# ObiRobotics/pf_monocular_pose_estimator

Hardware: AMD Instinct MI355X
Metric: particle-updates/sec (propagate+weight+resample) per GPU; frames/sec at N_particles (higher is better)
Workload: dtype f32; 1 GPU; C2: 5 LEDs, 100000 particles, 50 blobs/frame, f32 SoA state (BASELINE.json configs[1]); fused_fallbacks=0, state=f32, N_particles=100000, markers=5, blobs=50, rng=philox, parallelism=1 independent camera streams (1 per GPU), no collectives

## Files before the change

### include/pfmpe.h

```cpp
#ifndef PFMPE_H_
#define PFMPE_H_

#include <stdint.h>

#ifdef __cplusplus
extern "C" {
#endif

#define PFMPE_ABI_VERSION 1
#define PFMPE_MAX_MARKERS 16
#define PFMPE_MAX_BLOBS 1024

enum {
  PFMPE_OK = 0,
  PFMPE_E_ARG = -1,
  PFMPE_E_HIP = -2,
  PFMPE_E_CAP = -3,
  PFMPE_E_STATE = -4
};

enum { PFMPE_STATE_F32 = 0, PFMPE_STATE_F64 = 1, PFMPE_STATE_F16 = 2 };

enum {
  PFMPE_RNG_REFERENCE = 0,
// ... 113 lines not shown
void pfmpe_default_init_params(pfmpe_init_params* p);
int pfmpe_p3p_histogram(pfmpe_ctx* ctx, const double* blobs, int B, uint32_t* hist);
int pfmpe_initialise(pfmpe_ctx* ctx, const double* blobs, int B, const pfmpe_init_params* params,
                     pfmpe_init_out* out, uint32_t* hist);

#define PFMPE_INIT_MAX_STREAMS 64

typedef struct {
  const double* blobs;
  int32_t B;
  int32_t pad;
} pfmpe_init_in;
int pfmpe_initialise_multi(pfmpe_ctx* const* ctxs, int S, const pfmpe_init_in* in, const pfmpe_init_params* params,
                           pfmpe_init_out* out, uint32_t* const* hist);

typedef struct {
  int64_t items;
  int32_t first_block;
  int32_t blocks;
  int32_t bucket;
  int32_t lds_hist;
} pfmpe_init_plan;
int pfmpe_host_init_plan(const int32_t* M, const int32_t* B, int S, int num_cu, pfmpe_init_plan* plan,
                         int32_t* blocks_per_bucket);

typedef struct {
  int32_t threshold_value;
  int32_t active_markers;
  double gaussian_sigma;
  double min_blob_area;
  double max_blob_area;
  double max_width_height_distortion;
  double max_circular_distortion;
  double D[5];
  int32_t roi_x, roi_y, roi_w, roi_h;
} pfmpe_detect_params;
typedef struct {
  int32_t n;
  int32_t n_components;
  int32_t overflow;
  int32_t pad;
} pfmpe_detect_out;
void pfmpe_default_detect_params(pfmpe_detect_params* p);
int pfmpe_stage_image(pfmpe_ctx* ctx, const uint8_t* image, int width, int height, int pitch);
int pfmpe_find_leds(pfmpe_ctx* ctx, const uint8_t* image, int width, int height, int pitch,
                    const pfmpe_detect_params* params, double* blobs, float* distorted, int max_out,
                    pfmpe_detect_out* out);

#define PFMPE_DETECT_MAX_ROIS 64

int pfmpe_find_leds_multi(pfmpe_ctx* ctx, const uint8_t* image, int width, int height, int pitch,
                          const pfmpe_detect_params* params, int R, double* blobs, float* distorted,
                          int max_out, pfmpe_detect_out* out);

#define PFMPE_DETECT_MAX_IMAGES 64

typedef struct {
  pfmpe_ctx* ctx;
  const uint8_t* image;
  int32_t width, height, pitch, pad;
} pfmpe_detect_image;
int pfmpe_find_leds_streams(const pfmpe_detect_image* images, int I, const int32_t* image_of,
                            const pfmpe_detect_params* params, int R, double* blobs, float* distorted, int max_out,
                            pfmpe_detect_out* out);

typedef struct {
  int64_t offset;
  int32_t pitch;
  int32_t shared_with;
} pfmpe_detect_crop;
int pfmpe_host_detect_plan(const pfmpe_detect_image* images, int I, const int32_t* image_of,
                           const pfmpe_detect_params* params, int R, pfmpe_detect_crop* crops,
                           int64_t* upload_bytes);
int pfmpe_host_detect_pack(const pfmpe_detect_image* images, int I, const int32_t* image_of,
                           const pfmpe_detect_params* params, int R, const pfmpe_detect_crop* crops,
                           uint8_t* buffer, int64_t buffer_bytes);

int pfmpe_host_grow_roi(const int32_t roi[4], int32_t margin, int32_t image_w, int32_t image_h, int32_t grown[4]);

int pfmpe_parse_marker_yaml(const char* text, double* xyz, int max_markers);
typedef struct {
  pfmpe_params pf;
  pfmpe_init_params init;
  int32_t num_objects;
  int32_t markers_per_object[4];
  int32_t use_particle_filter;
  uint8_t downgrade[PFMPE_MAX_MARKERS];
} pfmpe_launch_config;
void pfmpe_default_launch_config(pfmpe_launch_config* cfg);
int pfmpe_parse_launch(const char* text, pfmpe_launch_config* cfg);
int pfmpe_parse_camera_info(const char* text, double* K, double* D, int32_t* width, int32_t* height);
int pfmpe_write_blob_stream(const char* path, const double* timestamps, const double* blobs, const int32_t* offsets,
                            int n_frames);
int pfmpe_read_blob_stream(const char* path, double* timestamps, double* blobs, int32_t* offsets, int max_frames,
                           int64_t max_blobs, int* n_frames, int64_t* n_blobs);
int pfmpe_stage_blob_stream(pfmpe_ctx* ctx, const char* path, int* n_frames);

int pfmpe_get_particles(pfmpe_ctx* ctx, int which, double* out);
int pfmpe_get_weights(pfmpe_ctx* ctx, double* out);
int pfmpe_get_counts(pfmpe_ctx* ctx, uint32_t* out);

enum { PFMPE_CLOUD_WEIGHTED = 0,
       PFMPE_CLOUD_POSTERIOR = 1 };
typedef struct {
  int64_t n;
  int32_t degenerate;
  int32_t pad;
  double wsum, ess;
  double mean_twist[6];
  double cov[36];
  double mean_pose[12];
  double max_trans, max_rot;
} pfmpe_cloud_out;
int pfmpe_cloud_stats(pfmpe_ctx* ctx, int which, const double* ref_pose12, pfmpe_cloud_out* out);

#define PFMPE_CLOUD_MAX_STREAMS 64

typedef struct {
  double ref_pose[12];
  int32_t which;
  int32_t pad;
} pfmpe_cloud_in;
int pfmpe_cloud_stats_multi(pfmpe_ctx* const* ctxs, int S, const pfmpe_cloud_in* in, pfmpe_cloud_out* out);

typedef struct { int32_t first_block, blocks; } pfmpe_cloud_plan;
int pfmpe_host_cloud_plan(const int32_t* N, int S, pfmpe_cloud_plan* plan, int32_t* total_blocks);

#define PFMPE_MODES_MAX 16
#define PFMPE_MODE_NONE 255
typedef struct {
  double trans_scale;
  double rot_scale;
  double max_dist;
} pfmpe_modes_params;
typedef struct {
  pfmpe_cloud_out stats;
  double share;
} pfmpe_mode_out;
void pfmpe_default_modes_params(pfmpe_modes_params* p);
int pfmpe_cloud_modes(pfmpe_ctx* ctx, int which, const double* seeds , int K,
                      const pfmpe_modes_params* params ,
                      pfmpe_mode_out* out , uint8_t* mode_of );
int pfmpe_host_cloud_assign(const double* poses, int64_t N, const double* seeds, int K,
                            const pfmpe_modes_params* params, uint8_t* mode_of, int64_t* counts );

enum { PFMPE_ASSOC_PROPAGATED = 0, PFMPE_ASSOC_POSTERIOR = 1 };
typedef struct {
  const double* blobs;
  int32_t B;
  int32_t bank_frame;
} pfmpe_assoc_in;
typedef struct {
  int64_t n;
  int32_t M, B;
  int64_t n_any;
  uint32_t matched[PFMPE_MAX_MARKERS];
  uint32_t mode_blob[PFMPE_MAX_MARKERS];
  uint32_t mode_votes[PFMPE_MAX_MARKERS];
  uint32_t second_votes[PFMPE_MAX_MARKERS];
  uint32_t npairs_hist[PFMPE_MAX_MARKERS + 1];
  uint32_t pad;
} pfmpe_assoc_out;
int pfmpe_assoc_stats(pfmpe_ctx* ctx, int which, const pfmpe_assoc_in* in, pfmpe_assoc_out* out, uint32_t* votes);
int pfmpe_get_pairs(pfmpe_ctx* ctx, int which, const pfmpe_assoc_in* in, int64_t first, int32_t count,
                    uint32_t* corr, int32_t* n_corr);

#define PFMPE_ASSOC_MAX_STREAMS 64
#define PFMPE_ASSOC_MAX_LAUNCHES 16

typedef struct {
  pfmpe_assoc_in blobs;
  int32_t which;
  int32_t pad;
} pfmpe_assoc_multi_in;
int pfmpe_assoc_stats_multi(pfmpe_ctx* const* ctxs, int S, const pfmpe_assoc_multi_in* in,
                            pfmpe_assoc_out* out, uint32_t* const* votes);

typedef struct {
  int64_t bins_offset;
  int32_t first_block, blocks, launch, lds_votes;
} pfmpe_assoc_plan;
typedef struct {
  int64_t bins_words;
  int32_t launches, pad;
  int32_t launch_blocks[PFMPE_ASSOC_MAX_LAUNCHES];
} pfmpe_assoc_plan_total;
int pfmpe_host_assoc_plan(const int32_t* N, const int32_t* M, const int32_t* B, const int32_t* which ,
                          const int32_t* prune , const int32_t* table_bytes , int S,
                          int state_dtype, pfmpe_assoc_plan* plan, pfmpe_assoc_plan_total* total);

typedef struct { double min_share; double lead; int32_t min_pairs; int32_t pad; } pfmpe_gate_params;
typedef struct { int32_t n_in, n_gated, fallback, pad; uint8_t reason[PFMPE_MAX_MARKERS]; } pfmpe_gate_out;
void pfmpe_default_gate_params(pfmpe_gate_params* p);
int pfmpe_host_gate_pairs(const uint32_t* votes, int M, int B, const uint32_t* corr ,
                          int n_corr, const pfmpe_gate_params* params ,
                          uint32_t* gated , pfmpe_gate_out* out);

#define PFMPE_TOP_MAX  1024
#define PFMPE_TOP_POOL 1024
enum { PFMPE_TOP_BY_WEIGHT = 0, PFMPE_TOP_BY_COUNT = 1 };
typedef struct {
  int32_t key;
  int32_t K;
  double  min_trans;
  double  min_rot;
} pfmpe_top_params;
typedef struct {
  int64_t n;
  int64_t n_positive;
  int32_t n_out;
  int32_t n_examined;
} pfmpe_top_out;
void pfmpe_default_top_params(pfmpe_top_params* p);
int pfmpe_top_particles(pfmpe_ctx* ctx, const pfmpe_top_params* params, const pfmpe_assoc_in* blobs, pfmpe_top_out* out,
                        int32_t* index, double* key_value, double* poses, uint32_t* corr, int32_t* n_corr);
int pfmpe_host_top_suppress(const double* poses, int32_t P, int32_t K, double min_trans, double min_rot,
                            int32_t* keep, int32_t* n_out, int32_t* n_examined);

typedef struct {
  int32_t max_iter;
  int32_t revert_on_divergence;
  double  converged;
} pfmpe_refine_params;
void pfmpe_default_refine_params(pfmpe_refine_params* p);

enum { PFMPE_REFINE_NO_PAIRS = 0, PFMPE_REFINE_CONVERGED = 1, PFMPE_REFINE_CAP_KEPT = 2, PFMPE_REFINE_CAP_REVERTED = 3 };
typedef struct {
  double pose[12];
  double rms_before, rms_after;
  int32_t iters;
  int32_t n_pairs;
  int32_t status, pad;
} pfmpe_refine_row;

typedef struct {
  int64_t n, n_with_pairs, n_converged, n_cap_kept, n_cap_reverted;
  int64_t iters_total; int32_t iters_max; int32_t pad;
  int64_t best;
  pfmpe_refine_row best_row;
  double best_cov[36];
} pfmpe_refine_out;

int pfmpe_refine_poses(pfmpe_ctx* ctx, const pfmpe_assoc_in* blobs, const pfmpe_refine_params* params,
                       const double* poses, const uint32_t* corr, int32_t K, pfmpe_refine_out* out,
                       pfmpe_refine_row* rows, double* cov);
int pfmpe_refine_cloud(pfmpe_ctx* ctx, int which, const pfmpe_assoc_in* blobs, const pfmpe_refine_params* params,
                       int64_t first, int32_t count, pfmpe_refine_out* out, pfmpe_refine_row* rows, double* cov);
#define PFMPE_REFINE_MAX_STREAMS 64
#define PFMPE_REFINE_MULTI_MAX_HYPOTHESES 65536
#define PFMPE_REFINE_DESC_BYTES 48

typedef struct {
  pfmpe_assoc_in blobs;
  const double* poses;
  const uint32_t* corr;
  int32_t K;
  int32_t pad;
} pfmpe_refine_in;
int pfmpe_refine_multi(pfmpe_ctx* const* ctxs, int S, const pfmpe_refine_in* in, const pfmpe_refine_params* params,
                       pfmpe_refine_out* out, pfmpe_refine_row* const* rows, double* const* cov);

typedef struct {
  int64_t first;
  int64_t model_offset;
  int64_t blobs_offset;
} pfmpe_refine_plan;
typedef struct {
  int64_t hypotheses;
  int64_t desc_offset, stream_of_offset, poses_offset, corr_offset;
  int64_t upload_bytes, download_bytes;
} pfmpe_refine_plan_total;
int pfmpe_host_refine_plan(const int32_t* K, const int32_t* B, int S, pfmpe_refine_plan* plan,
                           pfmpe_refine_plan_total* total);

int pfmpe_host_optimise_pose(const double* markers_xyz, int M, const double* K, const double* blobs, int B,
                             const uint32_t* corr, int n_rows, const pfmpe_refine_params* params, const double* pose12,
                             pfmpe_refine_row* row, double* cov36);

int pfmpe_step_refine(pfmpe_ctx* ctx, const pfmpe_frame_in* in, const pfmpe_refine_params* params,
                      pfmpe_frame_out* out, pfmpe_refine_out* gn, pfmpe_refine_row* row, double* cov36);
int pfmpe_step_refine_multi(pfmpe_ctx* const* ctxs, int S, const pfmpe_frame_in* in, const pfmpe_refine_params* params,
                            pfmpe_frame_out* out, pfmpe_refine_out* gn, pfmpe_refine_row* rows, double* cov);
int pfmpe_host_step_tail(const double* markers_xyz, int M, const double* K, const double* blobs, int B,
                         const pfmpe_frame_out* frame, const pfmpe_refine_params* params, pfmpe_refine_out* gn,
                         pfmpe_refine_row* row, double* cov36);

enum { PFMPE_OPT_RECORD_COUNTS = 1, PFMPE_OPT_PRUNE = 2, PFMPE_OPT_TIMING = 3, PFMPE_OPT_FUSED = 4,
       PFMPE_OPT_KEEP_PROPAGATED = 5, PFMPE_OPT_WAIT_BOUND_US = 6, PFMPE_OPT_FUSED_REARM = 7,
       PFMPE_OPT_MULTI_MAX_BLOCKS = 8, PFMPE_OPT_DEFER_RESAMPLE = 9 };
int pfmpe_set_option(pfmpe_ctx* ctx, int option, int64_t value);

enum { PFMPE_SHAPE_TWO_LAUNCH = 0,
       PFMPE_SHAPE_FRAME = 1,
       PFMPE_SHAPE_FRAME2 = 2 };
enum { PFMPE_INFO_FUSED = 1,
       PFMPE_INFO_FUSED_FALLBACKS = 2,
       PFMPE_INFO_LAST_SHAPE = 3,
       PFMPE_INFO_GUARD_SKIPS = 4,
       PFMPE_INFO_N = 5,
       PFMPE_INFO_LAST_WEIGH_PASS = 6,
       PFMPE_INFO_LAST_GRID = 7,
       PFMPE_INFO_LAST_RESAMPLE = 8,
       PFMPE_INFO_NUM_CU = 9,
       PFMPE_INFO_TAIL_FALLBACKS = 10 };
enum { PFMPE_WEIGH_BLOCKS = 0, PFMPE_WEIGH_STREAM = 1, PFMPE_WEIGH_PK = 2 };
enum { PFMPE_RESAMPLE_BLOCKS = 0, PFMPE_RESAMPLE_OWNERS = 1 };
int pfmpe_get_info(const pfmpe_ctx* ctx, int key, int64_t* value);

int pfmpe_stage_blob_bank(pfmpe_ctx* ctx, const double* blobs, const int32_t* offsets, int nframes);

enum { PFMPE_K_PROPAGATE = 0,
       PFMPE_K_RESAMPLE = 1,
       PFMPE_K_AUX = 2,
       PFMPE_K_FRAME = 3,
       PFMPE_K_ROI = 4,
       PFMPE_K_FINAL = 5,
       PFMPE_K_P3P_HIST = 6,
       PFMPE_K_P3P_CHECK = 7,
       PFMPE_K_DETECT = 8,
       PFMPE_K_COUNT = 9 };
int pfmpe_get_kernel_stats(pfmpe_ctx* ctx, int kernel, int64_t* launches, double* total_ms);
int pfmpe_reset_kernel_stats(pfmpe_ctx* ctx);
const char* pfmpe_kernel_name(int kernel);

double pfmpe_host_ref_uniform(uint32_t seed, uint64_t j, double a, double b);
void pfmpe_host_philox(const uint32_t ctr[4], const uint32_t key[2], uint32_t out[4]);
void pfmpe_host_pose_twist(const double* pose12, const double* ref_pose12, double* twist6);
int pfmpe_host_assoc_summary(const uint32_t* votes, int M, int B, pfmpe_assoc_out* out);

#ifdef __cplusplus
}
#endif
#endif
```

### pf_monocular_pose_estimator_amd/__init__.py

```python
from ._capi import (
    Engine, FrameIn, FrameOut, Params, PFError, default_params, load, host_philox, host_ref_uniform,
    STATE_F32, STATE_F64, STATE_F16, RNG_REFERENCE, RNG_PHILOX, FLAG_ACCEPTED, FLAG_REINIT,
    OPT_RECORD_COUNTS, OPT_PRUNE, OPT_TIMING, OPT_FUSED, OPT_KEEP_PROPAGATED, K_FRAME, K_ROI, K_FINAL, MAX_MARKERS, MAX_BLOBS, LIB_PATH,
    OPT_WAIT_BOUND_US, OPT_FUSED_REARM, OPT_MULTI_MAX_BLOCKS, OPT_DIAG, DIAG_LAG_LOADS, DIAG_ABANDON, DIAG_NO_STREAM, DIAG_FORCE_STREAM,
    DIAG_SERIAL_TOP, DIAG_NO_PK, DIAG_CORRUPT_DESC, DIAG_NO_DEFER, DIAG_BLOCK_RESAMPLE, DIAG_MIN_SIDE, DIAG_ABANDON_FINISH, OPT_DEFER_RESAMPLE, OK, E_ARG, E_HIP, E_CAP, E_STATE,
    SHAPE_TWO_LAUNCH, SHAPE_FRAME, SHAPE_FRAME2, INFO_FUSED, INFO_FUSED_FALLBACKS, INFO_LAST_SHAPE,
    INFO_GUARD_SKIPS, INFO_N, INFO_LAST_WEIGH_PASS, INFO_LAST_GRID, INFO_LAST_RESAMPLE, RESAMPLE_BLOCKS, RESAMPLE_OWNERS, WEIGH_BLOCKS, WEIGH_STREAM, WEIGH_PK,
    CLOUD_WEIGHTED, CLOUD_POSTERIOR, CloudOut, host_pose_twist,
    ASSOC_PROPAGATED, ASSOC_POSTERIOR, DIAG_ASSOC_DIRECT, AssocIn, AssocOut, host_assoc_summary,
    REFINE_NO_PAIRS, REFINE_CONVERGED, REFINE_CAP_KEPT, REFINE_CAP_REVERTED, REFINE_ROW_DTYPE, RefineParams, RefineRow,
    RefineOut, default_refine_params, host_optimise_pose,
    DETECT_MAX_ROIS, DetectParams, DetectOut, host_grow_roi,
    ROI_MAX_STREAMS, RoiIn, RoiOut, host_predict_roi,
    DETECT_MAX_IMAGES, DIAG_DET_COPY, DetectImage, DetectCrop, host_detect_plan, host_detect_pack,
    INIT_MAX_STREAMS, INFO_NUM_CU, InitIn, InitPlan, InitParams, InitOut, host_init_plan,
    REFINE_MAX_STREAMS, REFINE_MULTI_MAX_HYPOTHESES, REFINE_DESC_BYTES, RefineIn, RefinePlan, RefinePlanTotal,
    host_refine_plan,
    DIAG_TAIL_MISS, INFO_TAIL_FALLBACKS, host_step_tail,
    CLOUD_MAX_STREAMS, CloudIn, CloudPlan, host_cloud_plan,
    TOP_MAX, TOP_POOL, TOP_BY_WEIGHT, TOP_BY_COUNT, TopParams, TopOut, default_top_params, host_top_suppress,
    MODES_MAX, MODE_NONE, ModesParams, ModeOut, default_modes_params, host_cloud_assign,
    ASSOC_MAX_STREAMS, ASSOC_MAX_LAUNCHES, AssocMultiIn, AssocPlan, AssocPlanTotal, host_assoc_plan,
    GateParams, GateOut, default_gate_params, host_gate_pairs,
)

__all__ = [
    "Engine", "FrameIn", "FrameOut", "Params", "PFError", "default_params", "load",
    "STATE_F32", "STATE_F64", "RNG_REFERENCE", "RNG_PHILOX",
]
```

### pf_monocular_pose_estimator_amd/_capi.py

```python
from __future__ import annotations

import ctypes as C
import os

import numpy as np

_HERE = os.path.dirname(os.path.abspath(__file__))
LIB_PATH = os.path.join(_HERE, "libpfmpe.so")

MAX_MARKERS = 16
MAX_BLOBS = 1024

OK, E_ARG, E_HIP, E_CAP, E_STATE = 0, -1, -2, -3, -4
STATE_F32, STATE_F64, STATE_F16 = 0, 1, 2
RNG_REFERENCE, RNG_PHILOX = 0, 1
FLAG_ACCEPTED, FLAG_REINIT = 1, 4
OPT_RECORD_COUNTS, OPT_PRUNE, OPT_TIMING, OPT_FUSED, OPT_KEEP_PROPAGATED = 1, 2, 3, 4, 5
OPT_WAIT_BOUND_US, OPT_FUSED_REARM, OPT_MULTI_MAX_BLOCKS = 6, 7, 8
OPT_DIAG = 99
DIAG_LAG_LOADS, DIAG_ABANDON, DIAG_NO_STREAM, DIAG_FORCE_STREAM, DIAG_SERIAL_TOP = 64, 128, 512, 1024, 2048
DIAG_NO_PK, DIAG_CORRUPT_DESC, DIAG_NO_DEFER, DIAG_BLOCK_RESAMPLE, DIAG_MIN_SIDE = 4096, 8192, 16384, 32768, 65536
DIAG_ABANDON_FINISH = 131072
DIAG_DET_COPY = 524288
DIAG_TAIL_MISS = 1 << 20
DIAG_ASSOC_DIRECT = 262144
OPT_DEFER_RESAMPLE = 9
SHAPE_TWO_LAUNCH, SHAPE_FRAME, SHAPE_FRAME2 = 0, 1, 2
INFO_FUSED, INFO_FUSED_FALLBACKS, INFO_LAST_SHAPE, INFO_GUARD_SKIPS, INFO_N, INFO_LAST_WEIGH_PASS = 1, 2, 3, 4, 5, 6
INFO_LAST_GRID, INFO_LAST_RESAMPLE, INFO_NUM_CU, INFO_TAIL_FALLBACKS = 7, 8, 9, 10
WEIGH_BLOCKS, WEIGH_STREAM, WEIGH_PK = 0, 1, 2
RESAMPLE_BLOCKS, RESAMPLE_OWNERS = 0, 1
CLOUD_WEIGHTED, CLOUD_POSTERIOR = 0, 1
ASSOC_PROPAGATED, ASSOC_POSTERIOR = 0, 1
REFINE_NO_PAIRS, REFINE_CONVERGED, REFINE_CAP_KEPT, REFINE_CAP_REVERTED = 0, 1, 2, 3
K_PROPAGATE, K_RESAMPLE, K_AUX, K_FRAME, K_ROI, K_FINAL, K_P3P_HIST, K_P3P_CHECK, K_DETECT, K_COUNT = range(10)

EXPORTED_SYMBOLS = (
    "pfmpe_create", "pfmpe_destroy", "pfmpe_last_error", "pfmpe_abi_version",
    "pfmpe_set_model", "pfmpe_set_params", "pfmpe_default_params", "pfmpe_set_prior",
    "pfmpe_step", "pfmpe_step_batch", "pfmpe_step_multi", "pfmpe_step_multi_batch", "pfmpe_get_particles", "pfmpe_get_weights", "pfmpe_get_counts",
    "pfmpe_set_option", "pfmpe_stage_blob_bank", "pfmpe_get_kernel_stats",
    "pfmpe_reset_kernel_stats", "pfmpe_kernel_name", "pfmpe_host_ref_uniform", "pfmpe_host_philox",
    "pfmpe_predict_roi", "pfmpe_default_init_params", "pfmpe_p3p_histogram", "pfmpe_initialise",
    "pfmpe_parse_marker_yaml", "pfmpe_default_launch_config", "pfmpe_parse_launch", "pfmpe_parse_camera_info",
    "pfmpe_write_blob_stream", "pfmpe_read_blob_stream", "pfmpe_stage_blob_stream",
    "pfmpe_default_detect_params", "pfmpe_stage_image", "pfmpe_find_leds", "pfmpe_get_info",
    "pfmpe_cloud_stats", "pfmpe_host_pose_twist",
    "pfmpe_assoc_stats", "pfmpe_get_pairs", "pfmpe_host_assoc_summary",
    "pfmpe_default_refine_params", "pfmpe_refine_poses", "pfmpe_refine_cloud", "pfmpe_host_optimise_pose",
    "pfmpe_find_leds_multi", "pfmpe_host_grow_roi",
    "pfmpe_predict_roi_multi", "pfmpe_host_predict_roi",
    "pfmpe_find_leds_streams", "pfmpe_host_detect_plan", "pfmpe_host_detect_pack",
    "pfmpe_initialise_multi", "pfmpe_host_init_plan",
    "pfmpe_refine_multi", "pfmpe_host_refine_plan",
    "pfmpe_step_refine", "pfmpe_step_refine_multi", "pfmpe_host_step_tail",
    "pfmpe_cloud_stats_multi", "pfmpe_host_cloud_plan",
    "pfmpe_default_top_params", "pfmpe_top_particles", "pfmpe_host_top_suppress",
    "pfmpe_default_modes_params", "pfmpe_cloud_modes", "pfmpe_host_cloud_assign",
    "pfmpe_assoc_stats_multi", "pfmpe_host_assoc_plan", "pfmpe_default_gate_params", "pfmpe_host_gate_pairs",
)
MODES_MAX = 16
MODE_NONE = 255
TOP_MAX = 1024
TOP_POOL = 1024
TOP_BY_WEIGHT, TOP_BY_COUNT = 0, 1
DETECT_MAX_ROIS = 64
DETECT_MAX_IMAGES = 64
ROI_MAX_STREAMS = 64
INIT_MAX_STREAMS = 64
REFINE_MAX_STREAMS = 64
CLOUD_MAX_STREAMS = 64
ASSOC_MAX_STREAMS = 64
ASSOC_MAX_LAUNCHES = 16
REFINE_MULTI_MAX_HYPOTHESES = 65536
REFINE_DESC_BYTES = 48


class Params(C.Structure):
    _fields_ = [
        ("tol", C.c_double), ("tol_pf", C.c_double),
        ("ang_min", C.c_double), ("ang_max", C.c_double),
        ("trans_min", C.c_double), ("trans_max", C.c_double),
        ("growth", C.c_double),
        ("max_iter", C.c_int32), ("exit_cap", C.c_int32), ("accept_cap", C.c_int32),
        ("rng_mode", C.c_int32),
    ]


class FrameIn(C.Structure):
    _fields_ = [
        ("current_pose", C.c_double * 12), ("predicted_pose", C.c_double * 12),
        ("prediction", C.c_double * 12), ("cam_move_inv", C.c_double * 12),
        ("blobs", C.POINTER(C.c_double)), ("B", C.c_int32), ("bank_frame", C.c_int32),
        ("it_since_init", C.c_int32), ("force_iters", C.c_int32),
        ("dt", C.c_double), ("seed", C.c_uint64), ("frame_idx", C.c_uint64),
    ]


class RoiIn(C.Structure):
    _fields_ = [
        ("cam_move_inv", C.c_double * 12), ("prediction", C.c_double * 12), ("predicted_pose", C.c_double * 12),
        ("D", C.c_double * 5), ("image_w", C.c_int32), ("image_h", C.c_int32), ("border", C.c_int32),
        ("pad", C.c_int32),
    ]


class RoiOut(C.Structure):
    _fields_ = [("x", C.c_int32), ("y", C.c_int32), ("width", C.c_int32), ("height", C.c_int32),
                ("bbox", C.c_double * 4)]


class InitParams(C.Structure):
    _fields_ = [("certainty_threshold", C.c_double), ("valid_corr_threshold", C.c_double),
                ("n_particles", C.c_int32), ("max_candidates", C.c_int32)]


class InitOut(C.Structure):
    _fields_ = [("found", C.c_int32), ("flag_fail", C.c_int32), ("n_estimates", C.c_int32),
                ("n_candidates", C.c_int32), ("first_match", C.c_int32), ("n_corr", C.c_int32),
                ("corr", C.c_uint32 * (2 * MAX_MARKERS)), ("predicted_pose", C.c_double * 12),
                ("hist_total", C.c_uint64)]

    def as_dict(self) -> dict:
        return {"found": self.found, "flag_fail": self.flag_fail, "n_estimates": self.n_estimates,
                "n_candidates": self.n_candidates, "first_match": self.first_match,
                "pairs": np.array(self.corr[: 2 * self.n_corr], dtype=np.uint32).reshape(-1, 2),
                "predicted_pose": np.array(self.predicted_pose), "hist_total": self.hist_total}


class InitIn(C.Structure):
    _fields_ = [("blobs", C.POINTER(C.c_double)), ("B", C.c_int32), ("pad", C.c_int32)]


class InitPlan(C.Structure):
    _fields_ = [("items", C.c_int64), ("first_block", C.c_int32), ("blocks", C.c_int32), ("bucket", C.c_int32),
                ("lds_hist", C.c_int32)]

    def as_dict(self) -> dict:
        return {k: getattr(self, k) for k, _ in self._fields_}


class DetectParams(C.Structure):
    _fields_ = [("threshold_value", C.c_int32), ("active_markers", C.c_int32), ("gaussian_sigma", C.c_double),
                ("min_blob_area", C.c_double), ("max_blob_area", C.c_double),
                ("max_width_height_distortion", C.c_double), ("max_circular_distortion", C.c_double),
                ("D", C.c_double * 5), ("roi_x", C.c_int32), ("roi_y", C.c_int32), ("roi_w", C.c_int32),
                ("roi_h", C.c_int32)]


class DetectOut(C.Structure):
    _fields_ = [("n", C.c_int32), ("n_components", C.c_int32), ("overflow", C.c_int32), ("pad", C.c_int32)]


class DetectImage(C.Structure):
    _fields_ = [("ctx", C.c_void_p), ("image", C.POINTER(C.c_uint8)), ("width", C.c_int32), ("height", C.c_int32),
                ("pitch", C.c_int32), ("pad", C.c_int32)]


class DetectCrop(C.Structure):
    _fields_ = [("offset", C.c_int64), ("pitch", C.c_int32), ("shared_with", C.c_int32)]


class LaunchConfig(C.Structure):
    _fields_ = [("pf", Params), ("init", InitParams), ("num_objects", C.c_int32),
                ("markers_per_object", C.c_int32 * 4), ("use_particle_filter", C.c_int32),
                ("downgrade", C.c_uint8 * MAX_MARKERS)]


class FrameOut(C.Structure):
    _fields_ = [
        ("iters", C.c_int32), ("kept_iter", C.c_int32), ("most_likely_idx", C.c_int32),
        ("accepted", C.c_int32), ("resampled", C.c_int32), ("winner_idx", C.c_int32),
        ("n_corr", C.c_int32), ("flag_fail", C.c_int32),
        ("highest_prob", C.c_double), ("prob_sum", C.c_double),
        ("winner_pose", C.c_double * 12), ("most_likely_pose", C.c_double * 12),
        ("corr", C.c_uint32 * (2 * MAX_MARKERS)),
    ]

    def pairs(self) -> np.ndarray:
        return np.array(self.corr[: 2 * self.n_corr], dtype=np.uint32).reshape(-1, 2)

    def as_dict(self) -> dict:
        return {
            "iters": self.iters, "kept_iter": self.kept_iter, "most_likely_idx": self.most_likely_idx,
            "accepted": self.accepted, "resampled": self.resampled, "winner_idx": self.winner_idx,
            "n_corr": self.n_corr, "flag_fail": self.flag_fail, "highest_prob": self.highest_prob,
            "prob_sum": self.prob_sum, "winner_pose": np.array(self.winner_pose),
            "most_likely_pose": np.array(self.most_likely_pose), "pairs": self.pairs(),
        }


class CloudOut(C.Structure):
    _fields_ = [("n", C.c_int64), ("degenerate", C.c_int32), ("pad", C.c_int32),
                ("wsum", C.c_double), ("ess", C.c_double), ("mean_twist", C.c_double * 6),
                ("cov", C.c_double * 36), ("mean_pose", C.c_double * 12),
                ("max_trans", C.c_double), ("max_rot", C.c_double)]

    def as_dict(self) -> dict:
        return {"n": self.n, "degenerate": self.degenerate, "wsum": self.wsum, "ess": self.ess,
                "mean_twist": np.array(self.mean_twist), "cov": np.array(self.cov).reshape(6, 6),
                "mean_pose": np.array(self.mean_pose), "max_trans": self.max_trans, "max_rot": self.max_rot}


class CloudIn(C.Structure):
    _fields_ = [("ref_pose", C.c_double * 12), ("which", C.c_int32), ("pad", C.c_int32)]


class CloudPlan(C.Structure):
    _fields_ = [("first_block", C.c_int32), ("blocks", C.c_int32)]

    def as_dict(self) -> dict:
        return {"first_block": self.first_block, "blocks": self.blocks}


class ModesParams(C.Structure):
    _fields_ = [("trans_scale", C.c_double), ("rot_scale", C.c_double), ("max_dist", C.c_double)]


class ModeOut(C.Structure):
    _fields_ = [("stats", CloudOut), ("share", C.c_double)]

    def as_dict(self) -> dict:
        d = self.stats.as_dict()
        d["share"] = self.share
        return d


assert C.sizeof(ModesParams) == 24 and C.sizeof(CloudOut) == 480 and C.sizeof(ModeOut) == 488


class AssocIn(C.Structure):
    _fields_ = [("blobs", C.POINTER(C.c_double)), ("B", C.c_int32), ("bank_frame", C.c_int32)]


class AssocOut(C.Structure):
    _fields_ = [("n", C.c_int64), ("M", C.c_int32), ("B", C.c_int32), ("n_any", C.c_int64),
                ("matched", C.c_uint32 * MAX_MARKERS), ("mode_blob", C.c_uint32 * MAX_MARKERS),
                ("mode_votes", C.c_uint32 * MAX_MARKERS), ("second_votes", C.c_uint32 * MAX_MARKERS),
                ("npairs_hist", C.c_uint32 * (MAX_MARKERS + 1)), ("pad", C.c_uint32)]

    def as_dict(self) -> dict:
        M = self.M
        d = {"n": self.n, "M": M, "B": self.B, "n_any": self.n_any}
        for k in ("matched", "mode_blob", "mode_votes", "second_votes"):
            d[k] = np.array(getattr(self, k)[:M], dtype=np.uint32)
        d["npairs_hist"] = np.array(self.npairs_hist[: M + 1], dtype=np.uint32)
        return d


class AssocMultiIn(C.Structure):
    _fields_ = [("blobs", AssocIn), ("which", C.c_int32), ("pad", C.c_int32)]


class AssocPlan(C.Structure):
    _fields_ = [("bins_offset", C.c_int64), ("first_block", C.c_int32), ("blocks", C.c_int32),
                ("launch", C.c_int32), ("lds_votes", C.c_int32)]

    def as_dict(self) -> dict:
        return {k: getattr(self, k) for k, _ in self._fields_}


class AssocPlanTotal(C.Structure):
    _fields_ = [("bins_words", C.c_int64), ("launches", C.c_int32), ("pad", C.c_int32),
                ("launch_blocks", C.c_int32 * ASSOC_MAX_LAUNCHES)]

    def as_dict(self) -> dict:
        return {"bins_words": self.bins_words, "launches": self.launches,
                "launch_blocks": list(self.launch_blocks[: self.launches])}


class GateParams(C.Structure):
    _fields_ = [("min_share", C.c_double), ("lead", C.c_double), ("min_pairs", C.c_int32), ("pad", C.c_int32)]


class GateOut(C.Structure):
    _fields_ = [("n_in", C.c_int32), ("n_gated", C.c_int32), ("fallback", C.c_int32), ("pad", C.c_int32),
                ("reason", C.c_uint8 * MAX_MARKERS)]


assert (C.sizeof(AssocMultiIn), C.sizeof(AssocPlan), C.sizeof(AssocPlanTotal), C.sizeof(GateParams),
        C.sizeof(GateOut)) == (24, 24, 80, 24, 32)


class TopParams(C.Structure):
    _fields_ = [("key", C.c_int32), ("K", C.c_int32), ("min_trans", C.c_double), ("min_rot", C.c_double)]


class TopOut(C.Structure):
    _fields_ = [("n", C.c_int64), ("n_positive", C.c_int64), ("n_out", C.c_int32), ("n_examined", C.c_int32)]

    def as_dict(self) -> dict:
        return {k: getattr(self, k) for k, _ in self._fields_}


class RefineParams(C.Structure):
    _fields_ = [("max_iter", C.c_int32), ("revert_on_divergence", C.c_int32), ("converged", C.c_double)]


class RefineRow(C.Structure):
    _fields_ = [("pose", C.c_double * 12), ("rms_before", C.c_double), ("rms_after", C.c_double),
                ("iters", C.c_int32), ("n_pairs", C.c_int32), ("status", C.c_int32), ("pad", C.c_int32)]


REFINE_ROW_DTYPE = np.dtype([("pose", np.float64, 12), ("rms_before", np.float64), ("rms_after", np.float64),
                             ("iters", np.int32), ("n_pairs", np.int32), ("status", np.int32), ("pad", np.int32)])


class RefineOut(C.Structure):
    _fields_ = [("n", C.c_int64), ("n_with_pairs", C.c_int64), ("n_converged", C.c_int64), ("n_cap_kept", C.c_int64),
                ("n_cap_reverted", C.c_int64), ("iters_total", C.c_int64), ("iters_max", C.c_int32), ("pad", C.c_int32),
                ("best", C.c_int64), ("best_row", RefineRow), ("best_cov", C.c_double * 36)]

    def as_dict(self) -> dict:
        d = {k: getattr(self, k) for k in ("n", "n_with_pairs", "n_converged", "n_cap_kept", "n_cap_reverted",
                                           "iters_total", "iters_max", "best")}
        d["best_row"] = np.frombuffer(bytes(self.best_row), dtype=REFINE_ROW_DTYPE)[0].copy()
        d["best_cov"] = np.array(self.best_cov).reshape(6, 6)
        return d


class RefineIn(C.Structure):
    _fields_ = [("blobs", AssocIn), ("poses", C.POINTER(C.c_double)), ("corr", C.POINTER(C.c_uint32)),
                ("K", C.c_int32), ("pad", C.c_int32)]


class RefinePlan(C.Structure):
    _fields_ = [("first", C.c_int64), ("model_offset", C.c_int64), ("blobs_offset", C.c_int64)]

    def as_dict(self) -> dict:
        return {k: getattr(self, k) for k, _ in self._fields_}


# ... 1131 lines not shown
```

### pf_monocular_pose_estimator_amd/csrc/pf_kernels.hpp

```cpp
#pragma once
#include <stddef.h>
#include <stdint.h>

#include <algorithm>
#include <cstring>
#include <type_traits>

#include "pf_desc_tag.hpp"
#include "pf_likelihood.hpp"

namespace pfmpe {

template <typename T, int RNG>
__device__ __forceinline__ double target_num(const FrameArgsT<T>& fa, int iters, int64_t k) {
  double U;
  if (RNG == kRngReference) {
    const uint64_t motion = fa.N > 2 ? (uint64_t)12 * (uint64_t)(fa.N - 2) * (uint64_t)iters : 0u;
    const uint32_t g1 = lcg_output(fa.lcg_x0, motion + 2u * (uint64_t)k + 1u);
    const uint32_t g2 = lcg_next(g1);
    U = ref_uniform(ref_canonical(g1, g2), 0.0, 1.0);
  } else {
    const U32x4 o = philox4x32_10((uint32_t)k, kTagResample << 24, fa.flo, fa.fhi, fa.key0, fa.key1);
    U = u53(o.x, o.y);
  }
// ... 2247 lines not shown
  __shared__ ResampleLds<T> rsh;
  __shared__ OutDev rec;
  __shared__ FrameLds fsh;

  if (stamps && threadIdx.x == 0) stamp_min(stamps, 0, rt_now());
  const int n = blockIdx.x * kBlock + threadIdx.x;
  const bool valid = n < fa.N;
  const int lane = lane_id(), wv = wave_id();
  const int blk = blockIdx.x, g = blk / fa.gsz;

  copy_table(table, smem, (size_t)fa.tbytes);
  T A[12];
  if (valid && n >= 2) load_prior(fa, prior, n, A);
  const uint32_t gen_base = ((uint32_t)seq & 0xffffu) << 16;
  Ctrl c = load_ctrl_wt(ctrl);
  stage_consts(fa, sc);
  __syncthreads();
  const LdsBlobs<T> tb = view_table<T>(smem, fa.B);
  if (stamps && threadIdx.x == 0) {
    const uint64_t t = rt_now();
    stamp_max(stamps, 8, t);
    stamp_min(stamps, 19, t);
  }

  T P[12], w = (T)0;
  int iter = 0;
  for (;; ++iter) {
    const int slot = c.cur_slot;
    if (valid) {
      w = weigh_particle<T, RNG, MAXM, PRUNE>(fa, sc, tb, A, n, iter, P);
      (slot ? w1 : w0)[n] = w;
    }
    if (stamps && threadIdx.x == 0) stamp_max(stamps, 9, rt_now());
    publish_iteration<T, RNG>(fa, w, valid, n, slot, iter, wsh, part0, part1, bscan0, bscan1, gpart0, gpart1, gscan,
                              ctrl, gcount_w, tcount_w, gen, gen_base, stamps, blk);
    if (wv == 0) {
      int ab = 0;
      if (lane == 0) {
        const uint32_t want = gen_base + (uint32_t)iter + 1u;
        const uint64_t t0 = rt_now();
        while (__hip_atomic_load((gu32_t*)gen, __ATOMIC_RELAXED, __HIP_MEMORY_SCOPE_AGENT) != want) {
          __builtin_amdgcn_s_sleep(2);
          if (rt_now() - t0 > fa.wait_ticks) {
            ab = 1;
            break;
          }
        }
      }
      ab = lane_value(ab, 0);
      if (!ab) {
        constexpr int kCw = (int)(sizeof(Ctrl) / 8);
        static_assert(sizeof(Ctrl) % 8 == 0 && kCw + 8 <= 64, "Ctrl words");
        const uint64_t* src = nullptr;
        uint64_t* dst = nullptr;
        if (lane < kCw) {
          src = (const uint64_t*)ctrl + lane;
          dst = (uint64_t*)&fsh.c + lane;
        } else if (lane < kCw + 6) {
          const int sl = (lane - kCw) / 3, q = (lane - kCw) % 3;
          src = (const uint64_t*)((sl ? bscan1 : bscan0) + blk) + q;
          dst = (uint64_t*)&fsh.bs[sl] + q;
        } else if (lane < kCw + 8) {
          src = (const uint64_t*)(gscan + g) + (lane - kCw - 6);
          dst = (uint64_t*)&fsh.gs + (lane - kCw - 6);
        }
        if (src) *dst = ld_wt(src);
      }
      if (lane == 0) fsh.abort = ab;
    }
    __syncthreads();
    if (fsh.abort) return;
    c = fsh.c;
    if (c.done) break;
  }

  if (!c.accepted) {
    if (blk == 0 && wv == 0)
      finalize_frame<T, RNG, MAXM, SP>(fa, sc, c, ctrl, prior, -1, cand, mlpose, rec, out, 2 * seq + 1, stamps);
    return;
  }
  const int kslot = c.kept_slot;
  const bool have_P = c.kept_iter == iter;
  double wd = 0.0;
  if (valid) {
    if (have_P) {
      wd = (double)w;
    } else {
      wd = (double)(kslot ? w1 : w0)[n];
    }
  }
  const BlockScan bs = fsh.bs[kslot];
  const GroupScan gs = fsh.gs;
  if (flat)
    resample_phase<T, RNG, MAXM, SP, 2>(fa, sc, c, ctrl, table, prior, post, wd, A, P, have_P, bs, gs, rsh, rec, tb, cand,
                                        mlpose, cpart, cgroup, gcount_r, tcount_r, counts, out, seq, stamps, flat, blk);
  else
    resample_phase<T, RNG, MAXM, SP, 1>(fa, sc, c, ctrl, table, prior, post, wd, A, P, have_P, bs, gs, rsh, rec, tb, cand,
                                        mlpose, cpart, cgroup, gcount_r, tcount_r, counts, out, seq, stamps, nullptr,
                                        blk);
}

struct WaveArg {
  double maxw, minw;
  int argmax, argmin;
};
struct Frame2Lds {
  GroupPart gp[2][kFlatMaxGroups];
  WaveArg wa[2][kWaves];
  BlockScan bs[2];
  int dirty[kWaves];
  GroupScan gs;
  Ctrl c;
  Frame2Tail tail;
  int abort;
};

struct BlockIn {
  bool vb, mine;
  BlockPart p;
};
__device__ __forceinline__ bool group_math2(const BlockIn (&in)[2], GroupPart (&out)[2], BlockScan* own, WaveArg& wa,
                                            double (&zmin_in)[2]) {
  double sum[2], maxrel[2], minrel[2];
  double maxw = -INFINITY, minw = INFINITY;
  int amax = 0x7fffffff, amin = 0x7fffffff;
  bool min_placeholder = true, dirty = false;
#pragma unroll
  for (int k = 0; k < 2; ++k) {
    const bool vb = in[k].vb;
    if (vb) {
      cmb_max(maxw, amax, in[k].p.maxw, in[k].p.argmax);
      cmb_min(minw, amin, in[k].p.minw, in[k].p.argmin);
    }
    min_placeholder &= !vb || (in[k].p.minw == (double)INFINITY && in[k].p.argmin == 0x7fffffff);
    dirty |= vb && !(in[k].p.minw >= 0.0 && in[k].p.sum == in[k].p.sum);
    sum[k] = vb ? in[k].p.sum : 0.0;
    maxrel[k] = vb ? in[k].p.maxrel : -INFINITY;
    minrel[k] = vb ? in[k].p.minrel : INFINITY;
  }
  double incl[2] = {sum[0], sum[1]};
  if (__builtin_amdgcn_ballot_w64(!min_placeholder) == 0) {
    scan_steps([&](auto st) {
      using S = decltype(st);
      st_sum<S>(incl[0]);
      st_sum<S>(incl[1]);
      st_argmax<S>(maxw, amax);
    });
    minw = INFINITY;
    amin = 0x7fffffff;
  } else {
    scan_steps([&](auto st) {
      using S = decltype(st);
      st_sum<S>(incl[0]);
      st_sum<S>(incl[1]);
      st_argmax<S>(maxw, amax);
      st_argmin<S>(minw, amin);
    });
    bcast63(minw, amin);
  }
  double E[2], zi_max[2];
#pragma unroll
  for (int k = 0; k < 2; ++k) {
    E[k] = 0.0 + wave_shr1(incl[k], 0.0);
    zi_max[k] = in[k].vb ? E[k] + maxrel[k] : -INFINITY;
    zmin_in[k] = in[k].vb ? E[k] + minrel[k] : INFINITY;
  }
  scan_steps([&](auto st) {
    using S = decltype(st);
    st_max<S>(zi_max[0]);
    st_max<S>(zi_max[1]);
  });
  bcast63(maxw, amax);
  wa.maxw = maxw;
  wa.minw = minw;
  wa.argmax = amax;
  wa.argmin = amin;
#pragma unroll
  for (int k = 0; k < 2; ++k) {
    double zp_max = wave_shr1(zi_max[k], -(double)INFINITY);
    zp_max = zp_max > -INFINITY ? zp_max : -INFINITY;
    if (in[k].vb && in[k].mine) {
      own->E = E[k];
      own->zin_max = zp_max;
      own->zin_min = INFINITY;
      own->pad = 0.0;
    }
    const double tmax = lane_value(zi_max[k], 63);
    GroupPart& r = out[k];
    r.sum = 0.0 + lane_value(incl[k], 63);
    r.zmax = tmax > -INFINITY ? tmax : -INFINITY;
    r.zmin = INFINITY;
    r.maxw = -INFINITY;
    r.minw = INFINITY;
    r.argmax = r.argmin = 0x7fffffff;
  }
  return __builtin_amdgcn_ballot_w64(dirty) != 0;
}
__device__ __forceinline__ void group_zmin2(const BlockIn (&in)[2], double (&zi_min)[2], BlockScan* own, GroupPart* gp0,
                                            GroupPart* gp1) {
  scan_steps([&](auto st) {
    using S = decltype(st);
    st_min<S>(zi_min[0]);
    st_min<S>(zi_min[1]);
  });
#pragma unroll
  for (int k = 0; k < 2; ++k) {
    double zp_min = wave_shr1(zi_min[k], (double)INFINITY);
    zp_min = zp_min < INFINITY ? zp_min : INFINITY;
    if (in[k].vb && in[k].mine) own->zin_min = zp_min;
    const double tmin = lane_value(zi_min[k], 63);
    GroupPart* g = k ? gp1 : gp0;
    if (g && lane_id() == 0) g->zmin = tmin < INFINITY ? tmin : INFINITY;
  }
}

__device__ __forceinline__ double lanes8_incl_sum(double x) {
  x = x + dpp<kDppRowShr1>(x, 0.0);
  x = x + dpp<kDppRowShr2>(x, 0.0);
  x = x + dpp<kDppRowShr4>(x, 0.0);
  return x + 0.0;
}

template <typename T, int RNG, typename KeptF, typename ArgF>
__device__ __forceinline__ Ctrl top_math_regs(const FrameArgsT<T>& fa, Ctrl c, int iter, int slot, const GroupPart& q0,
                                              KeptF qk, ArgF garg, double* G_out, double* Gin_out,
                                              double* run_out) {
  const int lane = lane_id();
  const int ngrp = fa.ngrp;
  double incl = lanes8_incl_sum(lane < ngrp ? q0.sum : 0.0);
  double mv, mn_;
  int mi, ni_;
  garg(slot, mv, mi, mn_, ni_);
  if (mv > c.best_max) {
    c.best_max = mv;
    c.best_idx = mi;
    c.best_iter = iter;
    c.best_slot = slot;
    c.has_best = 1;
  }
  c.iters = iter + 1;
  const bool go_on = fa.force_iters > 0 ? (c.iters < fa.force_iters) : (c.iters < fa.max_iter && mv < fa.exit_thr);
  c.cur_slot = c.has_best ? 1 - c.best_slot : 1 - slot;
  if (!go_on) {
    c.done = 1;
    c.kept_slot = c.has_best ? c.best_slot : slot;
    c.kept_iter = c.has_best ? c.best_iter : iter;
    GroupPart kq = q0;
    double amv = mv, anv = mn_;
    int ami = mi, ani = ni_;
    if (c.kept_slot != slot) {
      kq = qk(c.kept_slot);
      incl = lanes8_incl_sum(lane < ngrp ? kq.sum : 0.0);
      garg(c.kept_slot, amv, ami, anv, ani);
    }
    const double S = 0.0 + lane_value(incl, 7);
    double run = -INFINITY;
    {
      const double prev = wave_shr1(incl, 0.0);
      const double G = lane == 0 ? 0.0 : 0.0 + prev;
      double cm = -INFINITY;
      if (lane < ngrp && S != 0.0) cm = (G + (S > 0.0 ? kq.zmax : kq.zmin)) / S;
      const double im = wave_incl_max(cm);
      double ex = wave_shr1(im, -(double)INFINITY);
      ex = ex > run ? ex : run;
      *G_out = G;
      *Gin_out = ex;
      const double tm = lane_value(im, 63);
      run = tm > run ? tm : run;
    }
    if (S == 0.0) run = -INFINITY;
    const double highest = c.has_best ? c.best_max : 0.0;
    c.S = S;
    c.invS = 1.0 / S;
    c.accepted = (S != 0.0 && highest > fa.accept_thr) ? 1 : 0;
    if (c.accepted) {
      c.most_likely_idx = c.best_idx;
#if PFMPE_TAIL_KT_IN_COUNTS
      *run_out = run;
      c.K_total = 0;
#else
      int64_t kt = lane == 0 ? count_targets<T, RNG>(fa, c.iters, run) : 0;
      c.K_total = (int64_t)(((uint64_t)(uint32_t)__builtin_amdgcn_readlane((int)(uint32_t)kt, 0)) |
                            ((uint64_t)(uint32_t)__builtin_amdgcn_readlane((int)(uint32_t)((uint64_t)kt >> 32), 0) << 32));
#endif
    } else {
      c.most_likely_idx = (S < 0.0) ? ani : ami;
      c.K_total = 0;
    }
  }
  return c;
}

#ifndef PFMPE_FRAME2_MIN_WAVES
#define PFMPE_FRAME2_MIN_WAVES 3
#endif
template <typename T>
struct Frame2Shared {
  LdsConst<T> sc;
  WeighLds wsh;
  ResampleLds<T> rsh;
  OutDev rec;
  Frame2Lds fl;
};
template <typename T, int RNG, int MAXM, bool PRUNE, typename SP>
__device__ __forceinline__ bool frame2_body(
    const FrameArgsT<T>& fa, const uint32_t* fa_words, const unsigned char* __restrict__ table,
    const SP* __restrict__ prior, SP* __restrict__ post, T* __restrict__ w0, T* __restrict__ w1,
    BlockPart* __restrict__ part0, BlockPart* __restrict__ part1, Ctrl* __restrict__ ctrl,
    CountPart* __restrict__ cpart, uint32_t* __restrict__ flat, uint32_t* __restrict__ counts, Cand* __restrict__ cand,
    double* __restrict__ mlpose, RecOut* __restrict__ out, int32_t seq, uint64_t* __restrict__ stamps,
    unsigned char* smem, Frame2Shared<T>& S2) {
  LdsConst<T>& sc = S2.sc;
  WeighLds& wsh = S2.wsh;
  ResampleLds<T>& rsh = S2.rsh;
  OutDev& rec = S2.rec;
  Frame2Lds& fl = S2.fl;
  if (stamps && threadIdx.x == 0) stamp_min(stamps, 0, rt_now());
  const int n = blockIdx.x * kBlock + threadIdx.x;
  const bool valid = n < fa.N;
  const int lane = lane_id(), wv = wave_id();
  const int blk = blockIdx.x, g_own = blk / fa.gsz;

  T A[12];
  if (valid && n >= 2) load_prior(fa, prior, n, A);
  stage_table_consts(table, smem, (size_t)fa.tbytes, fa_words, sc);
  if (threadIdx.x == 0) {
    fl.c = zero_ctrl();
    fl.abort = 0;
  }
  __syncthreads();
  const LdsBlobs<T> tb = view_table<T>(smem, fa.B);
  if (stamps && threadIdx.x == 0) {
    const uint64_t t = rt_now();
    stamp_max(stamps, 8, t);
    stamp_min(stamps, 19, t);
  }

  T P[12], w = (T)0;
  Ctrl c = fl.c;
  int iter = 0;
  for (;; ++iter) {
    const int slot = c.cur_slot;
    if (valid) {
      w = weigh_particle<T, RNG, MAXM, PRUNE, true>(fa, sc, tb, A, n, iter, P, nullptr, stamps);
      (slot ? w1 : w0)[n] = w;
    }
    if (stamps && threadIdx.x == 0) stamp_max(stamps, 9, rt_now());
    {
      double wi, rmx, rmn;
      T mx, mn;
      int ix, in_;
      wave_weight_partials(w, valid, n, wi, rmx, rmn, mx, ix, mn, in_);
      if (lane == 63) wsh.tot[wv] = wi;
      if (lane == 0) {
        wsh.rmax[wv] = rmx;
        wsh.rmin[wv] = rmn;
        wsh.mx[wv] = (double)mx;
        wsh.mn[wv] = (double)mn;
        wsh.ix[wv] = ix;
        wsh.in_[wv] = in_;
      }
      __syncthreads();
      if (wv == 0) {
        if (lane == 0) {
          double pre = 0.0, maxrel = -INFINITY, minrel = INFINITY, bmx = wsh.mx[0], bmn = wsh.mn[0];
          int bix = wsh.ix[0], bin = wsh.in_[0];
#pragma unroll
          for (int ww = 0; ww < kWaves; ++ww) {
            const double a = pre + wsh.rmax[ww], b = pre + wsh.rmin[ww];
            maxrel = a > maxrel ? a : maxrel;
            minrel = b < minrel ? b : minrel;
            if (ww) {
              cmb_max(bmx, bix, wsh.mx[ww], wsh.ix[ww]);
              cmb_min(bmn, bin, wsh.mn[ww], wsh.in_[ww]);
            }
            pre = pre + wsh.tot[ww];
          }
          BlockPart* bp = ((iter & 1) ? part1 : part0) + blk;
          st_wt_d(&bp->sum, pre);
          st_wt_d(&bp->maxrel, maxrel);
          st_wt_d(&bp->minrel, minrel);
          st_wt_d(&bp->maxw, bmx);
          st_wt_d(&bp->minw, bmn);
          st_wt(&bp->argmax, pack2(bix, bin));
          if (stamps) stamp_max(stamps, 1, rt_now());
          flat_arrive(flat, blk);
        }
        const uint32_t target = fa.flat_base_w + (uint32_t)(iter + 1) * (uint32_t)fa.nblk;
        const bool ok = !(fa.diag & kDiagAbandon) && flat_wait(flat, target, fa.wait_ticks);
        if (lane == 0 && !ok) fl.abort = 1;
      }
      __syncthreads();
      if (fl.abort) return false;
    }
    if (stamps && threadIdx.x == 0) stamp_max(stamps, 2, rt_now());
    BlockIn in[2];
    double zmin_in[2];
    {
      const BlockPart* pp = (iter & 1) ? part1 : part0;
      if ((fa.diag & kDiagLagLoads) && blk == fa.nblk - 1) {
        const uint64_t t0 = rt_now();
        while (rt_now() - t0 < 2000u) __builtin_amdgcn_s_sleep(2);
      }
      const int b0 = threadIdx.x, b1 = threadIdx.x + kBlock;
      const bool v0 = b0 < fa.nblk, v1 = b1 < fa.nblk;
      PartRaw r0, r1;
      ld_part_issue(pp + (v0 ? b0 : 0), r0);
      ld_part_issue(pp + (v1 ? b1 : 0), r1);
      wait_parts(r0, r1);
      if (stamps && threadIdx.x == 0) stamp_max(stamps, 24, rt_now());
      in[0].vb = v0;
      in[0].mine = b0 == blk;
      in[0].p = unpack_part(r0);
      in[1].vb = v1;
      in[1].mine = b1 == blk;
      in[1].p = unpack_part(r1);
      GroupPart gp[2];
      WaveArg wa;
      const bool dirty = group_math2(in, gp, &fl.bs[slot], wa, zmin_in);
      if (lane == 0) fl.wa[slot][wv] = wa;
      if (lane == 0 && wv < fa.ngrp) fl.gp[slot][wv] = gp[0];
      if (lane == 0 && wv + kWaves < fa.ngrp) fl.gp[slot][wv + kWaves] = gp[1];
      if (lane == 0) fl.dirty[wv] = dirty;
    }
    if (stamps && threadIdx.x == 0) stamp_max(stamps, 25, rt_now());
    __syncthreads();
    int dirty = 0;
#pragma unroll
    for (int w = 0; w < kWaves; ++w) dirty |= fl.dirty[w];
    if (dirty || (fa.diag & kDiagMinSide)) {
      group_zmin2(in, zmin_in, &fl.bs[slot], wv < fa.ngrp ? &fl.gp[slot][wv] : nullptr,
                  wv + kWaves < fa.ngrp ? &fl.gp[slot][wv + kWaves] : nullptr);
      __syncthreads();
    }
    if (wv == 0) {
      auto qk = [&](int ks) {
        const bool v = lane < fa.ngrp;
        const GroupPart& src = fl.gp[ks][v ? lane : 0];
        GroupPart q;
        q.sum = v ? src.sum : 0.0;
        q.zmax = v ? src.zmax : -INFINITY;
        q.zmin = v ? src.zmin : INFINITY;
        q.maxw = v ? src.maxw : -INFINITY;
        q.minw = v ? src.minw : INFINITY;
        q.argmax = v ? src.argmax : 0x7fffffff;
        q.argmin = v ? src.argmin : 0x7fffffff;
        return q;
      };
      const GroupPart q0 = qk(slot);
      auto garg = [&](int ks, double& mxv, int& mxi, double& mnv, int& mni) {
        mxv = fl.wa[ks][0].maxw;
        mxi = fl.wa[ks][0].argmax;
        mnv = fl.wa[ks][0].minw;
        mni = fl.wa[ks][0].argmin;
#pragma unroll
        for (int w = 1; w < kWaves; ++w) {
          cmb_max(mxv, mxi, fl.wa[ks][w].maxw, fl.wa[ks][w].argmax);
          cmb_min(mnv, mni, fl.wa[ks][w].minw, fl.wa[ks][w].argmin);
        }
      };
      double G = 0.0, Gin = -INFINITY, run = -INFINITY;
      const Ctrl cn = top_math_regs<T, RNG>(fa, c, iter, slot, q0, qk, garg, &G, &Gin, &run);
      if (lane == 0) fl.tail.run = run;
      if (lane == g_own) {
        fl.gs.G = G;
        fl.gs.Gin = Gin;
      }
      if (lane == 0) fl.c = cn;
      if (stamps && lane == 0) stamp_max(stamps, 26, rt_now());
    }
    __syncthreads();
    c = fl.c;
    if (stamps && threadIdx.x == 0) stamp_max(stamps, 3, rt_now());
    if (c.done) break;
  }

  if (!c.accepted) {
    if (blk == 0 && wv == 0)
      finalize_frame<T, RNG, MAXM, SP>(fa, sc, c, ctrl, prior, -1, cand, mlpose, rec, out, 2 * seq + 1, stamps);
    return true;
  }
  const int kslot = c.kept_slot;
  const bool have_P = c.kept_iter == iter;
  double wd = 0.0;
  if (valid) wd = have_P ? (double)w : (double)(kslot ? w1 : w0)[n];
  const BlockScan bs = fl.bs[kslot];
  const GroupScan gs = fl.gs;
  resample_phase<T, RNG, MAXM, SP, 2>(fa, sc, c, ctrl, table, prior, post, wd, A, P, have_P, bs, gs, rsh, rec,
                                                 tb, cand, mlpose, cpart, nullptr, nullptr, nullptr, counts, out, seq,
                                                 stamps, flat, blk, nullptr, nullptr, &fl.tail);
  return true;
}

template <typename T, int RNG, int MAXM, bool PRUNE, typename SP>
__global__ __launch_bounds__(kBlock) __attribute__((amdgpu_waves_per_eu(PFMPE_FRAME2_MIN_WAVES))) void k_frame2(
    const FrameArgsT<T> fa, const unsigned char* __restrict__ table, const SP* __restrict__ prior,
    SP* __restrict__ post, T* __restrict__ w0, T* __restrict__ w1, BlockPart* __restrict__ part0,
    BlockPart* __restrict__ part1, Ctrl* __restrict__ ctrl, CountPart* __restrict__ cpart,
    uint32_t* __restrict__ flat, uint32_t* __restrict__ counts, Cand* __restrict__ cand,
    double* __restrict__ mlpose, RecOut* __restrict__ out, int32_t seq, uint64_t* __restrict__ stamps) {
  extern __shared__ __attribute__((aligned(16))) unsigned char smem[];
  __shared__ Frame2Shared<T> S2;
  (void)frame2_body<T, RNG, MAXM, PRUNE, SP>(fa, (const uint32_t*)__builtin_amdgcn_kernarg_segment_ptr(), table, prior,
                                             post, w0, w1, part0, part1, ctrl, cpart, flat, counts, cand, mlpose, out,
                                             seq, stamps, smem, S2);
}

template <typename T, int RNG, typename SP>
__global__ __launch_bounds__(kBlock) void k_regen(const FrameArgsT<T> fa, int kept_iter, const SP* __restrict__ prior,
                                                 double* __restrict__ poses) {
  __shared__ LdsConst<T> sc;
  stage_consts(fa, sc);
  __syncthreads();
  const int n = blockIdx.x * blockDim.x + threadIdx.x;
  if (n >= fa.N) return;
  T P[12];
  make_particle<T, RNG, SP>(fa, sc, prior, n, kept_iter, P);
  for (int q = 0; q < 12; ++q) poses[12 * (int64_t)n + q] = (double)P[q];
}
template <typename T, int RNG, typename SP>
__global__ __launch_bounds__(kBlock) void k_regen_list(const FrameArgsT<T> fa, int kept_iter, const SP* __restrict__ prior,
                                                      const int32_t* __restrict__ list, const uint32_t* __restrict__ count,
                                                      int limit, double* __restrict__ poses) {
  __shared__ LdsConst<T> sc;
  stage_consts(fa, sc);
  __syncthreads();
  const int i = blockIdx.x * blockDim.x + threadIdx.x;
  const uint32_t cnt = *count;
  if (i >= limit || (uint32_t)i >= cnt) return;
  const int n = list[i];
  if (n < 0 || n >= fa.N) return;
  T P[12];
  make_particle<T, RNG, SP>(fa, sc, prior, n, kept_iter, P);
  for (int q = 0; q < 12; ++q) poses[12 * (int64_t)i + q] = (double)P[q];
}
template <typename T, int RNG, typename SP>
__global__ __launch_bounds__(64) void k_group_top_multi(const StreamDesc<T, SP>* __restrict__ descs, int S,
                                                        const uint32_t* __restrict__ status, uint32_t gen, int iter) {
  const int s = (int)blockIdx.y;
  if (s >= S || __builtin_amdgcn_readfirstlane(status[s]) != gen) return;
  const StreamDesc<T, SP>& d = descs[s];
  const int g = (int)blockIdx.x;
  const int ngrp = __builtin_amdgcn_readfirstlane(d.fa.ngrp);
  if (g >= ngrp) return;
  Ctrl* ctrl = d.ctrl;
  if (load_ctrl_word<(int)offsetof(Ctrl, done)>(ctrl)) return;
  const int slot = load_ctrl_word<(int)offsetof(Ctrl, cur_slot)>(ctrl);
  const GroupPart gr = propagate_group<true>(__builtin_amdgcn_readfirstlane(d.fa.nblk), __builtin_amdgcn_readfirstlane(d.fa.gsz),
                                             g, slot ? d.part1 : d.part0, slot ? d.bscan1 : d.bscan0,
                                             slot ? d.gpart1 : d.gpart0);
  const bool single = ngrp == 1;
  if (!single && !wave_arrive_last(d.tcount_w, ngrp)) return;
  propagate_top<T, RNG>(d.fa, ctrl, iter, d.gpart0, d.gpart1, d.gscan, nullptr, 0u, gr, single, slot);
}
template <typename T, typename SP>
__global__ __launch_bounds__(64) void k_group_multi(const StreamDesc<T, SP>* __restrict__ descs, int S,
                                                    const uint32_t* __restrict__ status, uint32_t gen) {
  const int s = (int)blockIdx.y;
  if (s >= S || __builtin_amdgcn_readfirstlane(status[s]) != gen) return;
  const StreamDesc<T, SP>& d = descs[s];
  const int g = (int)blockIdx.x;
  if (g >= __builtin_amdgcn_readfirstlane(d.fa.ngrp)) return;
  if (load_ctrl_word<(int)offsetof(Ctrl, done)>(d.ctrl)) return;
  const int slot = load_ctrl_word<(int)offsetof(Ctrl, cur_slot)>(d.ctrl);
  (void)propagate_group<true>(__builtin_amdgcn_readfirstlane(d.fa.nblk), __builtin_amdgcn_readfirstlane(d.fa.gsz), g,
                              slot ? d.part1 : d.part0, slot ? d.bscan1 : d.bscan0, slot ? d.gpart1 : d.gpart0);
}
template <typename T, int RNG, typename SP>
__global__ __launch_bounds__(64 * kTopWaves) void k_top_wide_multi(const StreamDesc<T, SP>* __restrict__ descs, int S,
                                                                const uint32_t* __restrict__ status, uint32_t gen,
                                                                int iter) {
  extern __shared__ __attribute__((aligned(16))) GroupPart gsm[];
  __shared__ TopWideLds tw;
  const int s = (int)blockIdx.x;
  if (s >= S || __builtin_amdgcn_readfirstlane(status[s]) != gen) return;
  const StreamDesc<T, SP>& d = descs[s];
  top_wide_body<T, RNG>(d.fa, d.gpart0, d.gpart1, d.gscan, d.ctrl, iter, gsm, tw);
}
template <typename T, int RNG, typename SP>
__global__ __launch_bounds__(64) void k_top_multi(const StreamDesc<T, SP>* __restrict__ descs, int S,
                                                  const uint32_t* __restrict__ status, uint32_t gen, int iter) {
  const int s = (int)blockIdx.x;
  if (s >= S || __builtin_amdgcn_readfirstlane(status[s]) != gen) return;
  const StreamDesc<T, SP>& d = descs[s];
  top_body<T, RNG>(d.fa, d.gpart0, d.gpart1, d.gscan, d.ctrl, iter, 0, nullptr);
}

}
```

### pf_monocular_pose_estimator_amd/csrc/pf_likelihood.hpp

```cpp
#pragma once
#include <algorithm>
#include <cmath>
#include <cstring>
#include <vector>

#include "pf_state.hpp"
#include "pf_wave.hpp"

namespace pfmpe {

template <typename T>
__device__ __forceinline__ void k_times_pose(const LdsConst<T>& sc, const T* P, bool k_upper, T* Q) {
  if (std::is_same<T, float>::value && k_upper) {
#pragma unroll
    for (int j = 0; j < 4; j += 2) {
      const f32x2 p0 = pk2(P[0 * 4 + j], P[0 * 4 + j + 1]);
      const f32x2 p1 = pk2(P[1 * 4 + j], P[1 * 4 + j + 1]);
      const f32x2 p2 = pk2(P[2 * 4 + j], P[2 * 4 + j + 1]);
      f32x2 s = p0 * sc.K[0];
      s = pk_fma(pk2(sc.K[1], sc.K[1]), p1, s);
      s = pk_fma(pk2(sc.K[2], sc.K[2]), p2, s);
      const f32x2 s1 = pk_fma(pk2(sc.K[5], sc.K[5]), p2, p1 * sc.K[4]);
      Q[0 * 4 + j] = s.x;
      Q[0 * 4 + j + 1] = s.y;
      Q[1 * 4 + j] = s1.x;
      Q[1 * 4 + j + 1] = s1.y;
      Q[2 * 4 + j] = P[2 * 4 + j];
      Q[2 * 4 + j + 1] = P[2 * 4 + j + 1];
    }
    return;
  }
#pragma unroll
  for (int i = 0; i < 3; ++i) {
#pragma unroll
    for (int j = 0; j < 4; ++j) {
      T s = sc.K[i * 3 + 0] * P[0 * 4 + j];
      s = fmadd(sc.K[i * 3 + 1], P[1 * 4 + j], s);
      s = fmadd(sc.K[i * 3 + 2], P[2 * 4 + j], s);
      Q[i * 4 + j] = s;
    }
  }
}

template <typename T, int MAXM>
__device__ __forceinline__ void project_markers(const FrameArgsT<T>& fa, const LdsConst<T>& sc, const T* P, T* u,
                                                T* v) {
  T Q[12];
  k_times_pose<T>(sc, P, fa.k_upper != 0, Q);
  if constexpr (std::is_same<T, float>::value) {
    const f32x2 q0 = pk2(Q[0], Q[4]), q1 = pk2(Q[1], Q[5]), q2 = pk2(Q[2], Q[6]), q3 = pk2(Q[3], Q[7]);
#pragma unroll
    for (int j = 0; j < MAXM; ++j) {
      const float X = sc.markers[3 * j], Y = sc.markers[3 * j + 1], Z = sc.markers[3 * j + 2];
      f32x2 s = q0 * X;
      s = pk_fma(q1, pk2(Y, Y), s);
      s = pk_fma(q2, pk2(Z, Z), s);
      s = s + q3;
      float z = Q[8] * X;
      z = fmadd(Q[9], Y, z);
      z = fmadd(Q[10], Z, z);
      z = z + Q[11];
      const f32x2 uv = s * rcp_t(z);
      u[j] = uv.x;
      v[j] = uv.y;
    }
    return;
  }
#pragma unroll
  for (int j = 0; j < MAXM; ++j) {
    if (marker_live<MAXM>(j, fa.M)) {
      const T X = sc.markers[3 * j], Y = sc.markers[3 * j + 1], Z = sc.markers[3 * j + 2];
      T p[3];
#pragma unroll
      for (int i = 0; i < 3; ++i) {
        T s = Q[i * 4 + 0] * X;
        s = fmadd(Q[i * 4 + 1], Y, s);
        s = fmadd(Q[i * 4 + 2], Z, s);
        p[i] = s + Q[i * 4 + 3];
      }
      persp(p[0], p[1], p[2], &u[j], &v[j]);
    } else {
      u[j] = v[j] = (T)0;
    }
  }
}

template <typename T>
__device__ __forceinline__ void project_one(const LdsConst<T>& sc, const T* P, int j, bool k_upper, T& u, T& v) {
  T Q[12];
  k_times_pose<T>(sc, P, k_upper, Q);
  const T X = sc.markers[3 * j], Y = sc.markers[3 * j + 1], Z = sc.markers[3 * j + 2];
  T p[3];
#pragma unroll
  for (int i = 0; i < 3; ++i) {
    T s = Q[i * 4 + 0] * X;
    s = fmadd(Q[i * 4 + 1], Y, s);
    s = fmadd(Q[i * 4 + 2], Z, s);
    p[i] = s + Q[i * 4 + 3];
  }
  persp(p[0], p[1], p[2], &u, &v);
}

__host__ __device__ __forceinline__ constexpr int bucket_count(int B) {
  int nb = 128;
  while (nb < kMaxBuckets && nb < 2 * B) nb *= 2;
  return nb;
}
template <typename T>
__host__ __device__ __forceinline__ int bucket_of(T x, T xmin, T inv_bw, int nb) {
  const T f = (x - xmin) * inv_bw;
  if (!(f >= (T)0)) return 0;
  if (f >= (T)(nb - 1)) return nb - 1;
  return (int)f;
}
template <typename T>
struct alignas(2 * sizeof(T)) BlobXY {
  T x, y;
};

template <typename T>
struct LdsBlobs;

__device__ __forceinline__ int bucket_of_bf(float x, float xmin, float inv_bw, int nb) {
  const float f = (x - xmin) * inv_bw;
  return (int)__builtin_fminf(__builtin_fmaxf(f, 0.0f), (float)(nb - 1));
}

template <typename T, int MAXM, bool PRUNE, bool PHASED = false>
__device__ __forceinline__ int column_minima(const FrameArgsT<T>& fa, const T* u, const T* v,
                                             const LdsBlobs<T>& tb, T* m, int* r) {
  const int B = fa.B, M = fa.M;
  int visited = 0;
  if constexpr (std::is_same<T, float>::value) {
    const GridArgs& ga = fa.grid;
    if (PRUNE && ga.on) {
      const unsigned char* cells = tb.base + ga.cell_off;
      const unsigned char* ents = tb.base + ga.ent_off;
      const f32x2 ic = pk2(ga.inv_c, ga.inv_c), oc = pk2(ga.ox, ga.oy);
      if constexpr (PHASED) {
        uint32_t rec[MAXM];
  #pragma unroll
        for (int j = 0; j < MAXM; ++j) {
          rec[j] = 0;
          if (marker_live<MAXM>(j, M)) {
            const f32x2 f = pk_fma(pk2(u[j], v[j]), ic, oc);
            const int cx = (int)__builtin_amdgcn_fmed3f(f.x, 0.0f, ga.fmaxx);
            const int cy = (int)__builtin_amdgcn_fmed3f(f.y, 0.0f, ga.fmaxy);
            rec[j] = *(const uint32_t*)(cells + mad24(cy, ga.ncx4, cx << 2));
          }
        }
        constexpr int c1 = MAXM > kExactM ? 2 : 1;
        bool more = false;
  #pragma unroll
        for (int j = 0; j < MAXM; ++j) {
          float bd = INFINITY;
          int bo = 0;
          if (marker_live<MAXM>(j, M)) {
            const f32x2 uvj = pk2(u[j], v[j]);
            const GridEnt* e = (const GridEnt*)(ents + (rec[j] & 0xffffu));
            const int n = (int)(rec[j] >> 16);
            visited += n;
            more |= n > c1;
            const GridEnt e0 = e[0];
            const f32x2 dd = pk2(e0.x, e0.y) - uvj;
            bd = __builtin_fminf(fmadd(dd.x, dd.x, dd.y * dd.y), INFINITY);
            bo = e0.orig;
            if constexpr (c1 == 2) {
              const GridEnt e1 = e[1];
              const f32x2 d1 = pk2(e1.x, e1.y) - uvj;
              const float d = fmadd(d1.x, d1.x, d1.y * d1.y);
              const bool take = (n > 1) & (d < bd);
              bd = take ? d : bd;
              bo = take ? e1.orig : bo;
            }
          }
          m[j] = bd;
          r[j] = bo;
        }
        if (__builtin_amdgcn_ballot_w64(more)) {
  #pragma unroll
          for (int j = 0; j < MAXM; ++j) {
            if (!marker_live<MAXM>(j, M)) continue;
            const int n = (int)(rec[j] >> 16);
            if (!__builtin_amdgcn_ballot_w64(n > c1)) continue;
            const f32x2 uvj = pk2(u[j], v[j]);
            const GridEnt* e = (const GridEnt*)(ents + (rec[j] & 0xffffu));
            float bd = m[j];
            int bo = r[j];
            auto visit = [&](const GridEnt& ec, bool in) {
              const f32x2 dd = pk2(ec.x, ec.y) - uvj;
              const float d = fmadd(dd.x, dd.x, dd.y * dd.y);
              const bool take = in & (d < bd);
              bd = take ? d : bd;
              bo = take ? ec.orig : bo;
            };
  #pragma unroll 2
            for (int c = c1; c < n; c += 2) {
              const GridEnt ea = e[c], eb = e[c + 1];
              visit(ea, true);
              visit(eb, c + 1 < n);
            }
            m[j] = bd;
            r[j] = bo;
          }
        }
      } else {
  #pragma unroll
        for (int j = 0; j < MAXM; ++j) {
          float bd = INFINITY;
          int bo = 0;
          if (marker_live<MAXM>(j, M)) {
            const f32x2 uvj = pk2(u[j], v[j]);
            const f32x2 f = pk_fma(uvj, ic, oc);
            const int cx = (int)__builtin_amdgcn_fmed3f(f.x, 0.0f, ga.fmaxx);
            const int cy = (int)__builtin_amdgcn_fmed3f(f.y, 0.0f, ga.fmaxy);
            const uint32_t rec = *(const uint32_t*)(cells + mad24(cy, ga.ncx4, cx << 2));
            const GridEnt* e = (const GridEnt*)(ents + (rec & 0xffffu));
            const int n = (int)(rec >> 16);
            visited += n;
            auto visit = [&](const GridEnt& ec, bool in) {
              const f32x2 dd = pk2(ec.x, ec.y) - uvj;
              const float d = fmadd(dd.x, dd.x, dd.y * dd.y);
              const bool take = in & (d < bd);
              bd = take ? d : bd;
              bo = take ? ec.orig : bo;
            };
            constexpr int c1 = MAXM > kExactM ? 2 : 1;
            {
              const GridEnt e0 = e[0];
              const f32x2 dd = pk2(e0.x, e0.y) - uvj;
              bd = __builtin_fminf(fmadd(dd.x, dd.x, dd.y * dd.y), INFINITY);
              bo = e0.orig;
              if constexpr (c1 == 2) visit(e[1], n > 1);
            }
            if (__builtin_amdgcn_ballot_w64(n > c1)) {
  #pragma unroll 2
              for (int c = c1; c < n; c += 2) {
                const GridEnt ea = e[c], eb = e[c + 1];
                visit(ea, true);
                visit(eb, c + 1 < n);
              }
            }
          }
          m[j] = bd;
          r[j] = bo;
        }
      }
      return visited;
    }
    const float fmaxb = (float)(tb.nb - 1);
    const float base_lo = tb.xmin + fa.tolq, base_hi = tb.xmin - fa.tolq;
#pragma unroll
    for (int j = 0; j < MAXM; ++j) {
      uint64_t best = ((uint64_t)0x7f800000u << 32) | 0x7fffffffu;
      if (marker_live<MAXM>(j, M)) {
        int c0 = 0, c1 = B;
        if (PRUNE) {
          const float flo = (u[j] - base_lo) * tb.inv_bw;
          const float fhi = (u[j] - base_hi) * tb.inv_bw;
          c0 = tb.bstart[(int)__builtin_amdgcn_fmed3f(flo, 0.0f, fmaxb)];
          c1 = tb.bstart[(int)__builtin_amdgcn_fmed3f(fhi, 0.0f, fmaxb) + 1];
        }
        visited += c1 - c0;
        const float uj = u[j], vj = v[j];
        const f32x2 uvj = pk2(uj, vj);
        auto visit = [&](BlobXY<float> p, int o, bool in) {
          const f32x2 dd = pk2(p.x, p.y) - uvj;
          const float d = fmadd(dd.x, dd.x, dd.y * dd.y);
          const uint64_t key = ((uint64_t)__float_as_uint(d) << 32) | (uint32_t)o;
          best = (in & (key < best)) ? key : best;
        };
        for (int c = c0; c < c1; c += 2) {
          const BlobXY<float> pa = tb.bxy[c], pb = tb.bxy[c + 1];
          const int oa = tb.orig[c], ob = tb.orig[c + 1];
          visit(pa, oa, true);
          visit(pb, ob, c + 1 < c1);
        }
      }
      const float bm = __uint_as_float((uint32_t)(best >> 32));
      m[j] = bm;
      r[j] = bm < INFINITY ? (int)(uint32_t)best : 0;
    }
    return visited;
  }
#pragma unroll
  for (int j = 0; j < MAXM; ++j) {
    T best = inf_t<T>();
    int bc = -1;
    if (marker_live<MAXM>(j, M)) {
      int c0 = 0, c1 = B;
      if (PRUNE) {
        c0 = tb.bstart[bucket_of(u[j] - fa.tolq, tb.xmin, tb.inv_bw, tb.nb)];
        c1 = tb.bstart[bucket_of(u[j] + fa.tolq, tb.xmin, tb.inv_bw, tb.nb) + 1];
      }
      visited += c1 - c0;
      auto visit = [&](int c, BlobXY<T> p) {
        const T dx = p.x - u[j];
        const T dy = p.y - v[j];
        const T d = fmadd(dx, dx, dy * dy);
        if (d < best) {
          best = d;
          bc = c;
        } else if (d == best && bc >= 0 && tb.orig[c] < tb.orig[bc]) {
          bc = c;
        }
      };
      int c = c0;
      for (; c + 1 < c1; c += 2) {
        const BlobXY<T> pa = tb.bxy[c], pb = tb.bxy[c + 1];
        visit(c, pa);
        visit(c + 1, pb);
      }
      if (c < c1) visit(c, tb.bxy[c]);
    }
    m[j] = best;
    r[j] = bc >= 0 ? tb.orig[bc] : 0;
  }
  return visited;
}

template <typename T>
__device__ __forceinline__ bool nan_at_origin(T b0x, T b0y, T u0, T v0) {
  const T dx = b0x - u0, dy = b0y - v0;
  const T d = dx * dx + dy * dy;
  return d != d;
}
template <typename T>
__device__ __forceinline__ bool nan_at_origin_tb(const FrameArgsT<T>& fa, const LdsBlobs<T>& tb, T u0, T v0) {
  if (fa.grid.b0fin) return __builtin_isunordered(u0, v0);
  const T* hdr = (const T*)tb.base;
  return nan_at_origin(hdr[2], hdr[3], u0, v0);
}

template <typename T>
__device__ __forceinline__ void cas_key(T& ma, int& ja, int& ra, T& mb, int& jb, int& rb) {
  const bool sw = mb < ma || (mb == ma && jb < ja);
  const T m0 = sw ? mb : ma, m1 = sw ? ma : mb;
  const int j0 = sw ? jb : ja, j1 = sw ? ja : jb;
  const int r0 = sw ? rb : ra, r1 = sw ? ra : rb;
  ma = m0; mb = m1; ja = j0; jb = j1; ra = r0; rb = r1;
}
template <typename T, int MAXM>
__device__ __forceinline__ void sort_minima(T* km, int* kj, int* kr) {
#pragma unroll
  for (int p = 1; p < MAXM; p <<= 1)
#pragma unroll
    for (int k = p; k >= 1; k >>= 1)
#pragma unroll
      for (int j = k % p; j + k < MAXM; j += 2 * k)
#pragma unroll
        for (int i = 0; i < k; ++i)
          if (i + j + k < MAXM && (i + j) / (2 * p) == (i + j + k) / (2 * p))
            cas_key(km[i + j], kj[i + j], kr[i + j], km[i + j + k], kj[i + j + k], kr[i + j + k]);
}

template <typename T, int MAXM, bool PAIRS>
__device__ __forceinline__ T score_minima(const FrameArgsT<T>& fa, const T* m, const int* r, uint32_t* pairs,
                                          int* npairs) {
  const int B = fa.B, M = fa.M;
  const int L = B < M ? B : M;
  const T tol = fa.tol, tol_pf = fa.tol_pf, Mt = (T)M;
  T km[MAXM];
  int kj[MAXM], kr[MAXM];
#pragma unroll
  for (int j = 0; j < MAXM; ++j) {
    km[j] = marker_live<MAXM>(j, M) ? m[j] : inf_t<T>();
    kj[j] = j;
    kr[j] = r[j];
  }
  sort_minima<T, MAXM>(km, kj, kr);
  T Pr = (T)0;
  int s = 1;
  bool live = true;
  if (PAIRS) *npairs = 0;
#pragma unroll
  for (int k = 0; k < MAXM; ++k) {
    if (k < L && live) {
      const T d = sqrt_t(km[k]);
      if (!(d <= tol_pf)) {
        live = false;
      } else {
        const T q = div_t(tol - d, tol);
        Pr = Pr + (Mt + q * q);
        bool dup = false;
#pragma unroll
        for (int e = 0; e < k; ++e) dup |= kr[e] == kr[k];
        if (dup) {
          Pr = Pr - (T)(s * 3);
          ++s;
        }
        if ((fa.downgrade >> kj[k]) & 1u) Pr = Pr - (T)2;
        if (PAIRS) {
          pairs[2 * k] = (uint32_t)kj[k] + 1u;
          pairs[2 * k + 1] = (uint32_t)kr[k] + 1u;
          *npairs = k + 1;
        }
      }
    }
  }
  return Pr;
}

template <int MAXM>
__device__ __forceinline__ float score_unordered(const FrameArgsT<float>& fa, const float* m, const int* r) {
  const int M = fa.M;
  const float tol = fa.tol, tol_pf = fa.tol_pf, Mt = (float)M;
  const float rtol = rcp_t(tol);
  float Pr = 0.0f;
  int dups = 0;
  bool acc[MAXM];
#pragma unroll
  for (int j = 0; j < MAXM; ++j) {
    const float d = sqrt_t(m[j]);
    acc[j] = d <= tol_pf;
    const float q = (tol - d) * rtol;
    Pr = acc[j] ? Pr + (Mt + q * q) : Pr;
    bool dup = false;
#pragma unroll
    for (int e = 0; e < j; ++e) dup |= acc[e] & (r[e] == r[j]);
    dups += (acc[j] & dup) ? 1 : 0;
  }
  int ndg = 0;
  if (fa.downgrade) {
#pragma unroll
    for (int j = 0; j < MAXM; ++j) ndg += (acc[j] && ((fa.downgrade >> j) & 1u)) ? 1 : 0;
  }
  return Pr - (float)(3 * dups * (dups + 1) / 2 + 2 * ndg);
}

constexpr int kGridMaxCells = 8192;
constexpr int kGridCoarseCells = 2048;
#ifndef PFMPE_GRID_FINE_MIN_BLOBS
#define PFMPE_GRID_FINE_MIN_BLOBS 128
#endif
constexpr int kGridFineMinBlobs = PFMPE_GRID_FINE_MIN_BLOBS;
constexpr int kGridMaxEntries = 1024;
template <typename T>
struct BlobTable {
  static constexpr size_t off_bstart() { return align16(4 * sizeof(T)); }
  static constexpr size_t off_xy(int B) { return off_bstart() + align16((size_t)(bucket_count(B) + 1) * 4); }
  static constexpr size_t off_orig(int B) { return off_xy(B) + align16((size_t)B * sizeof(BlobXY<T>)); }
  static constexpr size_t bytes(int B) { return off_orig(B) + align16((size_t)B * 4); }
  static constexpr size_t off_grid(int B) { return bytes(B); }
  static constexpr size_t grid_bytes(int ncell, int nent) {
    return sizeof(GridHdr) + align16((size_t)ncell * 4) + (size_t)(nent + 1) * sizeof(GridEnt);
  }
  static constexpr size_t total_bytes(int B, int ncell, int nent) { return bytes(B) + grid_bytes(ncell, nent); }
  static constexpr size_t max_bytes() { return total_bytes(kMaxBlobs, kGridMaxCells, kGridMaxEntries); }
  static constexpr size_t lds_bytes(size_t tbytes) { return tbytes + 16; }
};

template <typename T>
struct LdsBlobs {
  const unsigned char* base;
  const BlobXY<T>* bxy;
  const int32_t* orig;
  const int32_t* bstart;
  T xmin, inv_bw;
  int nb;
};

template <typename T>
__host__ __device__ __forceinline__ LdsBlobs<T> view_table(const unsigned char* base, int B) {
  LdsBlobs<T> t;
  const T* hdr = (const T*)base;
  t.base = base;
  t.xmin = hdr[0];
  t.inv_bw = hdr[1];
  t.nb = bucket_count(B);
  t.bstart = (const int32_t*)(base + BlobTable<T>::off_bstart());
  t.bxy = (const BlobXY<T>*)(base + BlobTable<T>::off_xy(B));
  t.orig = (const int32_t*)(base + BlobTable<T>::off_orig(B));
  return t;
}

template <typename T>
inline GridArgs grid_args(const GridHdr& gh, int B, float tolq) {
  GridArgs g{};
  g.b0fin = gh.b0fin;
  g.on = (gh.ncell > 0 && gh.gtolq >= tolq) ? 1 : 0;
  if (!g.on) return g;
  g.inv_c = gh.inv_c;
  g.ox = (float)(-(double)gh.gx0 * (double)gh.inv_c);
  g.oy = (float)(-(double)gh.gy0 * (double)gh.inv_c);
  g.fmaxx = gh.fmaxx;
  g.fmaxy = gh.fmaxy;
  g.ncx4 = 4 * gh.ncx;
  g.cell_off = (int32_t)(BlobTable<T>::off_grid(B) + sizeof(GridHdr));
  g.ent_off = g.cell_off + (int32_t)align16((size_t)gh.ncell * 4);
  return g;
}

template <typename T>
inline size_t build_blob_table_host(const double* blobs, int B, double tolq, unsigned char* dst) {
  T xmin = (T)INFINITY, xmax = -(T)INFINITY;
  for (int i = 0; i < B; ++i) {
    const T x = (T)blobs[2 * i];
    xmin = x < xmin ? x : xmin;
    xmax = x > xmax ? x : xmax;
  }
  if (B == 0 || !(xmax - xmin < (T)INFINITY)) {
    xmin = (T)0;
    xmax = (T)1;
  }
  T span = xmax - xmin;
  if (!(span > (T)0)) span = (T)1;
  const int nb = bucket_count(B);
  const T inv_bw = (T)nb / span;
  T* hdr = (T*)dst;
  hdr[0] = xmin;
  hdr[1] = inv_bw;
  hdr[2] = B > 0 ? (T)blobs[0] : (T)0;
  hdr[3] = B > 0 ? (T)blobs[1] : (T)0;
  int32_t* bstart = (int32_t*)(dst + BlobTable<T>::off_bstart());
  BlobXY<T>* xy = (BlobXY<T>*)(dst + BlobTable<T>::off_xy(B));
  int32_t* orig = (int32_t*)(dst + BlobTable<T>::off_orig(B));
  int32_t cnt[kMaxBuckets + 1] = {0};
  for (int i = 0; i < B; ++i) ++cnt[bucket_of((T)blobs[2 * i], xmin, inv_bw, nb) + 1];
  for (int b = 0; b < nb; ++b) cnt[b + 1] += cnt[b];
  for (int b = 0; b <= nb; ++b) bstart[b] = cnt[b];
  for (int i = 0; i < B; ++i) {
    const int pos = cnt[bucket_of((T)blobs[2 * i], xmin, inv_bw, nb)]++;
    xy[pos].x = (T)blobs[2 * i];
    xy[pos].y = (T)blobs[2 * i + 1];
    orig[pos] = i;
  }
  GridHdr* gh = (GridHdr*)(dst + BlobTable<T>::off_grid(B));
  std::memset(gh, 0, sizeof(GridHdr));
  gh->b0fin = (B > 0 && std::isfinite((double)hdr[2]) && std::isfinite((double)hdr[3])) ? 1 : 0;
  size_t total = BlobTable<T>::total_bytes(B, 0, 0);
  if (!std::is_same<T, float>::value || B == 0) return total;
  const double m = tolq + 0.01;
  double bx0 = INFINITY, bx1 = -INFINITY, by0 = INFINITY, by1 = -INFINITY;
  for (int i = 0; i < B; ++i) {
    const double x = (double)(float)blobs[2 * i], y = (double)(float)blobs[2 * i + 1];
    if (!(x - x == 0.0) || !(y - y == 0.0)) return total;
    bx0 = std::min(bx0, x), bx1 = std::max(bx1, x), by0 = std::min(by0, y), by1 = std::max(by1, y);
  }
  const double gx0 = bx0 - m, gy0 = by0 - m, w = bx1 - bx0 + 2 * m, h = by1 - by0 + 2 * m;
  for (int budget = B >= kGridFineMinBlobs ? kGridMaxCells : kGridCoarseCells;; budget = kGridCoarseCells) {
  double cs = std::max(2.0 * m, std::sqrt(w * h / (double)budget));
  int ncx = (int)std::ceil(w / cs), ncy = (int)std::ceil(h / cs);
  while ((int64_t)ncx * ncy > budget) {
    cs *= 1.0625;
    ncx = (int)std::ceil(w / cs);
    ncy = (int)std::ceil(h / cs);
  }
  ncx = std::max(1, ncx);
  ncy = std::max(1, ncy);
  const float inv_c = (float)(1.0 / cs), gx0f = (float)gx0, gy0f = (float)gy0;
  {
    const double ex = std::ldexp(std::abs((double)gx0f) * (double)inv_c + ncx + 1.0, -23) * cs;
    const double ey = std::ldexp(std::abs((double)gy0f) * (double)inv_c + ncy + 1.0, -23) * cs;
    if (!(std::max(ex, ey) <= 0.25 * (m - tolq))) return total;
  }
  auto crange = [&](double lo, double hi, float inv, float org, int n, int& c0, int& c1) {
    const double f0 = (lo - (double)org) * (double)inv, f1 = (hi - (double)org) * (double)inv;
    c0 = (int)std::max(0.0, std::min((double)(n - 1), std::floor(f0)));
    c1 = (int)std::max(0.0, std::min((double)(n - 1), std::floor(f1)));
  };
  const int ncell = ncx * ncy;
  std::vector<int32_t> count(ncell + 1, 0);
  int nent = 0;
  for (int pass = 0; pass < 2; ++pass) {
    std::vector<int32_t> fill;
    if (pass == 1) {
      for (int c = 0; c < ncell; ++c) count[c + 1] += count[c];
      fill.assign(count.begin(), count.end() - 1);
    }
    for (int i = 0; i < B; ++i) {
      const double x = (double)(float)blobs[2 * i], y = (double)(float)blobs[2 * i + 1];
      int cx0, cx1, cy0, cy1;
      crange(x - m, x + m, inv_c, gx0f, ncx, cx0, cx1);
      crange(y - m, y + m, inv_c, gy0f, ncy, cy0, cy1);
      for (int cy = cy0; cy <= cy1; ++cy)
        for (int cx = cx0; cx <= cx1; ++cx) {
          const int c = cy * ncx + cx;
          if (pass == 0) {
            ++count[c + 1];
            ++nent;
          } else {
            const int e = 1 + fill[c]++;
            GridEnt* ent = (GridEnt*)((unsigned char*)gh + sizeof(GridHdr) + align16((size_t)ncell * 4));
            ent[e] = GridEnt{(float)blobs[2 * i], (float)blobs[2 * i + 1], i, 0};
          }
        }
    }
    if (pass == 0 && nent > kGridMaxEntries) break;
  }
  if (nent > kGridMaxEntries) {
    if (budget == kGridCoarseCells) return total;
    continue;
  }
  uint32_t* cell = (uint32_t*)((unsigned char*)gh + sizeof(GridHdr));
  for (int c = 0; c < ncell; ++c) {
    const uint32_t n = (uint32_t)(count[c + 1] - count[c]);
    cell[c] = (n ? (uint32_t)(1 + count[c]) * (uint32_t)sizeof(GridEnt) : 0u) | (n << 16);
  }
  GridEnt* ent = (GridEnt*)((unsigned char*)cell + align16((size_t)ncell * 4));
  ent[0] = GridEnt{INFINITY, INFINITY, 0, 0};

  gh->inv_c = inv_c;
  gh->gx0 = gx0f;
  gh->gy0 = gy0f;
  gh->fmaxx = (float)(ncx - 1);
  gh->fmaxy = (float)(ncy - 1);
  gh->gtolq = (float)tolq;
  gh->ncx = ncx;
  gh->ncell = ncell;
  gh->nent = nent;
  return BlobTable<T>::total_bytes(B, ncell, nent);
  }
}

__device__ __forceinline__ void copy_table(const unsigned char* __restrict__ src, unsigned char* dst, size_t bytes) {
  typedef __attribute__((address_space(1))) const u32x4_t gv4_t;
  gv4_t* s4 = (gv4_t*)src;
  u32x4_t* d4 = (u32x4_t*)dst;
  const int n4 = (int)(bytes / 16);
  for (int i = threadIdx.x; i < n4; i += kBlock) d4[i] = s4[i];
}

template <typename T>
__device__ __forceinline__ void stage_table_consts(const unsigned char* __restrict__ src, unsigned char* dst, size_t bytes,
                                                   const uint32_t* cw_src, LdsConst<T>& sc) {
  typedef __attribute__((address_space(1))) const u32x4_t gv4_t;
  gv4_t* s4 = (gv4_t*)src;
  u32x4_t* d4 = (u32x4_t*)dst;
  const int n4 = (int)(bytes / 16);
  const int t = threadIdx.x;
  constexpr int kWordsC = (int)(sizeof(LdsConst<T>) / 4);
  static_assert(kWordsC <= kBlock, "one constant word per thread");
  u32x4_t r0 = {0u, 0u, 0u, 0u}, r1 = {0u, 0u, 0u, 0u};
  uint32_t cw = 0u;
  if (t < n4) r0 = s4[t];
  if (t + kBlock < n4) r1 = s4[t + kBlock];
  if (t < kWordsC) cw = cw_src[t];
  if (t < n4) d4[t] = r0;
  if (t + kBlock < n4) d4[t + kBlock] = r1;
  if (t < kWordsC) ((uint32_t*)&sc)[t] = cw;
  for (int i = t + 2 * kBlock; i < n4; i += kBlock) d4[i] = s4[i];
}

template <typename T, int RNG, int MAXM, bool PRUNE, bool PHASED = false>
__device__ __forceinline__ T weigh_particle(const FrameArgsT<T>& fa, const LdsConst<T>& sc, const LdsBlobs<T>& tb,
                                            const T* A, int n, int iter, T* P, int* nvisit = nullptr,
                                            uint64_t* st = nullptr) {
  T u[MAXM], v[MAXM];
  propagate<T, RNG>(fa, sc, A, n, iter, P);
  if (st && threadIdx.x == 0) stamp_max(st, 27, rt_now() + (P[11] == (T)12345 ? 1 : 0));
  project_markers<T, MAXM>(fa, sc, P, u, v);
  if (st && threadIdx.x == 0) stamp_max(st, 28, rt_now() + (u[0] == (T)12345 ? 1 : 0));
  T w = (T)0;
  if (fa.B > 0 && !nan_at_origin_tb(fa, tb, u[0], v[0])) {
    T m[MAXM];
    int r[MAXM];
    const int visited = column_minima<T, MAXM, PRUNE, PHASED>(fa, u, v, tb, m, r);
    if (nvisit) *nvisit = visited;
    if (st && threadIdx.x == 0) stamp_max(st, 29, rt_now() + (m[0] == (T)12345 ? 1 : 0));
    if constexpr (std::is_same<T, float>::value) {
      if (fa.B >= fa.M && !(fa.diag & kDiagSortedScore))
        w = score_unordered<MAXM>(fa, m, r);
      else
        w = score_minima<T, MAXM, false>(fa, m, r, nullptr, nullptr);
    } else {
      w = score_minima<T, MAXM, false>(fa, m, r, nullptr, nullptr);
    }
  }
  return w;
}

}
```

### pf_monocular_pose_estimator_amd/csrc/pf_rng.hpp

```cpp
#pragma once
#include <stdint.h>

#if defined(__HIPCC__)
#include <hip/hip_runtime.h>
#define PF_HD __host__ __device__ __forceinline__
#else
#define PF_HD inline
#endif

namespace pfmpe {

constexpr uint32_t kLcgA = 16807u;
constexpr uint32_t kLcgM = 2147483647u;

PF_HD uint32_t mulmod_m31(uint32_t a, uint32_t b) {
  const uint64_t p = (uint64_t)a * (uint64_t)b;
  uint64_t r = (p & kLcgM) + (p >> 31);
  r = (r & kLcgM) + (r >> 31);
  return (uint32_t)(r >= kLcgM ? r - kLcgM : r);
}

PF_HD uint32_t powmod_a(uint64_t e) {
  e %= (uint64_t)(kLcgM - 1u);
  uint32_t result = 1u, base = kLcgA;
  while (e) {
    if (e & 1u) result = mulmod_m31(result, base);
    base = mulmod_m31(base, base);
    e >>= 1;
  }
  return result;
}

PF_HD uint32_t lcg_seed(uint32_t s) {
  const uint32_t x = s % kLcgM;
  return x == 0u ? 1u : x;
}

PF_HD uint32_t lcg_output(uint32_t x0, uint64_t j) { return mulmod_m31(powmod_a(j), x0); }

PF_HD uint32_t lcg_next(uint32_t x) { return mulmod_m31(x, kLcgA); }

PF_HD double ref_canonical(uint32_t g1, uint32_t g2) {
  double sum = (double)(g1 - 1u);
  const double t = (double)(g2 - 1u) * 2147483646.0;
  sum = sum + t;
  double ret = sum / 4611686009837453312.0;
  if (ret >= 1.0) ret = 0x1.fffffffffffffp-1;
  return ret;
}

PF_HD double ref_uniform(double u, double a, double b) { return u * (b - a) + a; }

struct U32x4 {
  uint32_t x, y, z, w;
};

PF_HD uint32_t xor3_key(uint32_t a, uint32_t b, uint32_t k) {
#if defined(__HIP_DEVICE_COMPILE__)
  uint32_t r;
  asm("v_bitop3_b32 %0, %1, %2, %3 bitop3:0x96" : "=v"(r) : "v"(a), "v"(b), "s"(k));
  return r;
#else
  return a ^ b ^ k;
#endif
}

PF_HD U32x4 philox4x32_10(uint32_t c0, uint32_t c1, uint32_t c2, uint32_t c3, uint32_t k0, uint32_t k1) {
#if defined(__HIP_DEVICE_COMPILE__)
  asm volatile("" : "+s"(k0), "+s"(k1));
#endif
#pragma unroll
  for (int r = 0; r < 10; ++r) {
    if (r) {
      k0 += 0x9E3779B9u;
      k1 += 0xBB67AE85u;
    }
    const uint64_t p0 = (uint64_t)0xD2511F53u * c0;
    const uint64_t p1 = (uint64_t)0xCD9E8D57u * c2;
    const uint32_t n0 = xor3_key((uint32_t)(p1 >> 32), c1, k0);
    const uint32_t n1 = (uint32_t)p1;
    const uint32_t n2 = xor3_key((uint32_t)(p0 >> 32), c3, k1);
    const uint32_t n3 = (uint32_t)p0;
    c0 = n0; c1 = n1; c2 = n2; c3 = n3;
  }
  return U32x4{c0, c1, c2, c3};
}

PF_HD float u24f(uint32_t x) { return (float)(x >> 8) * (1.0f / 16777216.0f); }
PF_HD double u24d(uint32_t x) { return (double)(x >> 8) * (1.0 / 16777216.0); }
PF_HD double u53(uint32_t x0, uint32_t x1) {
  return ((double)(x0 >> 5) * 67108864.0 + (double)(x1 >> 6)) * (1.0 / 9007199254740992.0);
}

enum : uint32_t { kTagMotion = 0u, kTagResample = 2u };

struct Draws6 {
  uint32_t v[6];
};
PF_HD Draws6 philox_motion6(uint32_t n, uint32_t iter, uint32_t flo, uint32_t fhi, uint32_t k0, uint32_t k1) {
  const U32x4 o = philox4x32_10(n, iter | (kTagMotion << 24), flo, fhi, k0, k1);
  Draws6 d;
  d.v[0] = o.x >> 11;
  d.v[1] = o.y >> 11;
  d.v[2] = o.z >> 11;
  d.v[3] = o.w >> 11;
  d.v[4] = ((o.x & 0x7FFu) << 10) | (o.y & 0x3FFu);
  d.v[5] = ((o.z & 0x7FFu) << 10) | (o.w & 0x3FFu);
  return d;
}
PF_HD float u21f(uint32_t v) { return (float)v * (1.0f / 2097152.0f); }
PF_HD double u21d(uint32_t v) { return (double)v * (1.0 / 2097152.0); }

}
```

### pf_monocular_pose_estimator_amd/csrc/pf_state.hpp

```cpp
#pragma once
#include <hip/hip_fp16.h>
#include <math.h>

#include <type_traits>

#include "pf_rng.hpp"
#include "pf_types.hpp"

namespace pfmpe {

__host__ __device__ __forceinline__ float fmadd(float a, float b, float c) { return __builtin_fmaf(a, b, c); }
__host__ __device__ __forceinline__ double fmadd(double a, double b, double c) { return a * b + c; }
__device__ __forceinline__ void sincos_t(float x, float* s, float* c) {
  if (fabsf(x) <= 0.25f) {
    const float x2 = x * x;
    *s = x * fmadd(x2, fmadd(x2, fmadd(x2, fmadd(x2, 1.0f / 362880.0f, -1.0f / 5040.0f), 1.0f / 120.0f),
                             -1.0f / 6.0f), 1.0f);
    *c = fmadd(x2, fmadd(x2, fmadd(x2, fmadd(x2, 1.0f / 40320.0f, -1.0f / 720.0f), 1.0f / 24.0f), -0.5f), 1.0f);
  } else {
    sincosf(x, s, c);
  }
}
constexpr float kSmallAngle = 0.03f;
__device__ __forceinline__ void sincos_small(float x, float* s, float* c) {
  const float x2 = x * x;
  *s = x * fmadd(x2, -1.0f / 6.0f, 1.0f);
  *c = fmadd(x2, fmadd(x2, 1.0f / 24.0f, -0.5f), 1.0f);
}
__device__ __forceinline__ void sincos_t(double x, double* s, double* c) {
  *s = sin(x);
  *c = cos(x);
}
__device__ __forceinline__ void sincos_small(double x, double* s, double* c) { sincos_t(x, s, c); }
__device__ __forceinline__ float fmax_t(float a, float b) { return __builtin_fmaxf(a, b); }
__device__ __forceinline__ double fmax_t(double a, double b) { return __builtin_fmax(a, b); }
__device__ __forceinline__ float fmin_t(float a, float b) { return __builtin_fminf(a, b); }
__device__ __forceinline__ double fmin_t(double a, double b) { return __builtin_fmin(a, b); }
__device__ __forceinline__ float sqrt_t(float x) { return __builtin_amdgcn_sqrtf(x); }
__device__ __forceinline__ double sqrt_t(double x) { return sqrt(x); }
__device__ __forceinline__ float rcp_t(float b) { return __builtin_amdgcn_rcpf(b); }
__device__ __forceinline__ float div_t(float a, float b) { return a * __builtin_amdgcn_rcpf(b); }
__device__ __forceinline__ double div_t(double a, double b) { return a / b; }
__device__ __forceinline__ void persp(float p0, float p1, float p2, float* u, float* v) {
  const float r = rcp_t(p2);
  *u = p0 * r;
  *v = p1 * r;
}
__device__ __forceinline__ void persp(double p0, double p1, double p2, double* u, double* v) {
  *u = p0 / p2;
  *v = p1 / p2;
}
template <typename T>
__device__ __forceinline__ T inf_t() {
  return (T)INFINITY;
}

template <typename T>
__device__ __forceinline__ void stage_consts_from(const uint32_t* src, LdsConst<T>& sc) {
  static_assert(offsetof(FrameArgsT<T>, cur) == 0 && offsetof(FrameArgsT<T>, hi) == offsetof(LdsConst<T>, hi) &&
                    offsetof(FrameArgsT<T>, rgs) == offsetof(LdsConst<T>, rgs),
                "LdsConst must mirror the head of FrameArgsT");
  static_assert(sizeof(LdsConst<T>) % 4 == 0, "dword copy");
  uint32_t* dst = (uint32_t*)&sc;
  constexpr int kWordsC = (int)(sizeof(LdsConst<T>) / 4);
  for (int i = threadIdx.x; i < kWordsC; i += kBlock) dst[i] = src[i];
}
template <typename T>
__device__ __forceinline__ void stage_consts(const FrameArgsT<T>& fa, LdsConst<T>& sc) {
  (void)fa;
  stage_consts_from<T>((const uint32_t*)__builtin_amdgcn_kernarg_segment_ptr(), sc);
}

template <typename T>
__host__ __device__ __forceinline__ void compose(const T* A, const T* B, T* C) {
#pragma unroll
  for (int i = 0; i < 3; ++i) {
#pragma unroll
    for (int j = 0; j < 4; ++j) {
      T s = A[i * 4 + 0] * B[0 * 4 + j];
      s = fmadd(A[i * 4 + 1], B[1 * 4 + j], s);
      s = fmadd(A[i * 4 + 2], B[2 * 4 + j], s);
      if (j == 3) s = s + A[i * 4 + 3];
      C[i * 4 + j] = s;
    }
  }
}

typedef float f32x2 __attribute__((ext_vector_type(2)));
typedef uint32_t u32x4_t __attribute__((ext_vector_type(4)));

template <typename T, typename SP>
struct StateIO {
  static __host__ __device__ __forceinline__ T load(SP v, T) { return (T)v; }
  static __host__ __device__ __forceinline__ SP store(T v, T) { return (SP)v; }
};
template <>
struct StateIO<float, __half> {
  static __device__ __forceinline__ float load(__half v, float anchor) { return __half2float(v) + anchor; }
  static __device__ __forceinline__ __half store(float v, float anchor) { return __float2half(v - anchor); }
};

template <typename SP>
struct BufPlanes : std::false_type {};
template <>
struct BufPlanes<float> : std::true_type {};
template <>
struct BufPlanes<__half> : std::true_type {};

template <typename SP>
__device__ __forceinline__ __amdgpu_buffer_rsrc_t plane_rsrc(const SP* base, int64_t ld) {
  const uint32_t bytes = (uint32_t)(12 * ld * (int64_t)sizeof(SP));
  return __builtin_amdgcn_make_buffer_rsrc((void*)base, (short)0, (int)bytes, 0x00020000);
}
template <typename SP, int POL = 0>
__device__ __forceinline__ SP buf_ld(__amdgpu_buffer_rsrc_t r, uint32_t voff, uint32_t soff) {
  if constexpr (std::is_same<SP, float>::value)
    return __uint_as_float(__builtin_amdgcn_raw_buffer_load_b32(r, voff, soff, POL));
  else
    return __ushort_as_half(__builtin_amdgcn_raw_buffer_load_b16(r, voff, soff, POL));
}
constexpr int kPolSc1 = 16;
template <int POL = 0>
__device__ __forceinline__ void buf_st(float v, __amdgpu_buffer_rsrc_t r, uint32_t voff, uint32_t soff) {
  __builtin_amdgcn_raw_buffer_store_b32(__float_as_uint(v), r, voff, soff, POL);
}
template <int POL = 0>
__device__ __forceinline__ void buf_st(__half v, __amdgpu_buffer_rsrc_t r, uint32_t voff, uint32_t soff) {
  __builtin_amdgcn_raw_buffer_store_b16(__half_as_ushort(v), r, voff, soff, POL);
}

#ifndef PFMPE_F16_PAIRS
#define PFMPE_F16_PAIRS 1
#endif
template <typename SP>
__host__ __device__ __forceinline__ constexpr bool f16_pairs() {
  return std::is_same<SP, __half>::value && PFMPE_F16_PAIRS != 0;
}
template <typename SP>
__host__ __device__ __forceinline__ int64_t plane_index(int q, int64_t n, int64_t ld) {
  if constexpr (f16_pairs<SP>())
    return (int64_t)(q >> 1) * 2 * ld + 2 * n + (q & 1);
  else
    return (int64_t)q * ld + n;
}

template <typename SP, int POL = 0>
__device__ __forceinline__ void load_state_raw(const SP* __restrict__ base, int64_t ld, int n, SP* v) {
  if constexpr (f16_pairs<SP>()) {
    const __amdgpu_buffer_rsrc_t r = plane_rsrc(base, ld);
    const uint32_t pps = (uint32_t)(ld * 4);
#pragma unroll
    for (int p = 0; p < 6; ++p) {
      const uint32_t w = __builtin_amdgcn_raw_buffer_load_b32(r, (uint32_t)n * 4u, (uint32_t)p * pps, POL);
      v[2 * p] = __ushort_as_half((unsigned short)(w & 0xffffu));
      v[2 * p + 1] = __ushort_as_half((unsigned short)(w >> 16));
    }
  } else if constexpr (BufPlanes<SP>::value) {
    const __amdgpu_buffer_rsrc_t r = plane_rsrc(base, ld);
    const uint32_t ps = (uint32_t)(ld * (int64_t)sizeof(SP));
#pragma unroll
    for (int q = 0; q < 12; ++q) v[q] = buf_ld<SP, POL>(r, (uint32_t)n * (uint32_t)sizeof(SP), (uint32_t)q * ps);
  } else if constexpr (POL != 0) {
#pragma unroll
    for (int q = 0; q < 12; ++q)
      v[q] = __hip_atomic_load((const __attribute__((address_space(1))) SP*)(base + (int64_t)q * ld + n),
                               __ATOMIC_RELAXED, __HIP_MEMORY_SCOPE_AGENT);
  } else {
#pragma unroll
    for (int q = 0; q < 12; ++q) v[q] = base[(int64_t)q * ld + n];
  }
}
template <typename SP>
__device__ __forceinline__ void store_state_raw(SP* __restrict__ base, int64_t ld, int k, const SP* v) {
  constexpr int pol = 0;
  if constexpr (f16_pairs<SP>()) {
    const __amdgpu_buffer_rsrc_t r = plane_rsrc((const SP*)base, ld);
    const uint32_t pps = (uint32_t)(ld * 4);
#pragma unroll
    for (int p = 0; p < 6; ++p) {
      const uint32_t w = (uint32_t)__half_as_ushort(v[2 * p]) | ((uint32_t)__half_as_ushort(v[2 * p + 1]) << 16);
      __builtin_amdgcn_raw_buffer_store_b32(w, r, (uint32_t)k * 4u, (uint32_t)p * pps, pol);
    }
  } else if constexpr (BufPlanes<SP>::value) {
    const __amdgpu_buffer_rsrc_t r = plane_rsrc((const SP*)base, ld);
    const uint32_t ps = (uint32_t)(ld * (int64_t)sizeof(SP));
#pragma unroll
    for (int q = 0; q < 12; ++q) buf_st<pol>(v[q], r, (uint32_t)k * (uint32_t)sizeof(SP), (uint32_t)q * ps);
  } else {
#pragma unroll
    for (int q = 0; q < 12; ++q) base[(int64_t)q * ld + k] = v[q];
  }
}

__device__ __forceinline__ void store_state_words_f16(__half* __restrict__ base, int64_t ld, int k, const uint32_t* w) {
  const __amdgpu_buffer_rsrc_t r = plane_rsrc((const __half*)base, ld);
  if constexpr (f16_pairs<__half>()) {
    const uint32_t pps = (uint32_t)(ld * 4);
#pragma unroll
    for (int j = 0; j < 6; ++j) __builtin_amdgcn_raw_buffer_store_b32(w[j], r, (uint32_t)k * 4u, (uint32_t)j * pps, 0);
    return;
  }
  const uint32_t ps = (uint32_t)(ld * (int64_t)sizeof(__half));
  const uint32_t voff = (uint32_t)k * 2u;
#pragma unroll
  for (int j = 0; j < 6; ++j) {
    __builtin_amdgcn_raw_buffer_store_b16((uint16_t)w[j], r, voff, (uint32_t)(2 * j) * ps, 0);
    asm volatile("s_nop 4\n\tbuffer_store_short_d16_hi %0, %1, %2, %3 offen" ::"v"(w[j]), "v"(voff), "s"(r),
                 "s"((uint32_t)(2 * j + 1) * ps)
                 : "memory");
  }
}

typedef unsigned short u16x2 __attribute__((ext_vector_type(2)));
template <typename SP>
struct RawState {
  SP v[12];
};
template <>
struct RawState<__half> {
  u16x2 p[6];
};
template <>
struct RawState<float> {
  uint32_t v[12];
};
__device__ __forceinline__ int in_planes(int n, int N) { return (int)min((unsigned)n, (unsigned)(N - 1)); }
template <typename SP>
__device__ __forceinline__ void load_state_prefetch(const SP* __restrict__ base, int64_t ld, int n, bool want,
                                                    RawState<SP>& R) {
  if constexpr (BufPlanes<SP>::value) {
    const __amdgpu_buffer_rsrc_t r = plane_rsrc(base, ld);
    const uint32_t ps = (uint32_t)(ld * (int64_t)sizeof(SP));
    if constexpr (f16_pairs<SP>()) {
#pragma unroll
      for (int k = 0; k < 6; ++k)
        R.p[k] = __builtin_bit_cast(u16x2, __builtin_amdgcn_raw_buffer_load_b32(r, (uint32_t)n * 4u, (uint32_t)k * (uint32_t)(ld * 4), 0));
    } else if constexpr (sizeof(SP) == 2) {
#pragma unroll
      for (int k = 0; k < 6; ++k) {
        u16x2 x = R.p[k];
        x.x = __builtin_amdgcn_raw_buffer_load_b16(r, (uint32_t)n * 2u, (uint32_t)(2 * k) * ps, 0);
        x.y = __builtin_amdgcn_raw_buffer_load_b16(r, (uint32_t)n * 2u, (uint32_t)(2 * k + 1) * ps, 0);
        R.p[k] = x;
      }
    } else {
#pragma unroll
      for (int q = 0; q < 12; ++q) R.v[q] = __builtin_amdgcn_raw_buffer_load_b32(r, (uint32_t)n * 4u, (uint32_t)q * ps, 0);
    }
  } else {
    if (want) load_state_raw<SP>(base, ld, n, R.v);
  }
}
template <typename T, typename SP>
__device__ __forceinline__ T state_from_raw(const RawState<SP>& R, int q, T anchor) {
  if constexpr (std::is_same<SP, __half>::value)
    return StateIO<T, SP>::load(__ushort_as_half((q & 1) ? R.p[q >> 1].y : R.p[q >> 1].x), anchor);
  else if constexpr (std::is_same<SP, float>::value)
    return StateIO<T, SP>::load(__uint_as_float(R.v[q]), anchor);
  else
    return StateIO<T, SP>::load(R.v[q], anchor);
}

template <typename T>
__device__ __forceinline__ int prior_row(const FrameArgsT<T>& fa, int n) {
  return fa.owner ? (int)fa.owner[n] : n;
}
template <typename T, typename SP, int POL = 0>
__device__ __forceinline__ void load_prior(const FrameArgsT<T>& fa, const SP* __restrict__ prior, int n, T* A) {
  SP v[12];
  load_state_raw<SP, POL>(prior, fa.ld, prior_row(fa, n), v);
#pragma unroll
  for (int q = 0; q < 12; ++q) A[q] = StateIO<T, SP>::load(v[q], fa.anc_in[q]);
}
template <typename T, typename SP>
__device__ __forceinline__ void store_pose(SP* __restrict__ dst, int64_t ld, int k, const T* P, const T* anc) {
  if constexpr (std::is_same<SP, __half>::value && std::is_same<T, float>::value) {
    typedef _Float16 f16x2 __attribute__((ext_vector_type(2)));
    uint32_t w[6];
#pragma unroll
    for (int j = 0; j < 6; ++j) {
      const f32x2 d = f32x2{P[2 * j], P[2 * j + 1]} - f32x2{anc[2 * j], anc[2 * j + 1]};
      w[j] = __builtin_bit_cast(uint32_t, __builtin_convertvector(d, f16x2));
    }
    store_state_words_f16(dst, ld, k, w);
    return;
  }
  SP v[12];
#pragma unroll
  for (int q = 0; q < 12; ++q) v[q] = StateIO<T, SP>::store(P[q], anc[q]);
  store_state_raw<SP>(dst, ld, k, v);
}

template <typename T>
__device__ __forceinline__ T u21_t(uint32_t v);
template <>
__device__ __forceinline__ float u21_t<float>(uint32_t v) { return u21f(v); }
template <>
__device__ __forceinline__ double u21_t<double>(uint32_t v) { return u21d(v); }

template <typename T, int RNG>
__device__ __forceinline__ void propagate(const FrameArgsT<T>& fa, const LdsConst<T>& sc, const T* A_in, int n,
                                          int iter, T* P) {
  if (n == 0) {
#pragma unroll
    for (int q = 0; q < 12; ++q) P[q] = sc.cur[q];
    return;
  }
  if (n == 1) {
#pragma unroll
    for (int q = 0; q < 12; ++q) P[q] = sc.pred[q];
    return;
  }
  T A[12];
#pragma unroll
  for (int q = 0; q < 12; ++q) A[q] = A_in[q];
  if (fa.it > 1) {
    if (!fa.cam_identity) {
      T X[12];
      compose(sc.cam, A, X);
#pragma unroll
      for (int q = 0; q < 12; ++q) A[q] = X[q];
    }
    if ((iter % 10) != 0) {
      T X[12];
      compose(A, sc.predm, X);
#pragma unroll
      for (int q = 0; q < 12; ++q) A[q] = X[q];
    }
  }
  const double gd = 1.0 + fa.growth * (double)(iter / 10);
  T d[6];
  if (RNG == kRngReference) {
    const uint64_t before = 12u * ((uint64_t)(fa.N - 2) * (uint64_t)iter + (uint64_t)(n - 2));
    uint32_t g = lcg_output(fa.lcg_x0, before + 1u);
#pragma unroll
    for (int q = 0; q < 6; ++q) {
      const uint32_t g1 = g;
      const uint32_t g2 = lcg_next(g1);
      g = lcg_next(g2);
      d[q] = (T)(ref_uniform(ref_canonical(g1, g2), fa.dlo[q], fa.dhi[q]) * gd);
    }
  } else {
    const Draws6 r = philox_motion6((uint32_t)n, (uint32_t)iter, fa.flo, fa.fhi, fa.key0, fa.key1);
#pragma unroll
    for (int q = 0; q < 6; ++q) d[q] = (T)r.v[q] * sc.rgs[q] + sc.lo[q];
    if (iter >= 10) {
      asm volatile("");
      const T g = (T)gd;
#pragma unroll
      for (int q = 0; q < 6; ++q) d[q] = d[q] * g;
    }
  }
  T sa, ca, sb, cb, sz, cz;
  if (fa.small_angles) {
    sincos_small(d[0], &sa, &ca);
    sincos_small(d[1], &sb, &cb);
    sincos_small(d[2], &sz, &cz);
  } else {
    sincos_t(d[0], &sa, &ca);
    sincos_t(d[1], &sb, &cb);
    sincos_t(d[2], &sz, &cz);
  }
#pragma unroll
  for (int i = 0; i < 3; ++i) {
    const T a0 = A[i * 4 + 0], a1 = A[i * 4 + 1], a2 = A[i * 4 + 2];
    const T z0 = fmadd(a1, sz, a0 * cz);
    const T z1 = fmadd(a1, cz, a0 * (-sz));
    const T y0 = fmadd(a2, (-sb), z0 * cb);
    const T y2 = fmadd(a2, cb, z0 * sb);
    const T x1 = fmadd(y2, sa, z1 * ca);
    const T x2 = fmadd(y2, ca, z1 * (-sa));
    P[i * 4 + 0] = y0;
    P[i * 4 + 1] = x1;
    P[i * 4 + 2] = x2;
    P[i * 4 + 3] = A[i * 4 + 3] + d[3 + i];
  }
}

template <typename T, int RNG, typename SP>
__device__ __forceinline__ void make_particle(const FrameArgsT<T>& fa, const LdsConst<T>& sc,
                                              const SP* __restrict__ prior, int n, int iter, T* P) {
  T A[12];
  if (n >= 2) load_prior(fa, prior, n, A);
  propagate<T, RNG>(fa, sc, A, n, iter, P);
}

__device__ __forceinline__ int mad24(int a, int b, int c) {
  return (int)(((unsigned)a & 0xffffffu) * ((unsigned)b & 0xffffffu)) + c;
}
__device__ __forceinline__ f32x2 pk_fma(f32x2 a, f32x2 b, f32x2 c) { return __builtin_elementwise_fma(a, b, c); }
__device__ __forceinline__ f32x2 pk2(float a, float b) { return f32x2{a, b}; }

}
```

### pf_monocular_pose_estimator_amd/csrc/pf_types.hpp

```cpp
#pragma once
#include <hip/hip_runtime.h>
#include <stddef.h>
#include <stdint.h>

namespace pfmpe {

constexpr int kBlock = 256;
constexpr int kWaves = kBlock / 64;
constexpr int kGroup = 64;
constexpr int kMaxMarkers = 16;
constexpr int kMaxBlobs = 1024;
constexpr int kMaxBuckets = 512;
constexpr int kMaxIter = 4096;
constexpr int kPlanes = 12;

enum : int { kRngReference = 0, kRngPhilox = 1 };

constexpr int kExactM = 5;
template <int MAXM>
__host__ __device__ __forceinline__ bool marker_live(int j, int M) {
  return MAXM == kExactM ? j < kExactM : j < M;
}

struct alignas(16) GridEnt {
  float x, y;
  int32_t orig, pad;
};
struct GridArgs {
  float inv_c, ox, oy, pad0;
  float fmaxx, fmaxy;
  int32_t ncx4, on;
  int32_t cell_off, ent_off;
  int32_t b0fin;
  int32_t pad2;
};

template <typename T>
struct FrameArgsT {
  T cur[12], pred[12], predm[12], cam[12];
  T markers[kMaxMarkers * 3];
  T K[9];
  T lo[6], hi[6];
  T rgs[6];
  double dlo[6], dhi[6];
  double growth;
  T tol, tol_pf, tolq;
  double exit_thr, accept_thr;
  uint32_t key0, key1, flo, fhi;
  uint32_t lcg_x0;
  uint32_t downgrade;
  int32_t N, M, B, it;
  int32_t cam_identity, max_iter, force_iters, nblk;
  int32_t ngrp, gsz;
  int32_t diag;
  int32_t small_angles;
  int32_t k_upper;
  uint32_t wait_ticks;
  uint32_t flat_base_w, flat_base_c;
  int32_t tbytes;
  uint32_t gtag;
  GridArgs grid;
  int64_t ld;
  T anc_in[12], anc_out[12];
  const uint32_t* owner;
  uint32_t* owner_out;
};

template <typename T>
struct LdsConst {
  T cur[12], pred[12], predm[12], cam[12];
  T markers[kMaxMarkers * 3];
  T K[9];
  T lo[6], hi[6];
  T rgs[6];
};

struct Ctrl {
  double best_max;
  double S;
  double invS;
  int32_t done, has_best, best_idx, best_iter, best_slot, cur_slot;
  int32_t iters, kept_slot, kept_iter, accepted, most_likely_idx, pad0;
  int64_t K_total;
};

struct alignas(16) BlockPart {
  double sum;
  double maxrel, minrel;
  double maxw, minw;
  int32_t argmax, argmin;
};
struct alignas(16) GroupPart {
  double sum;
  double zmax, zmin;
  double maxw, minw;
  int32_t argmax, argmin;
};
struct alignas(16) BlockScan {
  double E, zin_max, zin_min, pad;
};
struct alignas(16) GroupScan {
  double G, Gin;
};
struct alignas(8) CountPart {
  int32_t maxcount, idx;
};
constexpr int kWinShards = 64;
constexpr int kWinStride = 16;
constexpr size_t kWinBytes = (size_t)(2 * kWinShards) * kWinStride * sizeof(unsigned long long);
__host__ __device__ __forceinline__ uint32_t* win_arrive(unsigned long long* winkey) {
  return (uint32_t*)(winkey + kWinShards * kWinStride);
}
constexpr int kArriveStride = 2 * kWinStride;
__host__ __device__ __forceinline__ unsigned long long win_key(int count, int idx) {
  return ((unsigned long long)(uint32_t)count << 32) | (uint32_t)(0x7fffffff - idx);
}

struct OutDev {
  int32_t iters, kept_iter, most_likely_idx, accepted, resampled, winner_idx, n_corr, flag_fail;
  double highest_prob, prob_sum;
  double winner_pose[12], most_likely_pose[12];
  uint32_t corr[2 * kMaxMarkers];
  int32_t kept_slot;
  int32_t tag;
};
constexpr int kRecWords = (int)(offsetof(OutDev, tag) / 4);
constexpr int kRecGran = 128;
static_assert(offsetof(OutDev, tag) % 4 == 0 && kRecWords <= kRecGran && kRecWords > 64, "record granules");
struct RecOut {
  uint64_t g[kRecGran];
};

constexpr int kStamps = 32;
enum : int {
  kDiagStamps = 4,
  kDiagVisits = 8,
  kDiagTreeCount = 16,
  kDiagSqrtGroups = 32,
  kDiagLagLoads = 64,
  kDiagAbandon = 128,
  kDiagSortedScore = 256,
  kDiagNoStream = 512,
  kDiagForceStream = 1024,
  kDiagSerialTop = 2048,
  kDiagNoPk = 4096,
  kDiagCorruptDesc = 8192,
  kDiagNoDefer = 16384,
  kDiagMinSide = 65536,
  kDiagAbandonFinish = 131072,
  kDiagBlockResample = 32768,
  kDiagAssocDirect = 262144,
  kDiagDetCopy = 524288,
  kDiagTailMiss = 1 << 20
};

constexpr int kShards = 8;
constexpr int kShardStride = 32;
constexpr int kFlatCountSet = kShards * kShardStride;
constexpr int kFlatWords = 2 * kShards * kShardStride;
constexpr int kFlatMaxGroups = 8;

constexpr size_t kGranPartBytes = (size_t)kFlatMaxGroups * kGroup * sizeof(BlockPart);
constexpr size_t kGranCountOff = 2 * kGranPartBytes;
constexpr size_t kGranBytes = kGranCountOff + (size_t)kFlatMaxGroups * kGroup * 16;

__host__ __device__ constexpr size_t align16(size_t x) { return (x + 15) / 16 * 16; }
struct GridHdr {
  float inv_c, gx0, gy0, pad0;
  float fmaxx, fmaxy;
  float gtolq;
  int32_t ncx, ncell, nent;
  int32_t b0fin, pad;
};
static_assert(sizeof(GridHdr) == 48, "grid header");

constexpr int kCandGran = 57;
struct alignas(16) Cand {
  uint64_t g[64];
};

struct AssocArgs {
  const double* dense;
  uint32_t* votes;
  uint32_t* corr;
  int32_t* n_corr;
  int32_t first, count;
  int32_t lds_votes;
  int32_t pad;
};
constexpr int kAssocMaxBlocks = 1024;
constexpr size_t kAssocLdsLimit = 64 * 1024;
__host__ __device__ inline int assoc_bins(int M, int B) { return M * B + M + 1; }

}
```

### pf_monocular_pose_estimator_amd/csrc/pfmpe_ctx.hpp

```cpp
#pragma once
#include <hip/hip_runtime.h>
#include <hip/hip_ext.h>

#include <hip/hip_fp16.h>

#include <time.h>

#include <algorithm>
#include <atomic>
#include <cmath>
#include <cstdio>
#include <cstddef>
#include <cstring>
#include <string>
#include <map>
#include <memory>
#include <optional>
#include <type_traits>
#include <vector>

#include "../../include/pfmpe.h"
#include "pf_types.hpp"

using namespace pfmpe;

static_assert(offsetof(OutDev, kept_slot) == sizeof(pfmpe_frame_out), "OutDev must start with pfmpe_frame_out");
static_assert(offsetof(OutDev, corr) == offsetof(pfmpe_frame_out, corr), "OutDev layout");
static_assert(offsetof(OutDev, prob_sum) == offsetof(pfmpe_frame_out, prob_sum), "OutDev layout");
static_assert(PFMPE_MAX_MARKERS == kMaxMarkers, "marker capacity mismatch");
static_assert(PFMPE_MAX_BLOBS == kMaxBlobs, "blob capacity mismatch");

struct EventPair {
  hipEvent_t a, b;
  int kid;
};

struct BatchFence {
  hipEvent_t ev = nullptr;
  hipStream_t stream = nullptr;
  bool recorded = false;
  ~BatchFence() {
    if (ev) (void)hipEventDestroy(ev);
  }
};

enum class Mem { Device, Pinned, Mapped };
inline std::atomic<int64_t>& live_blocks() {
  static std::atomic<int64_t> n{0};
  return n;
}
template <typename T, Mem K = Mem::Device>
class Buf {
 public:
  Buf() = default;
  Buf(const Buf&) = delete;
  Buf& operator=(const Buf&) = delete;
  Buf(Buf&& o) noexcept { swap(o); }
  Buf& operator=(Buf&& o) noexcept {
    Buf t(std::move(o));
    swap(t);
    return *this;
  }
  ~Buf() { reset(); }
  void swap(Buf& o) noexcept {
    std::swap(p_, o.p_);
    std::swap(dev_, o.dev_);
    std::swap(cap_, o.cap_);
  }
  T* get() const { return p_; }
  T* dev() const { return dev_; }
  size_t bytes() const { return cap_; }
  explicit operator bool() const { return p_ != nullptr; }
  int alloc(pfmpe_ctx* c, size_t bytes);
  int ensure(pfmpe_ctx* c, size_t bytes) { return p_ ? PFMPE_OK : alloc(c, bytes); }
  int grow(pfmpe_ctx* c, size_t need, size_t capacity);
  void reset() {
    if (p_) {
      (void)(K == Mem::Device ? hipFree((void*)p_) : hipHostFree((void*)p_));
      live_blocks() -= 1;
    }
    p_ = dev_ = nullptr;
    cap_ = 0;
  }

 private:
  T* p_ = nullptr;
  T* dev_ = nullptr;
  size_t cap_ = 0;
};

struct CtxQueue {
  hipStream_t stream = nullptr;
  std::vector<EventPair> ev_pool;
  hipEvent_t own_ev = nullptr;
  CtxQueue() = default;
  CtxQueue(const CtxQueue&) = delete;
  CtxQueue& operator=(const CtxQueue&) = delete;
  ~CtxQueue() {
    for (auto& e : ev_pool) {
      (void)hipEventDestroy(e.a);
      (void)hipEventDestroy(e.b);
    }
    if (own_ev) (void)hipEventDestroy(own_ev);
    if (stream) (void)hipStreamDestroy(stream);
  }
};

struct pfmpe_ctx : CtxQueue {
  int device = 0;
  int max_particles = 0, max_markers = 0, max_blobs = 0, state_dtype = PFMPE_STATE_F32;
  size_t es = 4;
  size_t ws = 4;
  double anchor[2][12] = {{0}};
  int64_t ld = 0;
  int max_blk = 0;

  Buf<void> d_state[2];
  int prior_idx = 0;
  Buf<void> d_w[2];
  Buf<void> d_prop[2];
  Buf<uint32_t> d_owner[2];
  int prior_owner = -1;
  int frame_owner_out = -1;
  bool defer = true;
  int max_grp = 0;
  Buf<BlockPart> d_part[2];
  Buf<BlockScan> d_bscan[2];
  Buf<GroupPart> d_gpart[2];
  Buf<GroupScan> d_gscan;
  Buf<CountPart> d_cpart;
  Buf<unsigned long long> d_winkey;
  Buf<CountPart> d_cgroup;
  Buf<uint32_t> d_counters;
  Buf<uint32_t> d_gen;
  Buf<Cand> d_cand;
  Buf<double> d_mlpose;
  Buf<uint32_t> d_pairs;
  Buf<unsigned char> d_refine;
  Buf<unsigned char> d_top;
  Buf<unsigned char, Mem::Pinned> h_top;
  Buf<unsigned char> d_refm;
  Buf<unsigned char, Mem::Pinned> h_refm;
  Buf<unsigned char, Mem::Mapped> h_tail;
  int tail_S = 0;
  int32_t tail_seq0 = 0;
  int64_t tail_fallbacks = 0;
  Buf<unsigned char> d_init;
  Buf<unsigned char, Mem::Pinned> h_init;
  Buf<unsigned char> d_det;
  Buf<uint8_t> d_img;
  int img_w = 0, img_h = 0, img_pitch = 0;
  Buf<void, Mem::Mapped> h_det;
  Buf<unsigned char> d_detm;
  Buf<unsigned char, Mem::Mapped> h_detm;
  Buf<void, Mem::Mapped> h_detm_out;
  Buf<uint8_t, Mem::Mapped> h_detm_pix;
  Buf<unsigned char> d_roim;
  Buf<unsigned char, Mem::Mapped> h_roim;
  Buf<unsigned char> d_cloudm;
  Buf<unsigned char, Mem::Mapped> h_cloudm;
  Buf<unsigned char> d_modes;
  Buf<unsigned char, Mem::Pinned> h_modes;
  Buf<unsigned char> d_assocm;
  Buf<unsigned char, Mem::Pinned> h_assocm;
  int num_cu = 0;
  bool coop = false;
  int fused = 2;
  Buf<uint32_t> d_flat;
  Buf<unsigned char> d_gran;
  uint32_t gframe = 0;
  uint32_t flat_base_w = 0, flat_base_c = 0;
  int64_t fused_fallbacks = 0;
  int fused_user = 2;
  int64_t fused_rearm = 0;
  int64_t clean_since_fallback = 0;
  int64_t wait_bound_us = 2000000;
  int64_t multi_max_blocks = 160000;
  int last_shape = -1;
  int last_weigh_pass = -1;
  int last_resample = -1;
  int64_t guard_skips = 0;
  std::map<std::pair<const void*, size_t>, int> occ;
  int64_t mt_enter = 0, mt_ns[4] = {0, 0, 0, 0}, mt_batches = 0;
  Buf<Ctrl> d_ctrl;
  Buf<RecOut, Mem::Mapped> h_rec;
  std::unique_ptr<OutDev> h_out;
  int32_t seq = 0;
  Buf<unsigned char> d_table;
  Buf<unsigned char, Mem::Pinned> h_table;
  Buf<unsigned char> d_bank;
  std::vector<size_t> bank_off;
  std::vector<int32_t> bank_B;
  std::vector<GridHdr> bank_grid;
  std::vector<double> bank_blobs;
  std::vector<int32_t> bank_offsets;
  double bank_tol_pf = 0.0;
  int last_grid = -1;
  Buf<double> d_xfer;
  Buf<uint32_t> d_counts;
  Buf<uint64_t> d_stamps;
  Buf<unsigned char> d_multi;
  Buf<unsigned char, Mem::Mapped> h_multi;
  hipEvent_t br_a = nullptr, br_b = nullptr;
  uint32_t multi_gen = 0;
  std::vector<int64_t> map_sig;
  hipStream_t last_stream = nullptr;
  std::shared_ptr<BatchFence> last_fence;
  std::shared_ptr<BatchFence> lead_fence;

  int M = 0;
  double markers[kMaxMarkers * 3] = {0};
  double K[9] = {0};
  uint32_t downgrade = 0;
  bool has_model = false;
  pfmpe_params params{};
  int N = 0;
  bool has_prior = false;

  bool record_counts = false;
  bool prune = true;
  bool keep_prop = true;
  int timing = 0;
  bool timing_now = false;
  int64_t timing_frame = 0;
  int diag = 0;

  FrameArgsT<float> last_fa_f{};
  FrameArgsT<double> last_fa_d{};
  bool has_last = false;
  int last_prior_idx = 0;
  bool last_accepted = false;
  int last_kept_slot = 0, last_kept_iter = 0;

  size_t ev_used = 0;
  int64_t k_launches[PFMPE_K_COUNT] = {0};
  double k_ms[PFMPE_K_COUNT] = {0};

  std::string err;
};

namespace pfmpe_impl {

constexpr int kMaxDevices = 64;
inline std::atomic<int>& fused_inflight(int dev) {
  static std::atomic<int> flags[kMaxDevices];
  return flags[(dev >= 0 && dev < kMaxDevices) ? dev : 0];
}

inline int fail(pfmpe_ctx* c, int code, const std::string& msg) {
  if (c) c->err = msg;
  return code;
}

#define HIPCHK(ctx, expr)                                                                       \
  do {                                                                                          \
    hipError_t e_ = (expr);                                                                     \
    if (e_ != hipSuccess)                                                                       \
      return fail((ctx), PFMPE_E_HIP, std::string(#expr) + ": " + hipGetErrorString(e_));       \
  } while (0)

#define RET(expr)              \
  do {                         \
    int r_ = (expr);           \
    if (r_ != PFMPE_OK) return r_; \
  } while (0)

}

template <typename T, Mem K>
int Buf<T, K>::alloc(pfmpe_ctx* c, size_t bytes) {
  reset();
  void* p = nullptr;
  const hipError_t e = K == Mem::Device   ? hipMalloc(&p, bytes)
                       : K == Mem::Pinned ? hipHostMalloc(&p, bytes, hipHostMallocDefault)
                                          : hipHostMalloc(&p, bytes, hipHostMallocMapped | hipHostMallocCoherent);
  if (e != hipSuccess)
    return pfmpe_impl::fail(c, PFMPE_E_HIP, "allocating " + std::to_string(bytes) + " bytes: " + hipGetErrorString(e));
  live_blocks() += 1;
  p_ = (T*)p;
  cap_ = bytes;
  if (K == Mem::Mapped) {
    void* d = nullptr;
    if (const hipError_t g = hipHostGetDevicePointer(&d, p, 0); g != hipSuccess) {
      reset();
      return pfmpe_impl::fail(c, PFMPE_E_HIP, std::string("hipHostGetDevicePointer: ") + hipGetErrorString(g));
    }
    dev_ = (T*)d;
  }
  return PFMPE_OK;
}
template <typename T, Mem K>
int Buf<T, K>::grow(pfmpe_ctx* c, size_t need, size_t capacity) {
  if (need <= cap_) return PFMPE_OK;
  if (p_)
    if (const hipError_t e = hipStreamSynchronize(c->stream); e != hipSuccess)
      return pfmpe_impl::fail(c, PFMPE_E_HIP, std::string("hipStreamSynchronize: ") + hipGetErrorString(e));
  return alloc(c, capacity);
}

template <typename T_, typename SP_, int RNG_ = 0>
struct StateTag {
  using T = T_;
  using SP = SP_;
  static constexpr int RNG = RNG_;
};
template <typename F>
auto visit_state(const pfmpe_ctx* c, F&& f) {
  switch (c->state_dtype) {
    case PFMPE_STATE_F64: return f(StateTag<double, double>{});
    case PFMPE_STATE_F16: return f(StateTag<float, __half>{});
    default: return f(StateTag<float, float>{});
  }
}
template <typename F>
auto visit_state_rng(const pfmpe_ctx* c, F&& f) {
  return visit_state(c, [&](auto s) {
    using S = decltype(s);
    return c->params.rng_mode == PFMPE_RNG_REFERENCE ? f(StateTag<typename S::T, typename S::SP, kRngReference>{})
                                                     : f(StateTag<typename S::T, typename S::SP, kRngPhilox>{});
  });
}
template <typename F>
auto visit_m(int M, bool exact5, F&& f) {
  if (exact5) return f(std::integral_constant<int, kExactM>{});
  if (M <= 8) return f(std::integral_constant<int, 8>{});
  if (M <= 12) return f(std::integral_constant<int, 12>{});
  return f(std::integral_constant<int, 16>{});
}

namespace pfmpe_impl {

inline int order_after(pfmpe_ctx* c, hipStream_t to, pfmpe_ctx* err) {
  if (!c->last_stream || c->last_stream == to) return PFMPE_OK;
  if (c->last_fence) {
    if (c->last_fence->stream) {
      if (!c->last_fence->recorded) {
        HIPCHK(err, hipEventRecord(c->last_fence->ev, c->last_fence->stream));
        c->last_fence->recorded = true;
      }
      HIPCHK(err, hipStreamWaitEvent(to, c->last_fence->ev, 0));
    }
  } else {
    if (!c->own_ev) HIPCHK(err, hipEventCreateWithFlags(&c->own_ev, hipEventDisableTiming));
    HIPCHK(err, hipEventRecord(c->own_ev, c->last_stream));
    HIPCHK(err, hipStreamWaitEvent(to, c->own_ev, 0));
  }
  c->last_stream = nullptr;
  c->last_fence.reset();
  return PFMPE_OK;
}

inline int seal_lead_fence(pfmpe_ctx* c) {
  BatchFence* f = c->lead_fence.get();
  if (!f || f->recorded || c->lead_fence.use_count() < 2) return PFMPE_OK;
  HIPCHK(c, hipEventRecord(f->ev, c->stream));
  f->recorded = true;
  return PFMPE_OK;
}

inline int set_device(pfmpe_ctx* c) {
  HIPCHK(c, hipSetDevice(c->device));
  if (const int r_ = seal_lead_fence(c)) return r_;
  if (const int r_ = order_after(c, c->stream, c)) return r_;
  c->last_stream = c->stream;
  return PFMPE_OK;
}

inline int open_bracket(pfmpe_ctx* c, int kid, EventPair** out) {
  *out = nullptr;
  if (!c->timing_now) return PFMPE_OK;
  if (c->ev_used == c->ev_pool.size()) {
    EventPair p{};
    p.kid = kid;
    HIPCHK(c, hipEventCreate(&p.a));
    HIPCHK(c, hipEventCreate(&p.b));
    c->ev_pool.push_back(p);
  }
  *out = &c->ev_pool[c->ev_used++];
  (*out)->kid = kid;
  return PFMPE_OK;
}
template <typename Launch>
int launch_ext(pfmpe_ctx* c, int kid, Launch&& fn) {
  EventPair* ep = nullptr;
  if (const int r_ = open_bracket(c, kid, &ep)) return r_;
  if (ep) {
    c->br_a = ep->a;
    c->br_b = ep->b;
  }
  fn();
  c->br_a = c->br_b = nullptr;
  HIPCHK(c, hipGetLastError());
  return PFMPE_OK;
}
template <typename Launch>
int launch(pfmpe_ctx* c, int kid, Launch&& fn) {
  EventPair* ep = nullptr;
  if (const int r_ = open_bracket(c, kid, &ep)) return r_;
  if (ep) HIPCHK(c, hipEventRecord(ep->a, c->stream));
  fn();
  HIPCHK(c, hipGetLastError());
  if (ep) HIPCHK(c, hipEventRecord(ep->b, c->stream));
  return PFMPE_OK;
}
template <typename... KArgs, typename... Args>
inline void klaunch(pfmpe_ctx* c, void (*kernel)(KArgs...), dim3 grid, dim3 block, size_t lds, Args... args) {
  if (c->br_b) {
    hipExtLaunchKernelGGL(kernel, grid, block, (uint32_t)lds, c->stream, c->br_a, c->br_b, 0u, args...);
    c->br_a = nullptr;
  } else {
    hipLaunchKernelGGL(kernel, grid, block, lds, c->stream, args...);
  }
}

template <typename F>
int timed(pfmpe_ctx* c, F&& fn) {
  const size_t ev_mark = c->ev_used;
  c->timing_now = c->timing > 0;
  const int rc = fn();
  c->timing_now = false;
  if (rc != PFMPE_OK && c->ev_used > ev_mark) c->ev_used = ev_mark;
  return rc;
}

constexpr size_t kHarvestPairs = 256;
constexpr size_t kEventPrealloc = 64;
inline int harvest_timing(pfmpe_ctx* c) {
  if (c->ev_used == 0) return PFMPE_OK;
  HIPCHK(c, hipEventSynchronize(c->ev_pool[c->ev_used - 1].b));
  for (size_t i = 0; i < c->ev_used; ++i) {
    float ms = 0.f;
    HIPCHK(c, hipEventElapsedTime(&ms, c->ev_pool[i].a, c->ev_pool[i].b));
    c->k_launches[c->ev_pool[i].kid] += 1;
    c->k_ms[c->ev_pool[i].kid] += ms;
  }
  c->ev_used = 0;
  return PFMPE_OK;
}

inline bool take_record(pfmpe_ctx* c, int32_t want) {
  volatile const uint64_t* g = c->h_rec.get()->g;
  const uint32_t t = (uint32_t)(g[0] >> 32);
  if ((int32_t)(t >> 1) != want) return false;
  if (t & 1u) {
    for (int k = kRecWords - 1; k > 0; --k)
      if ((uint32_t)(g[k] >> 32) != t) return false;
    __atomic_thread_fence(__ATOMIC_ACQUIRE);
    uint32_t* w = (uint32_t*)c->h_out.get();
    for (int k = 0; k < kRecWords; ++k) w[k] = (uint32_t)g[k];
  }
  c->h_out->tag = (int32_t)t;
  return true;
}
constexpr int64_t kQueryAfterNs = 200000;
inline int64_t now_ns() {
  timespec ts;
  clock_gettime(CLOCK_MONOTONIC, &ts);
  return (int64_t)ts.tv_sec * 1000000000ll + ts.tv_nsec;
}
inline int wait_frame(pfmpe_ctx* c, hipStream_t on = nullptr) {
  const int32_t want = c->seq;
  int64_t next_query = 0;
  for (uint64_t spin = 0;; ++spin) {
    if (take_record(c, want)) return PFMPE_OK;
    if ((spin & 63u) != 63u) {
      __builtin_ia32_pause();
      continue;
    }
    const int64_t t = now_ns();
    if (next_query == 0) next_query = t + kQueryAfterNs;
    if (t >= next_query) {
      next_query = t + kQueryAfterNs;
      const hipError_t q = hipStreamQuery(on ? on : c->stream);
      if (q == hipSuccess) {
        if (take_record(c, want)) return PFMPE_OK;
        return fail(c, PFMPE_E_HIP, "frame record was not written");
      }
      if (q != hipErrorNotReady) return fail(c, PFMPE_E_HIP, std::string("stream error: ") + hipGetErrorString(q));
    }
    __builtin_ia32_pause();
  }
// ... 178 lines not shown
```

### pf_monocular_pose_estimator_amd/csrc/pfmpe_engine.hip

```cpp
#include "pf_gn.hpp"
#include "pf_likelihood.hpp"
#include "pf_tail.hpp"
#include "pfmpe_prior.hpp"

using namespace pfmpe_impl;

PFMPE_DECLARE_INSTANCE(float, kRngReference, float, extern)
PFMPE_DECLARE_INSTANCE(float, kRngPhilox, float, extern)
PFMPE_DECLARE_INSTANCE(double, kRngReference, double, extern)
PFMPE_DECLARE_INSTANCE(double, kRngPhilox, double, extern)
PFMPE_DECLARE_INSTANCE(float, kRngReference, __half, extern)
PFMPE_DECLARE_INSTANCE(float, kRngPhilox, __half, extern)

namespace pfmpe_impl {

int dispatch_regen(pfmpe_ctx* c, int kept_iter, const void* prior, double* out) {
  return visit_state_rng(c, [&](auto s) {
    using S = decltype(s);
    return regen_m<typename S::T, S::RNG, typename S::SP>(c, kept_iter, prior, out);
  });
}

int dispatch_regen_list(pfmpe_ctx* c, int kept_iter, const void* prior, const int32_t* list, const uint32_t* count,
                        int limit, double* out) {
// ... 461 lines not shown
  RET(set_device(c));
  RET(ensure_xfer(c));
  const int N = c->N;
  if (which == 0)
    RET(dispatch_regen(c, c->last_kept_iter, c->d_state[c->last_prior_idx].get(), c->d_xfer.get()));
  else
    RET(export_prior(c, N));
  HIPCHK(c, hipMemcpyAsync(out, c->d_xfer.get(), (size_t)N * 12 * sizeof(double), hipMemcpyDeviceToHost, c->stream));
  HIPCHK(c, hipStreamSynchronize(c->stream));
  RET(harvest_timing(c));
  return PFMPE_OK;
}

int pfmpe_get_weights(pfmpe_ctx* c, double* out) {
  if (!c) return PFMPE_E_ARG;
  if (!out) return fail(c, PFMPE_E_ARG, "get_weights: null out");
  if (!c->has_last) return fail(c, PFMPE_E_STATE, "get_weights: no step yet");
  RET(set_device(c));
  RET(ensure_xfer(c));
  const int N = c->N;
  visit_state(c, [&](auto s) {
    using T = typename decltype(s)::T;
    hipLaunchKernelGGL((k_weights_export<T>), dim3((N + 255) / 256), dim3(256), 0, c->stream,
                       (const T*)c->d_w[c->last_kept_slot].get(), c->d_xfer.get(), N);
  });
  HIPCHK(c, hipGetLastError());
  HIPCHK(c, hipMemcpyAsync(out, c->d_xfer.get(), (size_t)N * sizeof(double), hipMemcpyDeviceToHost, c->stream));
  HIPCHK(c, hipStreamSynchronize(c->stream));
  return PFMPE_OK;
}

int pfmpe_get_counts(pfmpe_ctx* c, uint32_t* out) {
  if (!c) return PFMPE_E_ARG;
  if (!out) return fail(c, PFMPE_E_ARG, "get_counts: null out");
  if (!c->record_counts || !c->d_counts.get()) return fail(c, PFMPE_E_STATE, "get_counts: PFMPE_OPT_RECORD_COUNTS off");
  if (!c->has_last || !c->last_accepted) return fail(c, PFMPE_E_STATE, "get_counts: last step did not resample");
  RET(set_device(c));
  HIPCHK(c, hipMemcpyAsync(out, c->d_counts.get(), (size_t)c->N * sizeof(uint32_t), hipMemcpyDeviceToHost, c->stream));
  HIPCHK(c, hipStreamSynchronize(c->stream));
  return PFMPE_OK;
}

namespace {
void tail_summary(const pfmpe_refine_row& r, const double* cov, pfmpe_refine_out* o) {
  std::memset(o, 0, sizeof(*o));
  o->n = 1;
  o->n_with_pairs = r.n_pairs > 0 ? 1 : 0;
  o->n_converged = r.status == PFMPE_REFINE_CONVERGED ? 1 : 0;
  o->n_cap_kept = r.status == PFMPE_REFINE_CAP_KEPT ? 1 : 0;
  o->n_cap_reverted = r.status == PFMPE_REFINE_CAP_REVERTED ? 1 : 0;
  o->iters_total = r.iters;
  o->iters_max = r.iters;
  o->best = -1;
  if (gn_eligible(r)) {
    o->best = 0;
    o->best_row = r;
    std::memcpy(o->best_cov, cov, sizeof(o->best_cov));
  }
}
void tail_empty(pfmpe_refine_out* o) {
  std::memset(o, 0, sizeof(*o));
  o->best = -1;
}

struct TailLayout {
  size_t rec_off, in_off;
  static size_t align(size_t x) { return (x + 255) / 256 * 256; }
  explicit TailLayout(int S) : rec_off(align((size_t)S * sizeof(TailDesc))), in_off(rec_off + (size_t)S * sizeof(TailRec)) {}
  static size_t stream_bytes(int B) { return align(kTailModelBytes + 2 * (size_t)B * sizeof(double)); }
};
struct TailStream {
  const pfmpe_ctx* c;
  const double* blobs;
  int B;
  pfmpe_refine_params prm;
};
void tail_blobs(const pfmpe_ctx* c, const pfmpe_frame_in* in, TailStream* st) {
  st->c = c;
  st->B = in->B;
  st->blobs = in->bank_frame >= 0 ? c->bank_blobs.data() + 2 * (size_t)c->bank_offsets[in->bank_frame] : in->blobs;
}
int tail_stage(pfmpe_ctx* c0, const std::vector<TailStream>& st) {
  const int S = (int)st.size();
  const TailLayout L(S);
  size_t need = L.in_off;
  for (const TailStream& t : st) need += TailLayout::stream_bytes(t.B);
  if (need > UINT32_MAX) return fail(c0, PFMPE_E_CAP, "step_refine: the staging block exceeds 4 GiB");
  RET(c0->h_tail.grow(c0, need, need + need / 2));
  unsigned char* h = c0->h_tail.get();
  unsigned char* d = c0->h_tail.dev();
  std::memset(h + L.rec_off, 0, (size_t)S * sizeof(TailRec));
  size_t off = L.in_off;
  for (int s = 0; s < S; ++s) {
    const pfmpe_ctx* c = st[s].c;
    TailDesc x{};
    x.rec = ((const RecOut*)c->h_rec.dev())->g;
    x.out = ((TailRec*)(d + L.rec_off) + s)->g;
    x.model_off = (uint32_t)off;
    x.blobs_off = (uint32_t)(off + kTailModelBytes);
    x.seq0 = c->seq;
    x.M = c->M;
    x.B = st[s].B;
    x.max_iter = st[s].prm.max_iter;
    x.revert = st[s].prm.revert_on_divergence ? 1 : 0;
    x.converged = st[s].prm.converged;
    std::memcpy(h + (size_t)s * sizeof(TailDesc), &x, sizeof(x));
    std::memcpy(h + off, c->markers, sizeof(c->markers));
    std::memcpy(h + off + sizeof(c->markers), c->K, sizeof(c->K));
    if (st[s].B > 0) std::memcpy(h + x.blobs_off, st[s].blobs, 2 * (size_t)st[s].B * sizeof(double));
    off += TailLayout::stream_bytes(st[s].B);
  }
  __atomic_thread_fence(__ATOMIC_RELEASE);
  return PFMPE_OK;
}
static_assert(sizeof(((pfmpe_ctx*)nullptr)->markers) + sizeof(((pfmpe_ctx*)nullptr)->K) <= kTailModelBytes, "tail model");

uint32_t tail_wait(pfmpe_ctx* c0, int S, int s, int32_t want, pfmpe_refine_row* row, double* cov) {
  volatile const uint64_t* g = ((const TailRec*)(c0->h_tail.get() + TailLayout(S).rec_off) + s)->g;
  auto take = [&](uint32_t* state) {
    const uint32_t t = (uint32_t)(g[0] >> 32);
    if (t == 0u || (int32_t)(t >> 2) != want) return false;
    *state = t & 3u;
    if (*state != kTailRefined) return true;
    for (int k = kTailWords - 1; k > 0; --k)
      if ((uint32_t)(g[k] >> 32) != t) return false;
    __atomic_thread_fence(__ATOMIC_ACQUIRE);
    uint32_t w[kTailWords];
    for (int k = 0; k < kTailWords; ++k) w[k] = (uint32_t)g[k];
    std::memcpy(row, w + 1, sizeof(*row));
    std::memcpy(cov, w + 1 + kTailRowWords, 36 * sizeof(double));
    return true;
  };
  uint32_t state = kTailNotReady;
  int64_t next_query = 0;
  for (uint64_t spin = 0;; ++spin) {
    if (take(&state)) return state;
    if ((spin & 63u) != 63u) {
      __builtin_ia32_pause();
      continue;
    }
    const int64_t t = now_ns();
    if (next_query == 0) next_query = t + kQueryAfterNs;
    if (t >= next_query) {
      next_query = t + kQueryAfterNs;
      if (hipStreamQuery(c0->stream) != hipErrorNotReady) return take(&state) ? state : (uint32_t)kTailNotReady;
    }
    __builtin_ia32_pause();
  }
}

int tail_collect(pfmpe_ctx* c0, int S, int s, pfmpe_ctx* c, const TailStream& st, const pfmpe_frame_out* out,
                 pfmpe_refine_out* gn, pfmpe_refine_row* row, double* cov36) {
  pfmpe_refine_row r;
  double cov[36];
  const uint32_t state = tail_wait(c0, S, s, c->seq, &r, cov);
  if (state == kTailRefined) {
    tail_summary(r, cov, gn);
    if (row) *row = r;
    if (cov36) std::memcpy(cov36, cov, sizeof(cov));
    return PFMPE_OK;
  }
  if (state == kTailEmpty) {
    tail_empty(gn);
    return PFMPE_OK;
  }
  c->tail_fallbacks += 1;
  if (!tail_wanted(out->flag_fail, out->winner_pose)) {
    tail_empty(gn);
    return PFMPE_OK;
  }
  pfmpe_assoc_in ain{};
  ain.blobs = st.blobs;
  ain.B = st.B;
  ain.bank_frame = -1;
  return pfmpe_refine_poses(c, &ain, &st.prm, out->winner_pose, out->corr, 1, gn, row, cov36);
}
struct TailScope {
  pfmpe_ctx* c;
  TailScope(pfmpe_ctx* c_, int S) : c(c_) {
    c->tail_S = S;
    c->tail_seq0 = c->seq;
  }
  ~TailScope() { c->tail_S = 0; }
};
}

int pfmpe_step_refine(pfmpe_ctx* c, const pfmpe_frame_in* in, const pfmpe_refine_params* params, pfmpe_frame_out* out,
                      pfmpe_refine_out* gn, pfmpe_refine_row* row, double* cov36) {
  RET(check_step(c, in, out));
  std::vector<TailStream> st(1);
  pfmpe_default_refine_params(&st[0].prm);
  if (params) st[0].prm = *params;
  if (!gn) return fail(c, PFMPE_E_ARG, "step_refine: null gn");
  if (!refine_params_ok(st[0].prm)) return fail(c, PFMPE_E_ARG, "step_refine: bad parameters");
  tail_blobs(c, in, &st[0]);
  HIPCHK(c, hipSetDevice(c->device));
  RET(tail_stage(c, st));
  {
    TailScope scope(c, 1);
    RET(step_run(c, in, out));
  }
  return tail_collect(c, 1, 0, c, st[0], out, gn, row, cov36);
}

int pfmpe_step_refine_multi(pfmpe_ctx* const* ctxs, int S, const pfmpe_frame_in* in, const pfmpe_refine_params* params,
                            pfmpe_frame_out* out, pfmpe_refine_out* gn, pfmpe_refine_row* rows, double* cov) {
  RET(step_multi_check(ctxs, S, in, out, "step_refine_multi"));
  pfmpe_ctx* c0 = ctxs[0];
  if (!gn) return fail(c0, PFMPE_E_ARG, "step_refine_multi: null gn");
  std::vector<TailStream> st(S);
  for (int s = 0; s < S; ++s) {
    pfmpe_default_refine_params(&st[s].prm);
    if (params) st[s].prm = params[s];
    if (!refine_params_ok(st[s].prm))
      return fail(c0, PFMPE_E_ARG, "step_refine_multi: stream " + std::to_string(s) + ": bad parameters");
    tail_blobs(ctxs[s], &in[s], &st[s]);
  }
  HIPCHK(c0, hipSetDevice(c0->device));
  RET(tail_stage(c0, st));
  {
    TailScope scope(c0, S);
    RET(step_multi_run(ctxs, S, in, out));
  }
  for (int s = 0; s < S; ++s)
    RET(tail_collect(c0, S, s, ctxs[s], st[s], &out[s], &gn[s], rows ? rows + s : nullptr,
                     cov ? cov + 36 * (size_t)s : nullptr));
  return PFMPE_OK;
}

int pfmpe_host_step_tail(const double* markers_xyz, int M, const double* K, const double* blobs, int B,
                         const pfmpe_frame_out* frame, const pfmpe_refine_params* params, pfmpe_refine_out* gn,
                         pfmpe_refine_row* row, double* cov36) {
  pfmpe_refine_params prm;
  pfmpe_default_refine_params(&prm);
  if (params) prm = *params;
  if (!markers_xyz || !K || !frame || !gn || M < 1 || M > kMaxMarkers || B < 0 || (B > 0 && !blobs)) return PFMPE_E_ARG;
  if (!refine_params_ok(prm)) return PFMPE_E_ARG;
  if (!tail_wanted(frame->flag_fail, frame->winner_pose)) {
    tail_empty(gn);
    return PFMPE_OK;
  }
  double model[kMaxMarkers * 3] = {0}, zb[2 * kMaxMarkers] = {0}, c36[36];
  uint32_t lcorr[2 * kMaxMarkers];
  std::memcpy(model, markers_xyz, (size_t)M * 3 * sizeof(double));
  for (int j = 0; j < kMaxMarkers; ++j) {
    if (!tail_pair(frame->corr, j, M, B, lcorr + 2 * j)) return PFMPE_E_ARG;
    if (lcorr[2 * j + 1] != 0u) {
      zb[2 * j] = blobs[2 * (size_t)(frame->corr[2 * j + 1] - 1u)];
      zb[2 * j + 1] = blobs[2 * (size_t)(frame->corr[2 * j + 1] - 1u) + 1];
    }
  }
  pfmpe_refine_row r;
  tail_refine(model, K, zb, lcorr, prm.max_iter, prm.revert_on_divergence ? 1 : 0, prm.converged, frame->winner_pose, r,
              c36);
  tail_summary(r, c36, gn);
  if (row) *row = r;
  if (cov36) std::memcpy(cov36, c36, sizeof(c36));
  return PFMPE_OK;
}

int pfmpe_debug_stamps(pfmpe_ctx* c, uint64_t* out) {
  if (!c || !c->d_stamps) return PFMPE_E_STATE;
  RET(set_device(c));
  hipStream_t st = c->stream;
  const size_t rows = 1 + (size_t)c->max_blk;
  if (!out) {
    HIPCHK(c, hipMemsetAsync(c->d_stamps.get(), 0, rows * kStamps * sizeof(uint64_t), st));
    HIPCHK(c, hipStreamSynchronize(st));
    return PFMPE_OK;
  }
  std::vector<uint64_t> h(rows * kStamps);
  HIPCHK(c, hipMemcpyAsync(h.data(), c->d_stamps.get(), h.size() * sizeof(uint64_t), hipMemcpyDeviceToHost, st));
  HIPCHK(c, hipStreamSynchronize(st));
  for (int i = 0; i < kStamps; ++i) {
    const bool is_min = i == 0 || i == 4 || i == 19;
    uint64_t v = h[i];
    for (size_t r = 1; r < rows; ++r) {
      const uint64_t x = h[r * kStamps + i];
      if (!x) continue;
      if (!v || (is_min ? x < v : x > v)) v = x;
    }
    out[i] = v;
  }
  return PFMPE_OK;
}

int pfmpe_get_kernel_stats(pfmpe_ctx* c, int kernel, int64_t* launches, double* total_ms) {
  if (!c || kernel < 0 || kernel >= PFMPE_K_COUNT) return PFMPE_E_ARG;
  if (c->ev_used) {
    HIPCHK(c, hipSetDevice(c->device));
    RET(harvest_timing(c));
  }
  if (launches) *launches = c->k_launches[kernel];
  if (total_ms) *total_ms = c->k_ms[kernel];
  return PFMPE_OK;
}

int pfmpe_get_info(const pfmpe_ctx* c, int key, int64_t* value) {
  if (!c || !value) return PFMPE_E_ARG;
  switch (key) {
    case PFMPE_INFO_FUSED: *value = c->fused; return PFMPE_OK;
    case PFMPE_INFO_FUSED_FALLBACKS: *value = c->fused_fallbacks; return PFMPE_OK;
    case PFMPE_INFO_LAST_SHAPE: *value = c->last_shape; return PFMPE_OK;
    case PFMPE_INFO_LAST_WEIGH_PASS: *value = c->last_weigh_pass; return PFMPE_OK;
    case PFMPE_INFO_LAST_RESAMPLE: *value = c->last_resample; return PFMPE_OK;
    case PFMPE_INFO_LAST_GRID: *value = c->last_grid; return PFMPE_OK;
    case PFMPE_INFO_GUARD_SKIPS: *value = c->guard_skips; return PFMPE_OK;
    case PFMPE_INFO_N: *value = c->N; return PFMPE_OK;
    case PFMPE_INFO_NUM_CU: *value = c->num_cu; return PFMPE_OK;
    case PFMPE_INFO_TAIL_FALLBACKS: *value = c->tail_fallbacks; return PFMPE_OK;
    case 110: case 111: case 112: case 113: *value = c->mt_ns[key - 110]; return PFMPE_OK;
    case 114: *value = c->mt_batches; return PFMPE_OK;
    case 115: *value = live_blocks().load(); return PFMPE_OK;
    default: return PFMPE_E_ARG;
  }
}

int pfmpe_reset_kernel_stats(pfmpe_ctx* c) {
  if (!c) return PFMPE_E_ARG;
  if (c->ev_used) {
    HIPCHK(c, hipSetDevice(c->device));
    HIPCHK(c, hipEventSynchronize(c->ev_pool[c->ev_used - 1].b));
    c->ev_used = 0;
  }
  for (int k = 0; k < PFMPE_K_COUNT; ++k) {
    c->k_launches[k] = 0;
    c->k_ms[k] = 0;
  }
  return PFMPE_OK;
}

const char* pfmpe_kernel_name(int kernel) {
  static const char* names[PFMPE_K_COUNT] = {"k_propagate_weigh", "k_resample", "aux", "k_frame", "k_roi",
                                                 "k_resample_final", "k_p3p_hist", "k_p3p_check",
                                                 "k_det (detector pipeline)"};
  return (kernel >= 0 && kernel < PFMPE_K_COUNT) ? names[kernel] : "?";
}

double pfmpe_host_ref_uniform(uint32_t seed, uint64_t j, double a, double b) {
  const uint32_t x0 = lcg_seed(seed);
  const uint32_t g1 = lcg_output(x0, 2 * j + 1);
  const uint32_t g2 = lcg_next(g1);
  return ref_uniform(ref_canonical(g1, g2), a, b);
}

void pfmpe_host_philox(const uint32_t ctr[4], const uint32_t key[2], uint32_t out[4]) {
  const U32x4 o = philox4x32_10(ctr[0], ctr[1], ctr[2], ctr[3], key[0], key[1]);
  out[0] = o.x;
  out[1] = o.y;
  out[2] = o.z;
  out[3] = o.w;
}

}
```

### pf_monocular_pose_estimator_amd/csrc/pfmpe_seq.hpp

```cpp
#pragma once
#include "pf_kernels.hpp"
#include "pf_weigh_pk.hpp"
#include "pfmpe_args.hpp"

namespace pfmpe_impl {

struct BatchLayout {
  size_t doff, boff, soff, need;
};
template <typename Desc>
inline BatchLayout batch_layout(int na, int64_t total, size_t tbytes) {
  BatchLayout L;
  L.doff = tbytes;
  L.boff = L.doff + ((size_t)na * sizeof(Desc) + 255) / 256 * 256;
  L.soff = L.boff + ((size_t)total * sizeof(uint16_t) + 255) / 256 * 256;
  L.need = L.soff + (size_t)na * sizeof(uint32_t) + 256;
  return L;
}

template <typename T, int RNG, int MAXM, typename SP>
constexpr int kPkMarkers = (std::is_same<T, float>::value && RNG == kRngPhilox && (MAXM == kExactM || MAXM == kPk12M) &&
                            (std::is_same<SP, float>::value || std::is_same<SP, __half>::value))
                               ? MAXM
                               : 0;
inline bool pk_eligible(const FrameArgsT<float>& fa, int markers) {
  return fa.grid.on && fa.grid.b0fin && fa.small_angles && fa.cam_identity && fa.k_upper && fa.M == markers &&
         fa.B >= fa.M && !(fa.diag & (kDiagNoPk | kDiagSortedScore));
}
template <typename T, int RNG, int MAXM, typename SP>
constexpr auto pk_kernel() {
  if constexpr (kPkMarkers<T, RNG, MAXM, SP> == kExactM)
    return &k_weigh_pk<SP>;
  else if constexpr (kPkMarkers<T, RNG, MAXM, SP> == kPk12M)
    return &k_weigh_pk12<SP>;
  else
    return nullptr;
}

inline int occupancy(pfmpe_ctx* c, const void* fn, size_t lds, int at_least, int* blocks) {
  const auto key = std::make_pair(fn, lds);
  auto it = c->occ.find(key);
  if (it == c->occ.end()) {
    int per_cu = 0;
    HIPCHK(c, hipOccupancyMaxActiveBlocksPerMultiprocessor(&per_cu, fn, kBlock, lds));
    it = c->occ.emplace(key, std::max(at_least, per_cu)).first;
  }
  *blocks = it->second;
  return PFMPE_OK;
}

struct Counters {
  uint32_t *gcount_w, *tcount_w, *gcount_r, *tcount_r;
};
inline Counters counters(const pfmpe_ctx* c) {
  uint32_t* p = c->d_counters.get();
  return {p, p + c->max_grp, p + c->max_grp + 1, p + 2 * c->max_grp + 1};
}

inline int32_t next_seq(pfmpe_ctx* c) { return c->seq = (c->seq + 1) & 0x3fffffff; }

inline bool may_defer(const pfmpe_ctx* c) {
  return c->defer && c->d_owner[0].get() && c->d_owner[1].get() && !(c->diag & kDiagNoDefer);
}
inline uint32_t* defer_frame(pfmpe_ctx* c, bool kept) {
  c->frame_owner_out = -1;
  if (!kept || !may_defer(c)) return nullptr;
  c->frame_owner_out = c->prior_owner == 0 ? 1 : 0;
  return c->d_owner[c->frame_owner_out].get();
}

inline int reset_handoffs(pfmpe_ctx* c, hipStream_t on, bool flat = false) {
  HIPCHK(c, hipStreamSynchronize(on));
  HIPCHK(c, hipMemsetAsync(c->d_ctrl.get(), 0, sizeof(Ctrl), c->stream));
  HIPCHK(c, hipMemsetAsync(c->d_counters.get(), 0, counters_bytes(c), c->stream));
  HIPCHK(c, hipMemsetAsync(c->d_winkey.get(), 0, kWinBytes, c->stream));
  if (flat && c->d_flat.get()) HIPCHK(c, hipMemsetAsync(c->d_flat.get(), 0, kFlatWords * sizeof(uint32_t), c->stream));
  HIPCHK(c, hipStreamSynchronize(c->stream));
  return PFMPE_OK;
}

inline int abandoned(pfmpe_ctx* c) {
  RET(reset_handoffs(c, c->stream, true));
  c->flat_base_w = c->flat_base_c = 0;
  c->fused_fallbacks += 1;
  c->fused = 0;
  c->clean_since_fallback = 0;
  c->err = "one-launch frame abandoned at the wait bound (blocks not co-resident: other work on the device?); "
           "redone with two launches, one-launch frames off" +
           std::string(c->fused_rearm > 0 ? " until PFMPE_OPT_FUSED_REARM clean frames" : "");
  return PFMPE_OK;
}
constexpr uint32_t kGranFrames = 0xFFFFF;
inline int next_gtag(pfmpe_ctx* c, uint32_t* gtag) {
  if (c->gframe >= kGranFrames) {
    HIPCHK(c, hipMemsetAsync(c->d_gran.get(), 0, kGranBytes, c->stream));
    c->gframe = 0;
  }
  c->gframe += 1;
  *gtag = c->gframe << 12;
  return PFMPE_OK;
}
inline BlockPart* gran_part(const pfmpe_ctx* c, int parity) {
  return (BlockPart*)(c->d_gran.get() + (size_t)parity * kGranPartBytes);
}
inline CountPart* gran_count(const pfmpe_ctx* c) { return (CountPart*)(c->d_gran.get() + kGranCountOff); }

template <typename T, int RNG, int MAXM, typename SP>
struct Seq {
  static constexpr int kPkM = kPkMarkers<T, RNG, MAXM, SP>;
  static int iterate(pfmpe_ctx* c, const FrameArgsT<T>& fa, const unsigned char* table, int iter) {
    const SP* prior = (const SP*)c->d_state[c->prior_idx].get();
    const size_t lds = BlobTable<T>::lds_bytes(fa.tbytes);
    const Counters n = counters(c);
    RET(ensure_prop(c));
    SP* prop0 = c->keep_prop ? (SP*)c->d_prop[0].get() : nullptr;
    SP* prop1 = c->keep_prop ? (SP*)c->d_prop[1].get() : nullptr;
    T* w0 = (T*)c->d_w[0].get();
    T* w1 = (T*)c->d_w[1].get();
    const bool stream = !(c->diag & kDiagNoStream);
    bool pk = false;
    if constexpr (kPkM != 0) pk = stream && c->prune && pk_eligible(fa, kPkM);
    c->last_weigh_pass = pk ? PFMPE_WEIGH_PK : (stream ? PFMPE_WEIGH_STREAM : PFMPE_WEIGH_BLOCKS);
    if (stream) {
      auto k = c->prune ? k_weigh_stream<T, RNG, MAXM, true, SP> : k_weigh_stream<T, RNG, MAXM, false, SP>;
      int per_cu = 0;
      RET(occupancy(c, pk ? (const void*)pk_kernel<T, RNG, MAXM, SP>() : (const void*)k, lds, 1, &per_cu));
      const int grid = std::min(pk ? (fa.nblk + 1) / 2 : fa.nblk, per_cu * std::max(1, c->num_cu));
      RET(launch_ext(c, PFMPE_K_PROPAGATE, [&] {
        if constexpr (kPkM != 0) {
          if (pk) {
            klaunch(c, pk_kernel<T, RNG, MAXM, SP>(), dim3(grid), dim3(kBlock), lds, fa, table, prior, w0, w1,
                    c->d_part[0].get(), c->d_part[1].get(), (const Ctrl*)c->d_ctrl.get(), prop0, prop1, iter);
            return;
          }
        }
        klaunch(c, k, dim3(grid), dim3(kBlock), lds, fa, table, prior, w0, w1, c->d_part[0].get(), c->d_part[1].get(),
                c->d_ctrl.get(), prop0, prop1, iter);
      }));
      const size_t glds = fa.ngrp > 64 ? (size_t)fa.ngrp * sizeof(GroupPart) : 0;
      const bool staged = glds > 0 && glds <= 64 * 1024;
      if (fa.ngrp <= 64 && !(c->diag & kDiagSerialTop))
        return launch_ext(c, PFMPE_K_AUX, [&] {
          klaunch(c, k_group_top<T, RNG>, dim3(fa.ngrp), dim3(64), 0, fa, c->d_part[0].get(), c->d_part[1].get(), c->d_bscan[0].get(),
                  c->d_bscan[1].get(), c->d_gpart[0].get(), c->d_gpart[1].get(), c->d_gscan.get(), c->d_ctrl.get(), n.tcount_w, iter);
        });
      return launch_ext(c, PFMPE_K_AUX, [&] {
        klaunch(c, k_group<T>, dim3(fa.ngrp), dim3(64), 0, fa, c->d_part[0].get(), c->d_part[1].get(),
                           c->d_bscan[0].get(), c->d_bscan[1].get(), c->d_gpart[0].get(), c->d_gpart[1].get(), (const Ctrl*)c->d_ctrl.get());
        if (staged && fa.ngrp <= 64 * kTopMaxTiles && !(c->diag & kDiagSerialTop))
          klaunch(c, k_top_wide<T, RNG>, dim3(1), dim3(64 * kTopWaves), glds, fa, c->d_gpart[0].get(), c->d_gpart[1].get(),
                  c->d_gscan.get(), c->d_ctrl.get(), iter);
        else
          klaunch(c, k_top<T, RNG>, dim3(1), dim3(64), staged ? glds : 0, fa, c->d_gpart[0].get(),
                             c->d_gpart[1].get(), c->d_gscan.get(), c->d_ctrl.get(), iter, staged ? 1 : 0);
      });
    }
    auto k = c->prune ? k_propagate_weigh<T, RNG, MAXM, true, SP> : k_propagate_weigh<T, RNG, MAXM, false, SP>;
    return launch_ext(c, PFMPE_K_PROPAGATE, [&] {
      klaunch(c, k, dim3(fa.nblk), dim3(kBlock), lds, fa, table, prior, w0, w1, c->d_part[0].get(), c->d_part[1].get(),
              c->d_bscan[0].get(), c->d_bscan[1].get(), c->d_gpart[0].get(), c->d_gpart[1].get(), c->d_gscan.get(),
              c->d_ctrl.get(), n.gcount_w, n.tcount_w, prop0, prop1, iter, c->d_stamps.get());
    });
  }
  static int finish(pfmpe_ctx* c, const FrameArgsT<T>& fa, const unsigned char* table) {
    const SP* prior = (const SP*)c->d_state[c->prior_idx].get();
    SP* post = (SP*)c->d_state[1 - c->prior_idx].get();
    const Counters n = counters(c);
    const int32_t seq = next_seq(c);
    const bool kept = c->keep_prop && c->d_prop[0].get();
    FrameArgsT<T> far = fa;
    far.owner_out = defer_frame(c, kept);
    bool owners = false;
    RET(launch_ext(c, PFMPE_K_RESAMPLE, [&] {
      if (far.owner_out && !(c->diag & kDiagBlockResample)) {
        owners = true;
        klaunch(c, k_resample_owners<T, RNG, MAXM, SP>, dim3((unsigned)((fa.nblk + kWaves - 1) / kWaves)),
                dim3(kBlock), 0, far, c->d_ctrl.get(), prior, (const T*)c->d_w[0].get(), (const T*)c->d_w[1].get(), c->d_bscan[0].get(),
                c->d_bscan[1].get(), c->d_gscan.get(), c->record_counts ? c->d_counts.get() : nullptr, c->d_mlpose.get(), c->d_winkey.get(),
                win_arrive(c->d_winkey.get()), table, c->h_rec.dev(), seq, c->d_stamps.get());
        return;
      }
      auto k = kept ? k_resample<T, RNG, MAXM, SP, true> : k_resample<T, RNG, MAXM, SP, false>;
      klaunch(c, k, dim3(fa.nblk), dim3(kBlock), 0, far, c->d_ctrl.get(), table,
                         prior, post, (const T*)c->d_w[0].get(), (const T*)c->d_w[1].get(), c->d_bscan[0].get(), c->d_bscan[1].get(),
                         c->d_gscan.get(), c->d_cpart.get(), c->d_cgroup.get(), n.gcount_r, n.tcount_r,
                         c->record_counts ? c->d_counts.get() : nullptr, c->d_cand.get(), c->d_mlpose.get(), c->h_rec.dev(), seq,
                         c->d_stamps.get(), kept ? (const SP*)c->d_prop[0].get() : nullptr,
                         kept ? (const SP*)c->d_prop[1].get() : nullptr, c->d_winkey.get());
    }));
    c->last_resample = owners ? PFMPE_RESAMPLE_OWNERS : PFMPE_RESAMPLE_BLOCKS;
    if (!owners)
      RET(launch_ext(c, PFMPE_K_FINAL, [&] {
        klaunch(c, k_resample_final<T, RNG, MAXM, SP>, dim3(1), dim3(kFinalBlock), BlobTable<T>::bytes(fa.B), fa,
                c->d_ctrl.get(), table, prior, c->d_cpart.get(), c->d_cand.get(), c->d_mlpose.get(), c->h_rec.dev(), seq, c->d_stamps.get(), kept ? 1 : 0,
                c->d_winkey.get());
      }));
    RET(tail_after(c));
    if (const int rc = wait_frame(c); rc != PFMPE_OK) {
      const std::string err = c->err;
      (void)reset_handoffs(c, c->stream);
      return fail(c, rc, err);
    }
    return PFMPE_OK;
  }
  template <bool PRUNE>
  static int frame_fused(pfmpe_ctx* c, const FrameArgsT<T>& fa_in, const unsigned char* table, bool* launched) {
    *launched = false;
    const bool flat = c->fused == 2 && fa_in.nblk <= kFlatMaxGroups * kGroup && fa_in.gsz == kGroup && c->d_flat.get();
    const void* fn = flat ? (const void*)k_frame2<T, RNG, MAXM, PRUNE, SP> : (const void*)k_frame<T, RNG, MAXM, PRUNE, SP>;
    const size_t lds = BlobTable<T>::lds_bytes(fa_in.tbytes);
    int occ = 0;
    RET(occupancy(c, fn, lds, 0, &occ));
    const int per_cu = std::min(2, occ - 1);
    if (per_cu < 1 || (int64_t)per_cu * c->num_cu < fa_in.nblk) return PFMPE_OK;
    std::atomic<int>& busy = fused_inflight(c->device);
    int expect = 0;
    if (!busy.compare_exchange_strong(expect, 1)) {
      c->guard_skips += 1;
      return PFMPE_OK;
    }
    struct Release {
      std::atomic<int>& b;
      ~Release() { b.store(0); }
    } release{busy};
    FrameArgsT<T> a = fa_in;
    a.flat_base_w = c->flat_base_w;
    a.flat_base_c = c->flat_base_c;
    const bool tree_count = !flat && ((c->diag & kDiagTreeCount) || a.nblk > kFlatMaxGroups * kGroup);
    if (!tree_count) RET(next_gtag(c, &a.gtag));
    const SP* prior = (const SP*)c->d_state[c->prior_idx].get();
    SP* post = (SP*)c->d_state[1 - c->prior_idx].get();
    T* w0 = (T*)c->d_w[0].get();
    T* w1 = (T*)c->d_w[1].get();
    const Counters n = counters(c);
    uint32_t* counts = c->record_counts ? c->d_counts.get() : nullptr;
    const int32_t seq = next_seq(c);
    RET(launch_ext(c, PFMPE_K_FRAME, [&] {
      if (flat)
        klaunch(c, k_frame2<T, RNG, MAXM, PRUNE, SP>, dim3(a.nblk), dim3(kBlock), lds, a, table,
                           prior, post, w0, w1, gran_part(c, 0), gran_part(c, 1), c->d_ctrl.get(), gran_count(c), c->d_flat.get(),
                           counts, c->d_cand.get(), c->d_mlpose.get(), c->h_rec.dev(), seq, c->d_stamps.get());
      else
        klaunch(c, k_frame<T, RNG, MAXM, PRUNE, SP>, dim3(a.nblk), dim3(kBlock), lds, a, table,
                           prior, post, w0, w1, c->d_part[0].get(), c->d_part[1].get(), c->d_bscan[0].get(), c->d_bscan[1].get(),
                           c->d_gpart[0].get(), c->d_gpart[1].get(), c->d_gscan.get(), c->d_ctrl.get(),
                           tree_count ? c->d_cpart.get() : gran_count(c), c->d_cgroup.get(), n.gcount_w,
                           n.tcount_w, n.gcount_r, n.tcount_r, c->d_gen.get(), counts, c->d_cand.get(), c->d_mlpose.get(), c->h_rec.dev(), seq,
                           c->d_stamps.get(), tree_count ? nullptr : c->d_flat.get());
    }));
    RET(tail_after(c));
    *launched = true;
    if (wait_frame(c) != PFMPE_OK) {
      RET(abandoned(c));
      *launched = false;
      return PFMPE_OK;
    }
    if (flat || !(c->diag & kDiagTreeCount)) {
      const OutDev& o = *c->h_out;
      if (flat) c->flat_base_w += (uint32_t)o.iters * (uint32_t)a.nblk;
      if (o.resampled) c->flat_base_c += (uint32_t)a.nblk;
    }
    return PFMPE_OK;
  }

  static int step(pfmpe_ctx* c, const FrameArgsT<T>& fa, const unsigned char* table) {
    if (!c->fused && c->fused_user && c->fused_rearm > 0 && c->clean_since_fallback >= c->fused_rearm)
      c->fused = c->fused_user;
    const int64_t fallbacks0 = c->fused_fallbacks;
    if (c->fused) {
      bool launched = false;
      RET(c->prune ? frame_fused<true>(c, fa, table, &launched) : frame_fused<false>(c, fa, table, &launched));
      if (launched) {
        if (!frame_done(c)) return fail(c, PFMPE_E_STATE, "fused frame did not finish");
        c->last_shape = (c->fused == 2 && fa.nblk <= kFlatMaxGroups * kGroup && fa.gsz == kGroup) ? PFMPE_SHAPE_FRAME2
                                                                                                   : PFMPE_SHAPE_FRAME;
        last_args<T>(c) = fa;
        return PFMPE_OK;
      }
    }
    c->last_shape = PFMPE_SHAPE_TWO_LAUNCH;
    const int cap = iter_cap(fa);
    int iter = 0;
    RET(iterate(c, fa, table, iter++));
    RET(finish(c, fa, table));
    int batch = 1;
    while (!frame_done(c)) {
      if (iter >= cap) return fail(c, PFMPE_E_STATE, "PF iteration loop did not terminate");
      for (int b = 0; b < batch && iter < cap; ++b) RET(iterate(c, fa, table, iter++));
      RET(finish(c, fa, table));
      batch = std::min(batch * 2, 16);
    }
    if (!c->fused && c->fused_fallbacks == fallbacks0) c->clean_since_fallback += 1;
    last_args<T>(c) = fa;
    return PFMPE_OK;
  }
  static int batch_failure(pfmpe_ctx* c0, pfmpe_ctx* const* cs, const std::vector<int>& act,
                           const std::vector<StreamDesc<T, SP>>& want, const unsigned char* ddesc, const uint32_t* dstat,
                           uint32_t gen, const std::string& wait_err) {
    using Desc = StreamDesc<T, SP>;
    const int na = (int)act.size();
    std::vector<uint32_t> st(na, 0);
    std::vector<Desc> seen(na);
    if (hipStreamSynchronize(c0->stream) != hipSuccess ||
        hipMemcpy(st.data(), dstat, (size_t)na * sizeof(uint32_t), hipMemcpyDeviceToHost) != hipSuccess ||
        hipMemcpy((void*)seen.data(), ddesc, (size_t)na * sizeof(Desc), hipMemcpyDeviceToHost) != hipSuccess)
      return fail(c0, PFMPE_E_HIP, "step_multi: " + wait_err);
    static const std::pair<size_t, const char*> kFields[] = {
        {offsetof(Desc, table), "table"},   {offsetof(Desc, prior), "prior"},   {offsetof(Desc, post), "post"},
        {offsetof(Desc, w0), "w0"},         {offsetof(Desc, w1), "w1"},         {offsetof(Desc, part0), "part0"},
        {offsetof(Desc, part1), "part1"},   {offsetof(Desc, bscan0), "bscan0"}, {offsetof(Desc, bscan1), "bscan1"},
        {offsetof(Desc, gpart0), "gpart0"}, {offsetof(Desc, gpart1), "gpart1"}, {offsetof(Desc, gscan), "gscan"},
        {offsetof(Desc, ctrl), "ctrl"},     {offsetof(Desc, gcount_w), "gcount_w"}, {offsetof(Desc, tcount_w), "tcount_w"},
        {offsetof(Desc, gcount_r), "gcount_r"}, {offsetof(Desc, tcount_r), "tcount_r"}, {offsetof(Desc, prop0), "prop0"},
        {offsetof(Desc, prop1), "prop1"},   {offsetof(Desc, cpart), "cpart"},   {offsetof(Desc, cgroup), "cgroup"},
        {offsetof(Desc, counts), "counts"}, {offsetof(Desc, cand), "cand"},     {offsetof(Desc, mlpose), "mlpose"},
        {offsetof(Desc, out), "out"},       {offsetof(Desc, winkey), "winkey"},
        {offsetof(Desc, seq), "seq|first_blk"}, {offsetof(Desc, gen), "gen"},
        {offsetof(Desc, tag), "tag"},       {offsetof(FrameArgsT<T>, key0), "fa.key0|key1"},
        {offsetof(FrameArgsT<T>, flo), "fa.flo|fhi"}};
    auto name = [&](size_t off) -> std::string {
      for (const auto& f : kFields)
        if (f.first == off) return f.second;
      return off < sizeof(FrameArgsT<T>) ? "fa+" + std::to_string(off) : "+" + std::to_string(off);
    };
    for (int i = 0; i < na; ++i) {
      if (st[i] == gen) continue;
      std::string msg = "step_multi: stream " + std::to_string(act[i]) + ": descriptor failed the staging check (gen " +
                        std::to_string(gen) + ", status " + std::to_string(st[i]) + "); words read != written:";
      const uint64_t* a = (const uint64_t*)&want[i];
      const uint64_t* b = (const uint64_t*)&seen[i];
      int shown = 0;
      for (size_t k = 0; k < sizeof(Desc) / 8 && shown < 8; ++k)
        if (a[k] != b[k]) {
          char buf[96];
          std::snprintf(buf, sizeof buf, " %s host 0x%llx device 0x%llx;", name(8 * k).c_str(), (unsigned long long)a[k],
                        (unsigned long long)b[k]);
          msg += buf;
          ++shown;
        }
      if (!shown) msg += " none (the tag or generation check failed on words equal to the host's)";
      cs[act[i]]->err = msg;
      return fail(c0, PFMPE_E_STATE, msg);
    }
    return fail(c0, PFMPE_E_HIP, "step_multi: " + wait_err);
  }
  static int step_multi(pfmpe_ctx* const* cs, int S, const FrameArgsT<T>* fas, const unsigned char* const* tables,
                        unsigned char* h, const unsigned char* hdev, unsigned char* d, size_t tbytes) {
    using Desc = StreamDesc<T, SP>;
    pfmpe_ctx* c0 = cs[0];
    std::vector<int> act(S);
    for (int s = 0; s < S; ++s) act[s] = s;
    int iter = 0, nb = 1;
    for (int round = 0;; ++round) {
      const int na = (int)act.size();
      const BatchLayout L = batch_layout<Desc>(na, 0, tbytes);
      Desc* hd = (Desc*)(h + L.doff);
      int64_t total = 0;
      size_t lds_w = 0, lds_f = 0;
      bool all_kept = true;
      bool all_owners = true;
      if (++c0->multi_gen == 0u || c0->multi_gen == ~0u) c0->multi_gen = 1u;
      const uint32_t gen = c0->multi_gen;
      std::vector<Desc> want(na);
      auto write_desc = [&](int i) {
        Desc& x = want[i];
        x.tag = desc_tag((const uint64_t*)&x, (int)(offsetof(Desc, tag) / 8));
        std::memcpy((void*)&hd[i], (const void*)&x, sizeof(Desc));
        if (i == 0 && (c0->diag & kDiagCorruptDesc)) hd[0].fa.key0 ^= 1u;
      };
      for (int i = 0; i < na; ++i) {
        pfmpe_ctx* c = cs[act[i]];
        const FrameArgsT<T>& fa = fas[act[i]];
        Desc& x = want[i];
        std::memset((void*)&x, 0, sizeof(Desc));
        x.fa = fa;
        x.table = tables[act[i]];
        x.prior = (const SP*)c->d_state[c->prior_idx].get();
        x.post = (SP*)c->d_state[1 - c->prior_idx].get();
        x.w0 = (T*)c->d_w[0].get();
        x.w1 = (T*)c->d_w[1].get();
        x.part0 = c->d_part[0].get();
        x.part1 = c->d_part[1].get();
        x.bscan0 = c->d_bscan[0].get();
        x.bscan1 = c->d_bscan[1].get();
        x.gpart0 = c->d_gpart[0].get();
        x.gpart1 = c->d_gpart[1].get();
        x.gscan = c->d_gscan.get();
        x.ctrl = c->d_ctrl.get();
        const Counters n = counters(c);
        x.gcount_w = n.gcount_w;
        x.tcount_w = n.tcount_w;
        x.gcount_r = n.gcount_r;
        x.tcount_r = n.tcount_r;
        const bool kept = c->keep_prop && c->d_prop[0].get() && (may_defer(c) || std::is_same<SP, __half>::value);
        x.prop0 = kept ? (SP*)c->d_prop[0].get() : nullptr;
        x.prop1 = kept ? (SP*)c->d_prop[1].get() : nullptr;
        all_kept = all_kept && kept;
        x.fa.owner_out = defer_frame(c, kept);
        all_owners = all_owners && x.fa.owner_out;
        x.cpart = c->d_cpart.get();
        x.cgroup = c->d_cgroup.get();
        x.counts = c->record_counts ? c->d_counts.get() : nullptr;
        x.cand = c->d_cand.get();
        x.mlpose = c->d_mlpose.get();
        x.out = c->h_rec.dev();
        x.winkey = c->d_winkey.get();
        x.seq = next_seq(c);
        x.first_blk = (int32_t)total;
        x.gen = gen;
        write_desc(i);
        total += fa.nblk;
        lds_w = std::max(lds_w, BlobTable<T>::lds_bytes(fa.tbytes));
        lds_f = std::max(lds_f, BlobTable<T>::bytes(fa.B));
      }
      bool pk = false;
      int pk_grid_x = 0, max_ngrp = 0;
      if constexpr (kPkM == kExactM) {
        pk = c0->prune && !(c0->diag & (kDiagNoStream | kDiagNoPk));
        for (int i = 0; i < na && pk; ++i) pk = pk_eligible(fas[act[i]], kExactM);
        if (pk) {
          int per_cu = 0;
          RET(occupancy(c0, (const void*)k_weigh_pk_multi<SP>, lds_w, 1, &per_cu));
          const int64_t cap = (int64_t)per_cu * std::max(1, c0->num_cu);
          for (int i = 0; i < na; ++i) {
            const FrameArgsT<T>& fa = fas[act[i]];
            const int64_t tasks = 2 * (int64_t)fa.nblk;
            const int64_t share = std::max<int64_t>(1, cap * fa.nblk / std::max<int64_t>(1, total));
            const int wg = (int)std::max<int64_t>(1, std::min<int64_t>(share, (tasks + kWaves - 1) / kWaves));
            want[i].wg = wg;
            write_desc(i);
            pk_grid_x = std::max(pk_grid_x, wg);
            max_ngrp = std::max(max_ngrp, fa.ngrp);
          }
        }
      }
      const BatchLayout Lt = batch_layout<Desc>(na, total, tbytes);
      uint32_t* dstat = (uint32_t*)(d + Lt.soff);
      int room = 0;
      for (int i = 0; i < na; ++i) room = std::max(room, iter_cap(fas[act[i]]) - iter);
      const int nit = std::max(1, std::min(nb, room));
      const Desc* dd = (const Desc*)(d + Lt.doff);
      const uint16_t* db = (const uint16_t*)(d + Lt.boff);
      std::vector<int64_t> sig;
      sig.reserve(2 + 2 * (size_t)na);
      sig.push_back((int64_t)Lt.boff);
      sig.push_back(total);
      for (int i = 0; i < na; ++i) {
        sig.push_back(want[i].first_blk);
        sig.push_back(want[i].fa.nblk);
      }
      const bool map_kept = sig == c0->map_sig;
      c0->map_sig.swap(sig);
      const int64_t t_l0 = now_ns();
      if (round == 0) c0->mt_ns[0] += t_l0 - c0->mt_enter;
      RET(launch_ext(c0, PFMPE_K_AUX, [&] {
        klaunch(c0, k_stage_multi<T, SP>, dim3((unsigned)na), dim3(kBlock), 0, hdev, d, (uint32_t)Lt.doff,
                (uint32_t)(round == 0 ? tbytes : 0), map_kept ? kMapKept : (uint32_t)Lt.boff, dstat, gen);
      }));
      for (int k = 0; k < nit; ++k, ++iter) {
        if constexpr (kPkM == kExactM) {
          if (pk) {
            const uint32_t* cst = dstat;
            RET(launch_ext(c0, PFMPE_K_PROPAGATE, [&] {
              klaunch(c0, k_weigh_pk_multi<SP>, dim3((unsigned)pk_grid_x, (unsigned)na), dim3(kBlock), lds_w, dd, na,
                      cst, gen, iter);
            }));
            const size_t glds = (size_t)max_ngrp * sizeof(GroupPart);
            const bool wide = glds <= 64 * 1024 && max_ngrp <= 64 * kTopMaxTiles && !(c0->diag & kDiagSerialTop);
            RET(launch_ext(c0, PFMPE_K_AUX, [&] {
              if (max_ngrp <= 64 && !(c0->diag & kDiagSerialTop)) {
                klaunch(c0, k_group_top_multi<T, RNG, SP>, dim3((unsigned)max_ngrp, (unsigned)na), dim3(64), 0, dd, na,
                        cst, gen, iter);
              } else {
                klaunch(c0, k_group_multi<T, SP>, dim3((unsigned)max_ngrp, (unsigned)na), dim3(64), 0, dd, na, cst, gen);
                if (wide)
                  klaunch(c0, k_top_wide_multi<T, RNG, SP>, dim3((unsigned)na), dim3(64 * kTopWaves), glds, dd, na, cst,
                          gen, iter);
                else
                  klaunch(c0, k_top_multi<T, RNG, SP>, dim3((unsigned)na), dim3(64), 0, dd, na, cst, gen, iter);
              }
            }));
            continue;
          }
        }
        auto kw = c0->prune ? k_propagate_weigh_multi<T, RNG, MAXM, true, SP>
                            : k_propagate_weigh_multi<T, RNG, MAXM, false, SP>;
        RET(launch_ext(c0, PFMPE_K_PROPAGATE, [&] {
          klaunch(c0, kw, dim3((unsigned)total), dim3(kBlock), lds_w, dd, db, na, (const uint32_t*)dstat, gen, iter);
        }));
      }
      const bool owners = all_owners && !(c0->diag & kDiagBlockResample);
      for (int i = 0; i < na; ++i) {
        cs[act[i]]->last_weigh_pass = pk ? PFMPE_WEIGH_PK : PFMPE_WEIGH_BLOCKS;
        cs[act[i]]->last_resample = owners ? PFMPE_RESAMPLE_OWNERS : PFMPE_RESAMPLE_BLOCKS;
      }
      RET(launch_ext(c0, PFMPE_K_RESAMPLE, [&] {
        if (owners)
          klaunch(c0, k_resample_owners_multi<T, RNG, MAXM, SP>, dim3((unsigned)((total + kWaves - 1) / kWaves)),
                  dim3(kBlock), 0, dd, db, na, (const uint32_t*)dstat, gen, (int)total);
        else
          klaunch(c0, all_kept ? k_resample_multi<T, RNG, MAXM, SP, true> : k_resample_multi<T, RNG, MAXM, SP, false>,
                  dim3((unsigned)total), dim3(kBlock), 0, dd, db, na, (const uint32_t*)dstat, gen);
      }));
      if (!owners)
        RET(launch_ext(c0, PFMPE_K_FINAL, [&] {
          klaunch(c0, k_resample_final_multi<T, RNG, MAXM, SP>, dim3((unsigned)na), dim3(kFinalBlock), lds_f, dd,
                  (const uint32_t*)dstat, gen);
        }));
      if (c0->tail_S) RET(tail_launch(c0, round + 1));
      const int64_t t_l1 = now_ns();
      c0->mt_ns[1] += t_l1 - t_l0;
      std::vector<int> next;
      for (int i = 0; i < na; ++i) {
        pfmpe_ctx* c = cs[act[i]];
        if (wait_frame(c, c0->stream) != PFMPE_OK) {
          const std::string err = c->err;
          for (int k = 0; k < na; ++k) (void)reset_handoffs(cs[act[k]], c0->stream);
          return batch_failure(c0, cs, act, want, d + Lt.doff, dstat, gen, err);
        }
        if (!frame_done(c)) next.push_back(act[i]);
      }
      c0->mt_ns[2] += now_ns() - t_l1;
      if (next.empty()) break;
      for (int s : next)
        if (iter >= iter_cap(fas[s])) return fail(c0, PFMPE_E_STATE, "step_multi: PF iteration loop did not terminate");
      act.swap(next);
      nb = round == 0 ? 1 : std::min(nb * 2, 16);
    }
    for (int s = 0; s < S; ++s) {
      cs[s]->last_shape = PFMPE_SHAPE_TWO_LAUNCH;
      last_args<T>(cs[s]) = fas[s];
    }
    return PFMPE_OK;
  }
  static int regen(pfmpe_ctx* c, int kept_iter, const void* prior, double* out) {
    const FrameArgsT<T>& fa = last_args<T>(c);
    return launch_ext(c, PFMPE_K_AUX, [&] {
      klaunch(c, k_regen<T, RNG, SP>, dim3((fa.N + 255) / 256), dim3(256), 0, fa, kept_iter,
                         (const SP*)prior, out);
    });
  }
  static int regen_list(pfmpe_ctx* c, int kept_iter, const void* prior, const int32_t* list, const uint32_t* count,
                        int limit, double* out) {
    const FrameArgsT<T>& fa = last_args<T>(c);
    if (limit < 1) return PFMPE_OK;
    return launch_ext(c, PFMPE_K_AUX, [&] {
      klaunch(c, k_regen_list<T, RNG, SP>, dim3((limit + kBlock - 1) / kBlock), dim3(kBlock), 0, fa, kept_iter,
              (const SP*)prior, list, count, limit, out);
    });
  }
};

// ... 141 lines not shown
```

Measured before the change: 3.680 billion particle-updates/s.

## Add specialized fast frame2 kernel instance for f32 Philox exact-marker frames

Adds a k_frame2_fast instantiation, used when the frame is f32, Philox, exact marker count and pruned. It strips runtime branches (camera identity, k_upper, small-angle and diag checks), uses a Philox variant with scalar-register hints for the uniform counters, moves the n<2 special cases to a select after propagation, and scores with a duplicate check that only runs when a wave-wide ballot finds a collision. The goal is to cut per-particle instruction count and divergence in the weigh loop. The cost is extra code paths that must match the general kernel exactly, plus dependence on assumptions such as cam_identity and small angles holding whenever the host selects the fast path.

```diff
diff --git a/include/pfmpe.h b/include/pfmpe.h
--- a/include/pfmpe.h
+++ b/include/pfmpe.h
@@ -439,7 +439,9 @@
        PFMPE_INFO_LAST_GRID = 7,
        PFMPE_INFO_LAST_RESAMPLE = 8,
        PFMPE_INFO_NUM_CU = 9,
-       PFMPE_INFO_TAIL_FALLBACKS = 10 };
+       PFMPE_INFO_TAIL_FALLBACKS = 10,
+       PFMPE_INFO_LAST_FRAME2 = 11 };
+enum { PFMPE_FRAME2_GENERAL = 0, PFMPE_FRAME2_FAST = 1, PFMPE_FRAME2_FAST_STAMPS = 2 };
 enum { PFMPE_WEIGH_BLOCKS = 0, PFMPE_WEIGH_STREAM = 1, PFMPE_WEIGH_PK = 2 };
 enum { PFMPE_RESAMPLE_BLOCKS = 0, PFMPE_RESAMPLE_OWNERS = 1 };
 int pfmpe_get_info(const pfmpe_ctx* ctx, int key, int64_t* value);
diff --git a/pf_monocular_pose_estimator_amd/__init__.py b/pf_monocular_pose_estimator_amd/__init__.py
--- a/pf_monocular_pose_estimator_amd/__init__.py
+++ b/pf_monocular_pose_estimator_amd/__init__.py
@@ -22,6 +22,7 @@
     MODES_MAX, MODE_NONE, ModesParams, ModeOut, default_modes_params, host_cloud_assign,
     ASSOC_MAX_STREAMS, ASSOC_MAX_LAUNCHES, AssocMultiIn, AssocPlan, AssocPlanTotal, host_assoc_plan,
     GateParams, GateOut, default_gate_params, host_gate_pairs,
+    DIAG_STAMPS, DIAG_NO_FAST, INFO_LAST_FRAME2, FRAME2_GENERAL, FRAME2_FAST, FRAME2_FAST_STAMPS,
 )
 
 __all__ = [
diff --git a/pf_monocular_pose_estimator_amd/_capi.py b/pf_monocular_pose_estimator_amd/_capi.py
--- a/pf_monocular_pose_estimator_amd/_capi.py
+++ b/pf_monocular_pose_estimator_amd/_capi.py
@@ -28,6 +28,10 @@
 SHAPE_TWO_LAUNCH, SHAPE_FRAME, SHAPE_FRAME2 = 0, 1, 2
 INFO_FUSED, INFO_FUSED_FALLBACKS, INFO_LAST_SHAPE, INFO_GUARD_SKIPS, INFO_N, INFO_LAST_WEIGH_PASS = 1, 2, 3, 4, 5, 6
 INFO_LAST_GRID, INFO_LAST_RESAMPLE, INFO_NUM_CU, INFO_TAIL_FALLBACKS = 7, 8, 9, 10
+INFO_LAST_FRAME2 = 11
+FRAME2_GENERAL, FRAME2_FAST, FRAME2_FAST_STAMPS = 0, 1, 2
+DIAG_STAMPS = 4
+DIAG_NO_FAST = 1 << 21
 WEIGH_BLOCKS, WEIGH_STREAM, WEIGH_PK = 0, 1, 2
 RESAMPLE_BLOCKS, RESAMPLE_OWNERS = 0, 1
 CLOUD_WEIGHTED, CLOUD_POSTERIOR = 0, 1
diff --git a/pf_monocular_pose_estimator_amd/csrc/pf_kernels.hpp b/pf_monocular_pose_estimator_amd/csrc/pf_kernels.hpp
--- a/pf_monocular_pose_estimator_amd/csrc/pf_kernels.hpp
+++ b/pf_monocular_pose_estimator_amd/csrc/pf_kernels.hpp
@@ -2573,7 +2573,7 @@
   OutDev rec;
   Frame2Lds fl;
 };
-template <typename T, int RNG, int MAXM, bool PRUNE, typename SP>
+template <typename T, int RNG, int MAXM, bool PRUNE, typename SP, bool FAST = false>
 __device__ __forceinline__ bool frame2_body(
     const FrameArgsT<T>& fa, const uint32_t* fa_words, const unsigned char* __restrict__ table,
     const SP* __restrict__ prior, SP* __restrict__ post, T* __restrict__ w0, T* __restrict__ w1,
@@ -2593,7 +2593,7 @@
   const int blk = blockIdx.x, g_own = blk / fa.gsz;
 
   T A[12];
-  if (valid && n >= 2) load_prior(fa, prior, n, A);
+  if (valid && (FAST || n >= 2)) load_prior(fa, prior, n, A);
   stage_table_consts(table, smem, (size_t)fa.tbytes, fa_words, sc);
   if (threadIdx.x == 0) {
     fl.c = zero_ctrl();
@@ -2613,7 +2613,7 @@
   for (;; ++iter) {
     const int slot = c.cur_slot;
     if (valid) {
-      w = weigh_particle<T, RNG, MAXM, PRUNE, true>(fa, sc, tb, A, n, iter, P, nullptr, stamps);
+      w = weigh_particle<T, RNG, MAXM, PRUNE, true, FAST>(fa, sc, tb, A, n, iter, P, nullptr, stamps);
       (slot ? w1 : w0)[n] = w;
     }
     if (stamps && threadIdx.x == 0) stamp_max(stamps, 9, rt_now());
@@ -2669,7 +2669,7 @@
     double zmin_in[2];
     {
       const BlockPart* pp = (iter & 1) ? part1 : part0;
-      if ((fa.diag & kDiagLagLoads) && blk == fa.nblk - 1) {
+      if (!FAST && (fa.diag & kDiagLagLoads) && blk == fa.nblk - 1) {
         const uint64_t t0 = rt_now();
         while (rt_now() - t0 < 2000u) __builtin_amdgcn_s_sleep(2);
       }
@@ -2699,7 +2699,7 @@
     int dirty = 0;
 #pragma unroll
     for (int w = 0; w < kWaves; ++w) dirty |= fl.dirty[w];
-    if (dirty || (fa.diag & kDiagMinSide)) {
+    if (dirty || (!FAST && (fa.diag & kDiagMinSide))) {
       group_zmin2(in, zmin_in, &fl.bs[slot], wv < fa.ngrp ? &fl.gp[slot][wv] : nullptr,
                   wv + kWaves < fa.ngrp ? &fl.gp[slot][wv + kWaves] : nullptr);
       __syncthreads();
@@ -2777,6 +2777,20 @@
                                              seq, stamps, smem, S2);
 }
 
+template <typename SP, bool STAMPS>
+__global__ __launch_bounds__(kBlock) __attribute__((amdgpu_waves_per_eu(PFMPE_FRAME2_MIN_WAVES))) void k_frame2_fast(
+    const FrameArgsT<float> fa, const unsigned char* __restrict__ table, const SP* __restrict__ prior,
+    SP* __restrict__ post, float* __restrict__ w0, float* __restrict__ w1, BlockPart* __restrict__ part0,
+    BlockPart* __restrict__ part1, Ctrl* __restrict__ ctrl, CountPart* __restrict__ cpart,
+    uint32_t* __restrict__ flat, uint32_t* __restrict__ counts, Cand* __restrict__ cand,
+    double* __restrict__ mlpose, RecOut* __restrict__ out, int32_t seq, uint64_t* __restrict__ stamps) {
+  extern __shared__ __attribute__((aligned(16))) unsigned char smem[];
+  __shared__ Frame2Shared<float> S2;
+  (void)frame2_body<float, kRngPhilox, kExactM, true, SP, true>(
+      fa, (const uint32_t*)__builtin_amdgcn_kernarg_segment_ptr(), table, prior, post, w0, w1, part0, part1, ctrl, cpart,
+      flat, counts, cand, mlpose, out, seq, STAMPS ? stamps : nullptr, smem, S2);
+}
+
 template <typename T, int RNG, typename SP>
 __global__ __launch_bounds__(kBlock) void k_regen(const FrameArgsT<T> fa, int kept_iter, const SP* __restrict__ prior,
                                                  double* __restrict__ poses) {
diff --git a/pf_monocular_pose_estimator_amd/csrc/pf_likelihood.hpp b/pf_monocular_pose_estimator_amd/csrc/pf_likelihood.hpp
--- a/pf_monocular_pose_estimator_amd/csrc/pf_likelihood.hpp
+++ b/pf_monocular_pose_estimator_amd/csrc/pf_likelihood.hpp
@@ -42,11 +42,11 @@
   }
 }
 
-template <typename T, int MAXM>
+template <typename T, int MAXM, bool K_UPPER = false>
 __device__ __forceinline__ void project_markers(const FrameArgsT<T>& fa, const LdsConst<T>& sc, const T* P, T* u,
                                                 T* v) {
   T Q[12];
-  k_times_pose<T>(sc, P, fa.k_upper != 0, Q);
+  k_times_pose<T>(sc, P, K_UPPER || fa.k_upper != 0, Q);
   if constexpr (std::is_same<T, float>::value) {
     const f32x2 q0 = pk2(Q[0], Q[4]), q1 = pk2(Q[1], Q[5]), q2 = pk2(Q[2], Q[6]), q3 = pk2(Q[3], Q[7]);
 #pragma unroll
@@ -126,14 +126,15 @@
   return (int)__builtin_fminf(__builtin_fmaxf(f, 0.0f), (float)(nb - 1));
 }
 
-template <typename T, int MAXM, bool PRUNE, bool PHASED = false>
+template <typename T, int MAXM, bool PRUNE, bool PHASED = false, bool FAST = false>
 __device__ __forceinline__ int column_minima(const FrameArgsT<T>& fa, const T* u, const T* v,
                                              const LdsBlobs<T>& tb, T* m, int* r) {
   const int B = fa.B, M = fa.M;
   int visited = 0;
   if constexpr (std::is_same<T, float>::value) {
     const GridArgs& ga = fa.grid;
-    if (PRUNE && ga.on) {
+    static_assert(!FAST || (PRUNE && PHASED), "the fast instance searches the grid in phases");
+    if (PRUNE && (FAST || ga.on)) {
       const unsigned char* cells = tb.base + ga.cell_off;
       const unsigned char* ents = tb.base + ga.ent_off;
       const f32x2 ic = pk2(ga.inv_c, ga.inv_c), oc = pk2(ga.ox, ga.oy);
@@ -163,7 +164,10 @@
             more |= n > c1;
             const GridEnt e0 = e[0];
             const f32x2 dd = pk2(e0.x, e0.y) - uvj;
-            bd = __builtin_fminf(fmadd(dd.x, dd.x, dd.y * dd.y), INFINITY);
+            if constexpr (FAST)
+              bd = fmadd(dd.x, dd.x, dd.y * dd.y);
+            else
+              bd = __builtin_fminf(fmadd(dd.x, dd.x, dd.y * dd.y), INFINITY);
             bo = e0.orig;
             if constexpr (c1 == 2) {
               const GridEnt e1 = e[1];
@@ -427,6 +431,42 @@
   }
   return Pr - (float)(3 * dups * (dups + 1) / 2 + 2 * ndg);
 }
+template <int MAXM>
+__device__ __forceinline__ float score_unordered_rare(const FrameArgsT<float>& fa, const float* m, const int* r) {
+  static_assert(MAXM == kExactM && kMaxBlobs <= 0x8000, "every slot holds a marker; blob keys below 0x8000");
+  const float tol = fa.tol, tol_pf = fa.tol_pf, Mt = (float)MAXM;
+  const float rtol = rcp_t(tol);
+  float Pr = 0.0f;
+  bool acc[MAXM];
+  uint32_t key[MAXM];
+#pragma unroll
+  for (int j = 0; j < MAXM; ++j) {
+    const float d = sqrt_t(m[j]);
+    acc[j] = d <= tol_pf;
+    const float q = (tol - d) * rtol;
+    Pr = acc[j] ? Pr + (Mt + q * q) : Pr;
+    key[j] = acc[j] ? (uint32_t)r[j] : 0x8000u + (uint32_t)j;
+  }
+  uint32_t dmin = 0xffffffffu;
+#pragma unroll
+  for (int j = 1; j < MAXM; ++j)
+#pragma unroll
+    for (int e = 0; e < j; ++e) dmin = min(dmin, key[e] ^ key[j]);
+  if (__builtin_amdgcn_ballot_w64(dmin == 0u) != 0 || fa.downgrade) {
+    asm volatile("");
+    int dups = 0, ndg = 0;
+#pragma unroll
+    for (int j = 0; j < MAXM; ++j) {
+      bool dup = false;
+#pragma unroll
+      for (int e = 0; e < j; ++e) dup |= acc[e] & (r[e] == r[j]);
+      dups += (acc[j] & dup) ? 1 : 0;
+      ndg += (acc[j] && ((fa.downgrade >> j) & 1u)) ? 1 : 0;
+    }
+    Pr = Pr - (float)(3 * dups * (dups + 1) / 2 + 2 * ndg);
+  }
+  return Pr;
+}
 
 constexpr int kGridMaxCells = 8192;
 constexpr int kGridCoarseCells = 2048;
@@ -642,11 +682,28 @@
   for (int i = t + 2 * kBlock; i < n4; i += kBlock) d4[i] = s4[i];
 }
 
-template <typename T, int RNG, int MAXM, bool PRUNE, bool PHASED = false>
+template <typename T, int RNG, int MAXM, bool PRUNE, bool PHASED = false, bool FAST = false>
 __device__ __forceinline__ T weigh_particle(const FrameArgsT<T>& fa, const LdsConst<T>& sc, const LdsBlobs<T>& tb,
                                             const T* A, int n, int iter, T* P, int* nvisit = nullptr,
                                             uint64_t* st = nullptr) {
   T u[MAXM], v[MAXM];
+  if constexpr (FAST) {
+    static_assert(std::is_same<T, float>::value && RNG == kRngPhilox && MAXM == kExactM && PRUNE && PHASED,
+                  "the fast instance's frame class");
+    propagate<T, RNG, true>(fa, sc, A, n, iter, P);
+    if (st && threadIdx.x == 0) stamp_max(st, 27, rt_now() + (P[11] == (T)12345 ? 1 : 0));
+    project_markers<T, MAXM, true>(fa, sc, P, u, v);
+    if (st && threadIdx.x == 0) stamp_max(st, 28, rt_now() + (u[0] == (T)12345 ? 1 : 0));
+    T w = (T)0;
+    if (!__builtin_isunordered(u[0], v[0])) {
+      T m[MAXM];
+      int r[MAXM];
+      (void)column_minima<T, MAXM, PRUNE, PHASED, true>(fa, u, v, tb, m, r);
+      if (st && threadIdx.x == 0) stamp_max(st, 29, rt_now() + (m[0] == (T)12345 ? 1 : 0));
+      w = score_unordered_rare<MAXM>(fa, m, r);
+    }
+    return w;
+  }
   propagate<T, RNG>(fa, sc, A, n, iter, P);
   if (st && threadIdx.x == 0) stamp_max(st, 27, rt_now() + (P[11] == (T)12345 ? 1 : 0));
   project_markers<T, MAXM>(fa, sc, P, u, v);
diff --git a/pf_monocular_pose_estimator_amd/csrc/pf_rng.hpp b/pf_monocular_pose_estimator_amd/csrc/pf_rng.hpp
--- a/pf_monocular_pose_estimator_amd/csrc/pf_rng.hpp
+++ b/pf_monocular_pose_estimator_amd/csrc/pf_rng.hpp
@@ -108,6 +108,58 @@
   d.v[5] = ((o.z & 0x7FFu) << 10) | (o.w & 0x3FFu);
   return d;
 }
+PF_HD Draws6 philox_motion6_su(uint32_t n, uint32_t iter, uint32_t flo, uint32_t fhi, uint32_t k0, uint32_t k1) {
+  constexpr uint32_t M0 = 0xD2511F53u, M1 = 0xCD9E8D57u, W0 = 0x9E3779B9u, W1 = 0xBB67AE85u;
+  uint32_t c1 = iter | (kTagMotion << 24);
+#if defined(__HIP_DEVICE_COMPILE__)
+  asm volatile("" : "+s"(c1), "+s"(flo), "+s"(fhi), "+s"(k0), "+s"(k1));
+#endif
+  const uint64_t u1 = (uint64_t)M1 * flo;
+  const uint32_t r1n0 = (uint32_t)(u1 >> 32) ^ c1 ^ k0, r1n1 = (uint32_t)u1;
+  const uint32_t s13 = fhi ^ k1;
+  uint64_t p = (uint64_t)M0 * n;
+  uint32_t a2 = (uint32_t)(p >> 32) ^ s13, a3 = (uint32_t)p;
+  uint32_t rk0 = k0 + W0, rk1 = k1 + W1;
+  const uint64_t u2 = (uint64_t)M0 * r1n0;
+  const uint32_t r2n3 = (uint32_t)u2;
+  const uint32_t s20 = r1n1 ^ rk0, s22 = (uint32_t)(u2 >> 32) ^ rk1;
+  p = (uint64_t)M1 * a2;
+  uint32_t a0 = (uint32_t)(p >> 32) ^ s20, a1 = (uint32_t)p;
+  a2 = a3 ^ s22;
+  rk0 += W0;
+  rk1 += W1;
+  const uint32_t s33 = r2n3 ^ rk1;
+  {
+    const uint64_t q0 = (uint64_t)M0 * a0, q1 = (uint64_t)M1 * a2;
+    const uint32_t n0 = xor3_key((uint32_t)(q1 >> 32), a1, rk0), n2 = (uint32_t)(q0 >> 32) ^ s33;
+    a1 = (uint32_t)q1;
+    a3 = (uint32_t)q0;
+    a0 = n0;
+    a2 = n2;
+  }
+#if defined(__HIP_DEVICE_COMPILE__)
+  asm volatile("" : "+s"(rk0), "+s"(rk1));
+#endif
+#pragma unroll
+  for (int r = 3; r < 10; ++r) {
+    rk0 += W0;
+    rk1 += W1;
+    const uint64_t q0 = (uint64_t)M0 * a0, q1 = (uint64_t)M1 * a2;
+    const uint32_t n0 = xor3_key((uint32_t)(q1 >> 32), a1, rk0), n2 = xor3_key((uint32_t)(q0 >> 32), a3, rk1);
+    a1 = (uint32_t)q1;
+    a3 = (uint32_t)q0;
+    a0 = n0;
+    a2 = n2;
+  }
+  Draws6 d;
+  d.v[0] = a0 >> 11;
+  d.v[1] = a1 >> 11;
+  d.v[2] = a2 >> 11;
+  d.v[3] = a3 >> 11;
+  d.v[4] = ((a0 & 0x7FFu) << 10) | (a1 & 0x3FFu);
+  d.v[5] = ((a2 & 0x7FFu) << 10) | (a3 & 0x3FFu);
+  return d;
+}
 PF_HD float u21f(uint32_t v) { return (float)v * (1.0f / 2097152.0f); }
 PF_HD double u21d(uint32_t v) { return (double)v * (1.0 / 2097152.0); }
 
diff --git a/pf_monocular_pose_estimator_amd/csrc/pf_state.hpp b/pf_monocular_pose_estimator_amd/csrc/pf_state.hpp
--- a/pf_monocular_pose_estimator_amd/csrc/pf_state.hpp
+++ b/pf_monocular_pose_estimator_amd/csrc/pf_state.hpp
@@ -298,24 +298,26 @@
 template <>
 __device__ __forceinline__ double u21_t<double>(uint32_t v) { return u21d(v); }
 
-template <typename T, int RNG>
+template <typename T, int RNG, bool FAST = false>
 __device__ __forceinline__ void propagate(const FrameArgsT<T>& fa, const LdsConst<T>& sc, const T* A_in, int n,
                                           int iter, T* P) {
-  if (n == 0) {
-#pragma unroll
-    for (int q = 0; q < 12; ++q) P[q] = sc.cur[q];
-    return;
-  }
-  if (n == 1) {
-#pragma unroll
-    for (int q = 0; q < 12; ++q) P[q] = sc.pred[q];
-    return;
+  if constexpr (!FAST) {
+    if (n == 0) {
+#pragma unroll
+      for (int q = 0; q < 12; ++q) P[q] = sc.cur[q];
+      return;
+    }
+    if (n == 1) {
+#pragma unroll
+      for (int q = 0; q < 12; ++q) P[q] = sc.pred[q];
+      return;
+    }
   }
   T A[12];
 #pragma unroll
   for (int q = 0; q < 12; ++q) A[q] = A_in[q];
   if (fa.it > 1) {
-    if (!fa.cam_identity) {
+    if (!FAST && !fa.cam_identity) {
       T X[12];
       compose(sc.cam, A, X);
 #pragma unroll
@@ -341,7 +343,11 @@
       d[q] = (T)(ref_uniform(ref_canonical(g1, g2), fa.dlo[q], fa.dhi[q]) * gd);
     }
   } else {
-    const Draws6 r = philox_motion6((uint32_t)n, (uint32_t)iter, fa.flo, fa.fhi, fa.key0, fa.key1);
+    Draws6 r;
+    if constexpr (FAST)
+      r = philox_motion6_su((uint32_t)n, (uint32_t)iter, fa.flo, fa.fhi, fa.key0, fa.key1);
+    else
+      r = philox_motion6((uint32_t)n, (uint32_t)iter, fa.flo, fa.fhi, fa.key0, fa.key1);
 #pragma unroll
     for (int q = 0; q < 6; ++q) d[q] = (T)r.v[q] * sc.rgs[q] + sc.lo[q];
     if (iter >= 10) {
@@ -352,7 +358,7 @@
     }
   }
   T sa, ca, sb, cb, sz, cz;
-  if (fa.small_angles) {
+  if (FAST || fa.small_angles) {
     sincos_small(d[0], &sa, &ca);
     sincos_small(d[1], &sb, &cb);
     sincos_small(d[2], &sz, &cz);
@@ -375,6 +381,12 @@
     P[i * 4 + 2] = x2;
     P[i * 4 + 3] = A[i * 4 + 3] + d[3 + i];
   }
+  if constexpr (FAST) {
+    if (__builtin_amdgcn_readfirstlane(n) == 0) {
+#pragma unroll
+      for (int q = 0; q < 12; ++q) P[q] = n == 0 ? sc.cur[q] : (n == 1 ? sc.pred[q] : P[q]);
+    }
+  }
 }
 
 template <typename T, int RNG, typename SP>
diff --git a/pf_monocular_pose_estimator_amd/csrc/pf_types.hpp b/pf_monocular_pose_estimator_amd/csrc/pf_types.hpp
--- a/pf_monocular_pose_estimator_amd/csrc/pf_types.hpp
+++ b/pf_monocular_pose_estimator_amd/csrc/pf_types.hpp
@@ -151,7 +151,8 @@
   kDiagBlockResample = 32768,
   kDiagAssocDirect = 262144,
   kDiagDetCopy = 524288,
-  kDiagTailMiss = 1 << 20
+  kDiagTailMiss = 1 << 20,
+  kDiagNoFast = 1 << 21
 };
 
 constexpr int kShards = 8;
diff --git a/pf_monocular_pose_estimator_amd/csrc/pfmpe_ctx.hpp b/pf_monocular_pose_estimator_amd/csrc/pfmpe_ctx.hpp
--- a/pf_monocular_pose_estimator_amd/csrc/pfmpe_ctx.hpp
+++ b/pf_monocular_pose_estimator_amd/csrc/pfmpe_ctx.hpp
@@ -177,6 +177,7 @@
   int64_t wait_bound_us = 2000000;
   int64_t multi_max_blocks = 160000;
   int last_shape = -1;
+  int last_frame2 = -1;
   int last_weigh_pass = -1;
   int last_resample = -1;
   int64_t guard_skips = 0;
diff --git a/pf_monocular_pose_estimator_amd/csrc/pfmpe_engine.hip b/pf_monocular_pose_estimator_amd/csrc/pfmpe_engine.hip
--- a/pf_monocular_pose_estimator_amd/csrc/pfmpe_engine.hip
+++ b/pf_monocular_pose_estimator_amd/csrc/pfmpe_engine.hip
@@ -787,6 +787,7 @@
     case PFMPE_INFO_FUSED: *value = c->fused; return PFMPE_OK;
     case PFMPE_INFO_FUSED_FALLBACKS: *value = c->fused_fallbacks; return PFMPE_OK;
     case PFMPE_INFO_LAST_SHAPE: *value = c->last_shape; return PFMPE_OK;
+    case PFMPE_INFO_LAST_FRAME2: *value = c->last_frame2; return PFMPE_OK;
     case PFMPE_INFO_LAST_WEIGH_PASS: *value = c->last_weigh_pass; return PFMPE_OK;
     case PFMPE_INFO_LAST_RESAMPLE: *value = c->last_resample; return PFMPE_OK;
     case PFMPE_INFO_LAST_GRID: *value = c->last_grid; return PFMPE_OK;
diff --git a/pf_monocular_pose_estimator_amd/csrc/pfmpe_seq.hpp b/pf_monocular_pose_estimator_amd/csrc/pfmpe_seq.hpp
--- a/pf_monocular_pose_estimator_amd/csrc/pfmpe_seq.hpp
+++ b/pf_monocular_pose_estimator_amd/csrc/pfmpe_seq.hpp
@@ -207,7 +207,17 @@
   static int frame_fused(pfmpe_ctx* c, const FrameArgsT<T>& fa_in, const unsigned char* table, bool* launched) {
     *launched = false;
     const bool flat = c->fused == 2 && fa_in.nblk <= kFlatMaxGroups * kGroup && fa_in.gsz == kGroup && c->d_flat.get();
-    const void* fn = flat ? (const void*)k_frame2<T, RNG, MAXM, PRUNE, SP> : (const void*)k_frame<T, RNG, MAXM, PRUNE, SP>;
+    constexpr bool kHasFast = std::is_same<T, float>::value && RNG == kRngPhilox && MAXM == kExactM && PRUNE &&
+                              std::is_same<SP, float>::value;
+    int inst = PFMPE_FRAME2_GENERAL;
+    auto k2 = k_frame2<T, RNG, MAXM, PRUNE, SP>;
+    if constexpr (kHasFast) {
+      if (flat && pk_eligible(fa_in, kExactM) && !(fa_in.diag & (kDiagNoFast | kDiagLagLoads | kDiagMinSide))) {
+        inst = (fa_in.diag & kDiagStamps) ? PFMPE_FRAME2_FAST_STAMPS : PFMPE_FRAME2_FAST;
+        k2 = inst == PFMPE_FRAME2_FAST ? k_frame2_fast<SP, false> : k_frame2_fast<SP, true>;
+      }
+    }
+    const void* fn = flat ? (const void*)k2 : (const void*)k_frame<T, RNG, MAXM, PRUNE, SP>;
     const size_t lds = BlobTable<T>::lds_bytes(fa_in.tbytes);
     int occ = 0;
     RET(occupancy(c, fn, lds, 0, &occ));
@@ -237,7 +247,7 @@
     const int32_t seq = next_seq(c);
     RET(launch_ext(c, PFMPE_K_FRAME, [&] {
       if (flat)
-        klaunch(c, k_frame2<T, RNG, MAXM, PRUNE, SP>, dim3(a.nblk), dim3(kBlock), lds, a, table,
+        klaunch(c, k2, dim3(a.nblk), dim3(kBlock), lds, a, table,
                            prior, post, w0, w1, gran_part(c, 0), gran_part(c, 1), c->d_ctrl.get(), gran_count(c), c->d_flat.get(),
                            counts, c->d_cand.get(), c->d_mlpose.get(), c->h_rec.dev(), seq, c->d_stamps.get());
       else
@@ -248,6 +258,7 @@
                            n.tcount_w, n.gcount_r, n.tcount_r, c->d_gen.get(), counts, c->d_cand.get(), c->d_mlpose.get(), c->h_rec.dev(), seq,
                            c->d_stamps.get(), tree_count ? nullptr : c->d_flat.get());
     }));
+    if (flat) c->last_frame2 = inst;
     RET(tail_after(c));
     *launched = true;
     if (wait_frame(c) != PFMPE_OK) {
```

New measurement: 3.632 billion particle-updates/s. 1.3% lower.
